# ISAE-PNX/SaDVIO

Measured on AMD Instinct MI355X. Metric: BA iterations/sec (ms/solve in ms_per_solve), 20-KF/8k-landmark window, higher is better.
Workload: dtype f64; 1 GPU; synthetic 20 KF x 8000 landmarks x 40000 reprojection factors (pixel), GN 10 iters (LM step attempts, early exits disabled); windows_per_gpu=1, parallelism=single window, n_kf=20, n_lmk=8000, n_obs=40000, reduced_dim=114

## Files before the change

### sadvio_amd/csrc/ba_capi.hip

```cpp
#include <hip/hip_runtime.h>
#include <dlfcn.h>

#include <algorithm>
#include <chrono>
#include <cmath>
#include <cstdio>
#include <cstdlib>
#include <cstring>
#include <map>
#include <string>
#include <vector>

#include "../../include/sadvio_ba.h"
#include "kernels.h"
#include "dense_chol.h"
#include "marg_kernels.h"
#include "lm_kernels.h"
#include "viinit_kernels.h"
#include "nofov_kernels.h"

using namespace sadvio;

namespace {

#define HIP_TRY(expr)                                                                         \
    do {                                                                                      \
        hipError_t _e = (expr);                                                               \
        if (_e != hipSuccess) {                                                               \
            h->err = std::string(#expr) + ": " + hipGetErrorString(_e);                       \
            return SADVIO_E_HIP;                                                              \
        }                                                                                     \
    } while (0)

template <typename T>
struct DevBuf {
    T* p = nullptr;
    size_t n = 0;
    hipError_t alloc(size_t count) {
        if (count <= n && p && !view) return hipSuccess;
        if (p && !view) (void)hipFree(p);
        view = false;
        p = nullptr; n = 0;
        hipError_t e = hipMalloc((void**)&p, std::max<size_t>(count, 1) * sizeof(T));
        if (e == hipSuccess) n = count;
        return e;
    }
    bool view = false;
    void set_view(T* ptr, size_t count) { if (p && !view) (void)hipFree(p); p = ptr; n = count; view = true; }
    void release() { if (p && !view) (void)hipFree(p); p = nullptr; n = 0; view = false; }
    void swap(DevBuf& o) { std::swap(p, o.p); std::swap(n, o.n); std::swap(view, o.view); }
    DevBuf() = default;
    DevBuf(const DevBuf&) = delete;
    DevBuf& operator=(const DevBuf&) = delete;
    ~DevBuf() { release(); }
};

struct KernelClass {
    const char* name;
    double total_ms = 0;
    long long launches = 0;
};

struct HostWin {
    WinDev d;
    std::vector<int64_t> kf_id, lmk_id;
    int hb_lmk = 0;
};

}

struct NcclId { char internal[128]; };
struct RcclLib {
    void* lib = nullptr;
    void* comm = nullptr;
    int (*get_id)(NcclId*) = nullptr;
    int (*init_rank)(void**, int, NcclId, int) = nullptr;
    int (*all_reduce)(const void*, void*, size_t, int, int, void*, hipStream_t) = nullptr;
    int (*destroy)(void*) = nullptr;
    const char* (*err_string)(int) = nullptr;
    int (*comm_count)(void*, int*) = nullptr;
    int (*comm_user_rank)(void*, int*) = nullptr;
    int (*comm_cu_device)(void*, int*) = nullptr;
};

struct SrcWin {
    sadvio_flat_window v{};
    std::vector<int64_t> kf_id, lmk_id;
    std::vector<double> kf_T, kf_vel, kf_ba, kf_bg, cam_K, cam_T, cam_sigma, lmk_p, obs_meas;
    std::vector<uint8_t> kf_const, lmk_const;
    std::vector<int32_t> lmk_obs_ptr, obs_kf, obs_cam;
    std::vector<int32_t> a_ptr, a_kf, a_cam, a_src;
    std::vector<double> a_meas;
    std::vector<double> u_cam_K, u_cam_T, u_cam_sigma;
    std::vector<int32_t> u_obs_cam;
    std::vector<int> cam_map;
};

// ... 27 lines not shown
        if (pinned) { memcpy(np, pinned, used); (void)hipHostFree(pinned); }
        pinned = np; pinned_cap = cap;
    }
    void add(void* dst, const void* src, size_t bytes) {
        if (!bytes) return;
        wait();
        const size_t off = (used + 7) & ~(size_t)7;
        reserve(off + bytes);
        if (failed) return;
        memcpy(pinned + off, src, bytes);
        used = off + bytes;
        items.push_back({(unsigned long long)dst, (unsigned long long)off, (unsigned long long)bytes});
    }
    hipError_t flush(hipStream_t stream) {
        if (failed) { failed = false; items.clear(); used = 0; return hipErrorOutOfMemory; }
        if (items.empty()) return hipSuccess;
        const size_t data_bytes = (used + 7) & ~(size_t)7;
        const size_t total = data_bytes + items.size() * sizeof(UploadItem);
        reserve(total);
        if (failed) { failed = false; items.clear(); used = 0; return hipErrorOutOfMemory; }
        hipError_t e = hipSuccess;
        auto drop = [&](hipError_t err) { items.clear(); used = 0; return err; };
        if (!ev && (e = hipEventCreateWithFlags(&ev, hipEventDisableTiming)) != hipSuccess) return drop(e);
        if (dev_cap < total) {
            if (dev) { (void)hipStreamSynchronize(stream); (void)hipFree(dev); }
            dev = nullptr; dev_cap = 0;
            if ((e = hipMalloc((void**)&dev, total + total / 2)) != hipSuccess) return drop(e);
            dev_cap = total + total / 2;
        }
        memcpy(pinned + data_bytes, items.data(), items.size() * sizeof(UploadItem));
        if ((e = hipMemcpyAsync(dev, pinned, total, hipMemcpyHostToDevice, stream)) != hipSuccess) return drop(e);
        hipLaunchKernelGGL(k_scatter_uploads, dim3(64, (unsigned)std::min<size_t>(items.size(), 64)), dim3(256), 0, stream, dev, (const UploadItem*)(dev + data_bytes), (int)items.size());
        e = hipEventRecord(ev, stream);
        in_flight = e == hipSuccess;
        if (!in_flight) e = hipStreamSynchronize(stream);
        items.clear(); used = 0;
        return e;
    }
    ~UploadBatch() { wait(); if (ev) (void)hipEventDestroy(ev); if (pinned) (void)hipHostFree(pinned); if (dev) (void)hipFree(dev); }
};

struct DensePriorHost {
    int n_full = 0, n = 0, kf_keep = -1, kf_col = 0;
    bool resident = false;
    unsigned long long serial = 0;
    std::vector<double> J, r0;
    std::vector<int> lmk_index, lmk_col;
};

struct PriorState {
    bool valid = false;
    int n_full = 0, n = 0, form = 0, cut_mode = 0;
    DevBuf<double> J, r0;
    DevBuf<double> Z;
    bool z_valid = false;
    DevBuf<int> step_of;
    DevBuf<double> H, g;
    bool hg_valid = false;
    unsigned long long serial = 0;
};

struct TriLevel { int first, count, max_m, max_n; };
struct MargScratch {
    DevBuf<double> A, b, G, V, ev, Vs, Ainv, T, Ak, bk, newJ, newr, lastJ, lastr, L, Tb, Zt, S, mi, jsel, lam, wtmp, Hl;
    DevBuf<int> ditems, flag, sel, lastcol, piv_of, lc, piv_mm;
    DevBuf<MargSmall> small;
    DevBuf<NfrSpecC> spec;
    std::vector<int> lcol, items, items_l, col;
    std::vector<double> hev, hS;
    struct TriPlan { DevBuf<TriNode> nodes; std::vector<TriLevel> levels; int leaves = 0; };
    std::map<int, TriPlan> tri_plans;
};

struct LineSetHost {
    std::vector<int64_t> id;
    std::vector<double> T, model, meas;
    std::vector<unsigned char> is_const;
    std::vector<int> ptr, obs_kf, obs_cam;
    int n() const { return (int)id.size(); }
};

struct LayoutScratch {
    std::vector<double> kf_T0, kf_vel, kf_ba, kf_bg, cam_K, cam_T, cam_isig, lmk_p, obs_meas;
    std::vector<int> kf_fidx, lmk_ob, lmk_oe, obs_kf, obs_cam, tile_kf, tile_row, pkf, pcam, run_max, idx, mark, add, kfs, slot_of, chunk_ob, chunk_lm, perm;
    std::vector<unsigned char> lmk_const, obs_slot, obs_lslot;
    std::vector<char> held;
};

struct EnvCfg {
    int debug = 0;
    int lm = -1, pf_wg = -1;
    int tile_rounds = 0, lm_subs = 0, band_c = 0;
    double jacobi_tol = 1e-14;
    bool marg_last_small = false, marg_eig_mm = false, marg_pivoted = false, marg_unpivoted = false, pchol_swap = false, pchol_strict = false,
         jacobi_b4 = false, jacobi_plain = false, no_lpt = false, no_pre = false, no_fork = false, no_bcr = false, imu_items = false;
    void read() {
        auto on = [](const char* k) { return getenv(k) != nullptr; };
        auto num = [](const char* k, int unset) { const char* e = getenv(k); return e ? atoi(e) : unset; };
        debug = num("SADVIO_DEBUG", 0); lm = num("SADVIO_LM", -1); pf_wg = num("SADVIO_PF_WG", -1);
        tile_rounds = num("SADVIO_TILE_ROUNDS", 0); lm_subs = num("SADVIO_LM_SUBS", 0); band_c = num("SADVIO_BAND_C", 0);
        if (const char* e = getenv("SADVIO_JACOBI_TOL")) jacobi_tol = atof(e);
        marg_last_small = on("SADVIO_MARG_LAST_SMALL"); marg_eig_mm = on("SADVIO_MARG_EIG_MM"); marg_pivoted = on("SADVIO_MARG_PIVOTED");
        marg_unpivoted = on("SADVIO_MARG_UNPIVOTED"); pchol_swap = on("SADVIO_PCHOL_SWAP"); pchol_strict = on("SADVIO_PCHOL_STRICT");
        jacobi_b4 = on("SADVIO_JACOBI_B4"); jacobi_plain = on("SADVIO_JACOBI_PLAIN"); no_lpt = on("SADVIO_NO_LPT"); no_pre = on("SADVIO_NO_PRE"); no_fork = on("SADVIO_NO_FORK");
        no_bcr = on("SADVIO_NO_BCR");
        imu_items = on("SADVIO_IMU_ITEMS");
    }
};

struct sadvio_ba_handle {
    EnvCfg env;
    sadvio_ba_config cfg{};
    LayoutScratch ls;
    int device = 0;
    hipStream_t stream = nullptr;
    std::string err;
    std::vector<HostWin> wins;
    std::vector<Tile> tiles;
    std::vector<PriorDev> priors;
    std::vector<int> obs_perm;
    std::vector<std::vector<PriorDev>> priors_per_win;
    std::vector<std::vector<ImuDev>> imus_per_win;
    std::vector<ImuDev> imus;
    int n_kf_tot = 0, n_cam_tot = 0, n_lmk_tot = 0, n_obs_tot = 0, np_tot = 0;
    long long s_tot = 0;
    int factor_type = 0;
    int max_n_kf = 0, max_npose = 0, max_np = 0, n_big = 0;
    DevBuf<int> d_big_info;
    DevBuf<double> d_big_M;
    DevBuf<double> d_big_Lx;
    DevBuf<double> d_big_linv;
    DevBuf<double> d_coll_band;
    DevBuf<double> d_bcr;
    DevBuf<double> d_big_mid;
    bool uploaded = false, solved = false;
    bool defer = false, pending = false;
    UploadBatch up;
    int world = 1, rank = 0;
    sadvio_allreduce_fn coll_fn = nullptr;
    void* coll_ctx = nullptr;
    RcclLib rccl;
    long long red_total = 0;
    DevBuf<double> d_rank_b, d_rank_s;
    std::vector<DensePriorHost> dprior_per_win;
    PriorState prior;
    MargScratch mg;
    std::vector<SrcWin> src;
    std::vector<std::vector<char>> sp_elim;
    std::vector<int> n_obs_user;
    std::vector<std::vector<sadvio_sparse_prior>> sparse_per_win;
    std::vector<LineSetHost> lines_per_win;
    DevBuf<LineDev> d_lines;
    DevBuf<LineObsDev> d_lobs;
    DevBuf<double> d_xline, d_line_scratch;
    int n_line_tot = 0, n_lobs_tot = 0;
    DevBuf<SparseDev> d_sparse;
    DevBuf<int> d_sp_list;
    int n_sp_list = 0;
    size_t n_sparse_tot = 0;
    DevBuf<double> d_sp_scratch;
    std::vector<unsigned char> h_lmk_const_user;
    std::vector<int> h_lmk_ob, h_lmk_oe, h_kf_fidx, h_obs_kf;
    bool user_lmk_const = false;
    int n_kept = 0;
    DevBuf<int> d_lmk_red, d_kept_obs, d_dp_ints;
    DevBuf<double> d_dp_data;
    int slots_cap = 0;
    int last_slots = 0;
    DevBuf<WinDev> d_win;
    DevBuf<Tile> d_tiles;
    DevBuf<double> d_kf_T0, d_xp, d_xv, d_xba, d_xbg, d_kf_vel, d_kf_ba, d_kf_bg;
    DevBuf<int> d_kf_fidx;
    DevBuf<double> d_cam_K, d_cam_T, d_cam_isig;
    DevBuf<double> d_lmk_p, d_xl, d_s_lmk;
    DevBuf<unsigned char> d_lmk_const;
    DevBuf<int> d_lmk_ob, d_lmk_oe, d_obs_kf, d_obs_cam, d_tile_kf, d_tile_row;
    DevBuf<int> d_pre_lane, d_pre_kf;
    bool pre_ok = false, pre_dirty = false;
    DevBuf<int> d_rank_col; DevBuf<double> d_rank_x;
    DevBuf<unsigned char> d_obs_slot, d_obs_lslot;
    DevBuf<int> d_chunk_ob, d_chunk_lm, d_tile_perm;
    DevBuf<int> d_jac_ints;
    DevBuf<double> d_jac_dbl;
    DevBuf<double> d_lm_hg, d_lm_dt, d_lm_sacc;
    DevBuf<int> d_lm_sub;
    int lm_n_sub = 0, lm_ksub = 1, lm_sub_per_item = 8;
    int lm_max_cam = 1;
    int hidden_eig_count = 0;
    int marg_stats[4] = {0, 0, 0, 0};
    int lm_sub_obs = 0;
    bool gemm_run4 = false;
    bool lm_ok = false;
    long long lm_landmarks = 0;
    DevBuf<double> d_ptab;
    int max_tile_kf = 1, max_tile_free = 0, max_gemm_free = 0;
    DevBuf<double> d_obs_meas;
    DevBuf<PriorDev> d_priors;
    DevBuf<double> d_prior_lin;
    DevBuf<ImuDev> d_imus;
    DevBuf<double> d_imu_scratch;
    DevBuf<double> d_S, d_gred, d_gfull, d_hdiag, d_delta, d_s_pose;
    DevBuf<LmState> d_states;
    DevBuf<double> d_trace;
    DevBuf<long long> d_tstart;
    DevBuf<IterAcc> d_acc;
    DevBuf<FinalRec> d_final;
    FinalRec* h_final = nullptr;
    double* h_deltas = nullptr; size_t h_deltas_cap = 0; bool deltas_cached = false;
    size_t h_final_n = 0;
    std::vector<FinalRec> fin;
    DevBuf<TileAcc> d_tacc;
    DevBuf<long long> d_dbg;
    hipGraphExec_t graph_exec = nullptr;
    std::vector<unsigned char> graph_key;
    DevBuf<double> d_probe;
    bool has_lmk_const = false;
    std::vector<KernelClass> kclasses;
    hipStream_t side = nullptr;
    hipEvent_t ev_fork = nullptr, ev_lin = nullptr, ev_solved = nullptr, ev_cost = nullptr;
    std::vector<std::pair<hipEvent_t, hipEvent_t>> ev_pool;
    std::vector<std::pair<int, int>> ev_used;
    size_t ev_next = 0;
};

namespace {

int kclass_id(sadvio_ba_handle* h, const char* name) {
    for (size_t i = 0; i < h->kclasses.size(); i++)
        if (!strcmp(h->kclasses[i].name, name)) return (int)i;
    KernelClass k; k.name = name;
    h->kclasses.push_back(k);
    return (int)h->kclasses.size() - 1;
}

struct ScopedTimer {
    sadvio_ba_handle* h;
    int pool = -1;
    ScopedTimer(sadvio_ba_handle* h_, const char* name) : h(h_) {
        if (!h->cfg.profile_kernels) return;
        if (h->ev_next == h->ev_pool.size()) {
            hipEvent_t a, b;
            if (hipEventCreate(&a) != hipSuccess || hipEventCreate(&b) != hipSuccess) return;
            h->ev_pool.push_back({a, b});
        }
        pool = (int)h->ev_next++;
        h->ev_used.push_back({kclass_id(h, name), pool});
        (void)hipEventRecord(h->ev_pool[pool].first, h->stream);
    }
    ~ScopedTimer() {
        if (pool >= 0) (void)hipEventRecord(h->ev_pool[pool].second, h->stream);
    }
};

void collect_timers(sadvio_ba_handle* h) {
    for (auto& u : h->ev_used) {
        float ms = 0;
        if (hipEventElapsedTime(&ms, h->ev_pool[u.second].first, h->ev_pool[u.second].second) == hipSuccess) {
            h->kclasses[u.first].total_ms += ms;
            h->kclasses[u.first].launches += 1;
        }
    }
    h->ev_used.clear();
    h->ev_next = 0;
}

DevPtrs make_ptrs(sadvio_ba_handle* h, const SolveOpts& o, int state_stride) {
    DevPtrs P{};
    P.win = h->d_win.p; P.tiles = h->d_tiles.p;
    P.kf_T0 = h->d_kf_T0.p; P.kf_fidx = h->d_kf_fidx.p;
    P.xp = h->d_xp.p; P.xv = h->d_xv.p; P.xba = h->d_xba.p; P.xbg = h->d_xbg.p;
    P.xp_stride = 6LL * h->n_kf_tot; P.xv_stride = 3LL * h->n_kf_tot; P.xl_stride = 3LL * h->n_lmk_tot;
    P.kf_vel = h->d_kf_vel.p; P.kf_ba = h->d_kf_ba.p; P.kf_bg = h->d_kf_bg.p;
    P.cam_K = h->d_cam_K.p; P.cam_T = h->d_cam_T.p; P.cam_isig = h->d_cam_isig.p;
    P.lmk_p = h->d_lmk_p.p; P.xl = h->d_xl.p; P.s_lmk = h->d_s_lmk.p;
    P.lmk_const = h->has_lmk_const ? h->d_lmk_const.p : nullptr;
    P.lmk_ob = h->d_lmk_ob.p; P.lmk_oe = h->d_lmk_oe.p;
    P.obs_kf = h->d_obs_kf.p; P.obs_cam = h->d_obs_cam.p; P.obs_meas = h->d_obs_meas.p;
    P.obs_slot = h->d_obs_slot.p; P.tile_kf = h->d_tile_kf.p; P.tile_row = h->d_tile_row.p;
    P.pre_lane = h->pre_ok ? (const int4*)h->d_pre_lane.p : nullptr; P.pre_kf = h->pre_ok ? (const int2*)h->d_pre_kf.p : nullptr;
    P.ptab = h->d_ptab.p; P.ptab_stride = (long long)POSE_TAB * h->n_kf_tot;
    P.priors = h->d_priors.p; P.prior_lin = h->d_prior_lin.p; P.prior_lin_stride = (long long)h->priors.size() * PRIOR_LIN; P.n_prior_tot = (int)h->priors.size();
    P.imus = h->d_imus.p; P.imu_scratch = h->d_imu_scratch.p; P.imu_scratch_stride = (long long)h->imus.size() * IMU_ROW;
    P.S = h->d_S.p; P.gred = h->d_gred.p; P.gfull = h->d_gfull.p; P.hdiag = h->d_hdiag.p;
    P.delta = h->d_delta.p; P.s_pose = h->d_s_pose.p;
    P.dbg_ts = h->d_dbg.p;
    P.trace = h->d_trace.p; P.t_start = h->d_tstart.p;
    P.states = h->d_states.p; P.acc = h->d_acc.p; P.tacc = h->d_tacc.p; P.n_tiles = (int)h->tiles.size();
    P.state_stride = state_stride;
    P.final_out = h->h_final ? h->h_final : h->d_final.p;
    P.big_info = h->d_big_info.p;
    P.world = h->world; P.rank = h->rank; P.rank_b = h->d_rank_b.p; P.rank_s = h->d_rank_s.p;
    P.lmk_red = h->d_lmk_red.p; P.kept_obs = h->d_kept_obs.p; P.n_kept = h->n_kept;
    P.dp_data = h->d_dp_data.p; P.dp_ints = h->d_dp_ints.p;
    P.sparse = h->d_sparse.p; P.sp_scratch = h->d_sp_scratch.p; P.sp_list = h->d_sp_list.p;
    P.sp_scratch_stride = (long long)std::max<size_t>(h->n_sparse_tot, 1) * SPARSE_J; P.n_imu_tot = (int)h->imus.size(); P.n_sp_list = h->n_sp_list;
    P.chunk_ob = h->d_chunk_ob.p; P.chunk_lm = h->d_chunk_lm.p; P.tile_perm = h->d_tile_perm.p; P.obs_lslot = h->d_obs_lslot.p;
    P.lm_hg = h->d_lm_hg.p; P.lm_hg_stride = (long long)LM_HG * std::max(h->n_lmk_tot, 1);
    P.lm_dt = h->d_lm_dt.p; P.lm_dt_stride = (long long)LM_DT * std::max<long long>((long long)h->tiles.size(), 1) * h->lm_ksub;
    P.lm_sub = h->d_lm_sub.p; P.lm_ksub = h->lm_ksub; P.lm_sub_per_item = h->lm_sub_per_item; P.lm_sacc = h->lm_ok ? h->d_lm_sacc.p : nullptr;
    P.lines = h->d_lines.p; P.lobs = h->d_lobs.p; P.xline = h->d_xline.p; P.line_scratch = h->d_line_scratch.p;
    P.xline_stride = 6LL * h->n_line_tot;
    P.n_xp = (long long)h->d_xp.n; P.n_xv = (long long)h->d_xv.n; P.n_xl = (long long)h->d_xl.n;
    P.n_win = (int)h->wins.size();
    P.debug = h->env.debug;
    P.o = o;
    return P;
}

__global__ void k_dense_prior_prepare(const double* J, double* Jt, int nf, int n) {
    const long long idx = (long long)blockIdx.x * blockDim.x + threadIdx.x;
    if (idx < (long long)nf * n) {
        const int i = (int)(idx / n), a = (int)(idx - (long long)i * n);
        Jt[(size_t)a * nf + i] = J[idx];
    }
}

__global__ void k_sym_from_lower(const double* __restrict__ A, int n, double* __restrict__ H) {
    const long long idx = (long long)blockIdx.x * blockDim.x + threadIdx.x;
    if (idx >= (long long)n * n) return;
    const int i = (int)(idx / n), j = (int)(idx - (long long)i * n);
    H[idx] = i >= j ? A[idx] : A[(size_t)j * n + i];
}

int layout_reduced(sadvio_ba_handle* h) {
    const int n_windows = (int)h->wins.size();
    for (int w = 0; w < n_windows && w < (int)h->dprior_per_win.size(); w++) {
        const DensePriorHost& D = h->dprior_per_win[w];
        if (D.n_full > 0 && D.resident && (!h->prior.valid || h->prior.serial != D.serial || h->prior.n_full != D.n_full || h->prior.n != D.n)) {
            h->up.reset();
            h->err = "the handle's prior changed after set_dense_prior(SADVIO_PRIOR_RESIDENT) attached it to a window: attach it again"; return SADVIO_E_STATE;
        }
    }
    int red_b = 0; long long s_b = 0;
    h->max_np = 0; h->n_big = 0;
    std::vector<int> lmk_red(std::max(h->n_lmk_tot, 1), -1);
    std::vector<unsigned char> lmk_const = h->h_lmk_const_user;
    std::vector<int> kept, dp_ints;
    std::vector<SparseDev> sparse;
    std::vector<int> sp_list;
    std::vector<LineDev> lines;
    std::vector<LineObsDev> lobs;
    long long dp_total = 0;
    bool any_red = false;
    struct Prep { long long off; int nf, n, w; };
    std::vector<Prep> preps;
    for (int w = 0; w < n_windows; w++) {
        WinDev& d = h->wins[w].d;
        const DensePriorHost& D = h->dprior_per_win[w];
        int n_red = 0;
        d.dp_n_full = d.dp_n = 0; d.dp_off = 0; d.dp_int_off = 0;
        d.kept_begin = (int)kept.size() / 3;
        if (D.n_full > 0) {
            const int n = D.n, nf = D.n_full;
            std::vector<int> kind(n, -1), index(n, 0), col(n, -1);
            if (D.kf_keep >= 0) {
                const int g = d.kf_base + D.kf_keep, fi = h->h_kf_fidx[g];
                for (int q = 0; q < 15; q++) {
                    const int a = D.kf_col + q;
                    if (q < 6) { kind[a] = 0; index[a] = 6 * g + q; }
                    else { kind[a] = 1 + (q - 6) / 3; index[a] = 3 * g + (q - 6) % 3; }
                    col[a] = (fi >= 0 && q < d.dpf) ? fi * d.dpf + q : -1;
// ... 98 lines not shown
    h->d_gred.set_view(h->d_S.p + s_b, (size_t)red_b); h->d_gfull.set_view(h->d_gred.p + red_b, (size_t)red_b);
    h->d_hdiag.set_view(h->d_gfull.p + red_b, (size_t)red_b); h->d_rank_b.set_view(h->d_hdiag.p + red_b, (size_t)nrb);
    HIP_TRY(h->d_rank_s.alloc((size_t)nrb));
    HIP_TRY(h->d_delta.alloc((size_t)std::max(red_b, 1))); HIP_TRY(h->d_s_pose.alloc((size_t)std::max(red_b, 1)));
    HIP_TRY(hipMemsetAsync(h->d_S.p, 0, sizeof(double) * (size_t)std::max<long long>(h->red_total, 1), h->stream));
    HIP_TRY(hipMemsetAsync(h->d_rank_s.p, 0, sizeof(double) * (size_t)nrb, h->stream));
    HIP_TRY(h->d_sparse.alloc(std::max<size_t>(sparse.size(), 1))); HIP_TRY(h->d_sp_scratch.alloc(2 * std::max<size_t>(sparse.size(), 1) * SPARSE_J)); h->n_sparse_tot = sparse.size();
    h->up.add(h->d_sparse.p, sparse.data(), sparse.size() * sizeof(SparseDev));
    HIP_TRY(h->d_sp_list.alloc(std::max<size_t>(sp_list.size(), 1)));
    h->n_sp_list = (int)sp_list.size();
    h->up.add(h->d_sp_list.p, sp_list.data(), sp_list.size() * sizeof(int));
    h->n_line_tot = (int)lines.size(); h->n_lobs_tot = (int)lobs.size();
    HIP_TRY(h->d_lines.alloc(std::max<size_t>(lines.size(), 1))); HIP_TRY(h->d_lobs.alloc(std::max<size_t>(lobs.size(), 1)));
    HIP_TRY(h->d_xline.alloc(std::max<size_t>(12 * lines.size(), 1))); HIP_TRY(h->d_line_scratch.alloc(std::max<size_t>(lobs.size(), 1) * LINE_ROW));
    h->up.add(h->d_lines.p, lines.data(), lines.size() * sizeof(LineDev));
    h->up.add(h->d_lobs.p, lobs.data(), lobs.size() * sizeof(LineObsDev));
    if (kept.empty()) kept.assign(3, 0);
    if (dp_ints.empty()) dp_ints.push_back(0);
    HIP_TRY(h->d_tiles.alloc(h->tiles.size())); HIP_TRY(h->d_lmk_red.alloc(lmk_red.size())); HIP_TRY(h->d_lmk_const.alloc(lmk_const.size()));
    HIP_TRY(h->d_kept_obs.alloc(kept.size())); HIP_TRY(h->d_dp_ints.alloc(dp_ints.size())); HIP_TRY(h->d_dp_data.alloc((size_t)std::max<long long>(dp_total, 1)));
#define UP(dst, src) h->up.add((dst).p, (src).data(), (src).size() * sizeof((src)[0]))
    UP(h->d_tiles, h->tiles); UP(h->d_lmk_red, lmk_red); UP(h->d_lmk_const, lmk_const); UP(h->d_kept_obs, kept);
    UP(h->d_dp_ints, dp_ints);
#undef UP
    if (!preps.empty()) HIP_TRY(hipMemsetAsync(h->d_dp_data.p, 0, sizeof(double) * (size_t)dp_total, h->stream));
    for (const Prep& pr : preps) {
        const DensePriorHost& D = h->dprior_per_win[pr.w];
        double* J = h->d_dp_data.p + pr.off;
        double* r0 = J + 2 * (size_t)pr.nf * pr.n + (size_t)pr.n * pr.n;
        if (D.resident) {
            if (!h->prior.valid || h->prior.serial != D.serial || h->prior.n_full != pr.nf || h->prior.n != pr.n) {
                h->err = "the handle's prior changed after set_dense_prior(SADVIO_PRIOR_RESIDENT) attached it to a window: attach it again"; return SADVIO_E_STATE;
            }
            HIP_TRY(hipMemcpyAsync(J, h->prior.J.p, sizeof(double) * (size_t)pr.nf * pr.n, hipMemcpyDeviceToDevice, h->stream));
            HIP_TRY(hipMemcpyAsync(r0, h->prior.r0.p, sizeof(double) * (size_t)pr.nf, hipMemcpyDeviceToDevice, h->stream));
        } else {
            h->up.add(J, D.J.data(), sizeof(double) * (size_t)pr.nf * pr.n);
            h->up.add(r0, D.r0.data(), sizeof(double) * (size_t)pr.nf);
        }
    }
    if (!preps.empty()) HIP_TRY(h->up.flush(h->stream));
    for (const Prep& pr : preps) {
        double* J = h->d_dp_data.p + pr.off;
        double* Jt = J + (size_t)pr.nf * pr.n;
        double* H = Jt + (size_t)pr.n * pr.nf;
        const long long items = (long long)pr.nf * pr.n;
        hipLaunchKernelGGL(k_dense_prior_prepare, dim3((unsigned)((items + 255) / 256)), dim3(256), 0, h->stream, J, Jt, pr.nf, pr.n);
        if (h->dprior_per_win[pr.w].resident && h->prior.hg_valid && h->prior.n == pr.n && !h->env.marg_last_small)
            hipLaunchKernelGGL(k_sym_from_lower, dim3((unsigned)(((long long)pr.n * pr.n + 255) / 256)), dim3(256), 0, h->stream, h->prior.H.p, pr.n, H);
        else
        hipLaunchKernelGGL(k_mgemm, dim3((pr.n + 63) / 64, (pr.n + 63) / 64), dim3(256), 0, h->stream, H, (long long)pr.n, J, 1LL, (long long)pr.n, J, (long long)pr.n, 1LL,
                           pr.n, pr.n, pr.nf, 1.0, 0.0);
    }
    return SADVIO_OK;
}

int upload_priors(sadvio_ba_handle* h) {
    h->priors.clear();
    for (size_t w = 0; w < h->wins.size(); w++) {
        h->wins[w].d.prior_begin = (int)h->priors.size();
        for (auto& p : h->priors_per_win[w]) h->priors.push_back(p);
        h->wins[w].d.prior_end = (int)h->priors.size();
    }
    HIP_TRY(h->d_priors.alloc(h->priors.size()));
    HIP_TRY(h->d_prior_lin.alloc(2 * h->priors.size() * (size_t)PRIOR_LIN));
    if (!h->priors.empty())
        h->up.add(h->d_priors.p, h->priors.data(), h->priors.size() * sizeof(PriorDev));
    h->imus.clear();
    for (size_t w = 0; w < h->wins.size(); w++) {
        h->wins[w].d.imu_begin = (int)h->imus.size();
        for (auto& f : h->imus_per_win[w]) { h->imus.push_back(f); h->imus.back().win = (int)w; }
        h->wins[w].d.imu_end = (int)h->imus.size();
    }
    HIP_TRY(h->d_imus.alloc(h->imus.size()));
    HIP_TRY(h->d_imu_scratch.alloc(2 * h->imus.size() * (size_t)IMU_ROW));
    if (!h->imus.empty())
        h->up.add(h->d_imus.p, h->imus.data(), h->imus.size() * sizeof(ImuDev));
    std::vector<WinDev> wd(h->wins.size());
    for (size_t w = 0; w < h->wins.size(); w++) wd[w] = h->wins[w].d;
    h->up.add(h->d_win.p, wd.data(), wd.size() * sizeof(WinDev));
    HIP_TRY(h->up.flush(h->stream));
    if (h->pre_ok && h->pre_dirty) {
        hipLaunchKernelGGL(k_pre_packets, dim3((unsigned)h->tiles.size()), dim3(BUILD_THREADS), 0, h->stream, h->d_tiles.p, h->d_lmk_ob.p, h->d_lmk_oe.p, h->d_tile_kf.p,
                           h->d_kf_fidx.p, (int4*)h->d_pre_lane.p, (int2*)h->d_pre_kf.p);
        h->pre_dirty = false;
    }
    return SADVIO_OK;
}

}

extern "C" {

int sadvio_ba_device_count(void) {
    int n = 0;
    if (hipGetDeviceCount(&n) != hipSuccess) return 0;
    int ok = 0;
    for (int i = 0; i < n; i++) {
        hipDeviceProp_t p;
        if (hipGetDeviceProperties(&p, i) == hipSuccess && strstr(p.gcnArchName, "gfx950")) ok++;
    }
    return ok;
}

void sadvio_ba_default_options(sadvio_solve_options* o) {
    if (!o) return;
    memset(o, 0, sizeof(*o));
    o->max_num_iterations = 20;
    o->function_tolerance = 1e-3;
    o->jacobi_scaling = 1;
    o->max_num_consecutive_invalid_steps = 5;
    o->gradient_tolerance = 1e-10;
    o->parameter_tolerance = 1e-8;
    o->initial_trust_region_radius = 1e4;
    o->max_trust_region_radius = 1e16;
    o->min_trust_region_radius = 1e-32;
    o->min_lm_diagonal = 1e-6;
    o->max_lm_diagonal = 1e32;
    o->min_relative_decrease = 1e-3;
}

int sadvio_ba_create(const sadvio_ba_config* cfg, sadvio_ba_handle** out) {
    if (!out) return SADVIO_E_INVALID_ARG;
    *out = nullptr;
    int n = 0;
    if (hipGetDeviceCount(&n) != hipSuccess || n == 0) return SADVIO_E_NO_DEVICE;
    int dev = cfg ? cfg->device : 0;
    if (dev < 0 || dev >= n) return SADVIO_E_INVALID_ARG;
    hipDeviceProp_t prop;
    if (hipGetDeviceProperties(&prop, dev) != hipSuccess) return SADVIO_E_HIP;
    if (!strstr(prop.gcnArchName, "gfx950")) return SADVIO_E_NO_DEVICE;
    if (hipSetDevice(dev) != hipSuccess) return SADVIO_E_HIP;
    auto* h = new sadvio_ba_handle();
    h->env.read();
    if (cfg) h->cfg = *cfg;
    h->device = dev;
    if (hipStreamCreateWithFlags(&h->stream, hipStreamNonBlocking) != hipSuccess) { delete h; return SADVIO_E_HIP; }
    if (hipStreamCreateWithFlags(&h->side, hipStreamNonBlocking) != hipSuccess) h->side = nullptr;
    for (hipEvent_t* e : {&h->ev_fork, &h->ev_lin, &h->ev_solved, &h->ev_cost})
        if (hipEventCreateWithFlags(e, hipEventDisableTiming) != hipSuccess) { *e = nullptr; if (h->side) { (void)hipStreamDestroy(h->side); h->side = nullptr; } }
    *out = h;
    return SADVIO_OK;
}

void sadvio_ba_destroy(sadvio_ba_handle* h) {
    if (!h) return;
    (void)hipSetDevice(h->device);
    if (h->stream) { (void)hipStreamSynchronize(h->stream); }
    if (h->graph_exec) (void)hipGraphExecDestroy(h->graph_exec);
    if (h->rccl.comm) (void)h->rccl.destroy(h->rccl.comm);
    if (h->h_final) (void)hipHostFree(h->h_final);
    if (h->h_deltas) (void)hipHostFree(h->h_deltas);
    if (h->side) { (void)hipStreamSynchronize(h->side); (void)hipStreamDestroy(h->side); }
    for (hipEvent_t e : {h->ev_fork, h->ev_lin, h->ev_solved, h->ev_cost}) if (e) (void)hipEventDestroy(e);
    if (h->stream) (void)hipStreamDestroy(h->stream);
    for (auto& e : h->ev_pool) { (void)hipEventDestroy(e.first); (void)hipEventDestroy(e.second); }
    h->d_win.release(); h->d_tiles.release(); h->d_kf_T0.release(); h->d_xp.release(); h->d_xv.release();
    h->d_xba.release(); h->d_xbg.release(); h->d_kf_vel.release(); h->d_kf_ba.release(); h->d_kf_bg.release();
    h->d_kf_fidx.release(); h->d_cam_K.release(); h->d_cam_T.release(); h->d_cam_isig.release();
    h->d_lmk_p.release(); h->d_xl.release(); h->d_s_lmk.release(); h->d_lmk_const.release();
    h->d_lmk_ob.release(); h->d_lmk_oe.release(); h->d_obs_kf.release(); h->d_obs_cam.release();
    h->d_obs_meas.release(); h->d_priors.release(); h->d_prior_lin.release(); h->d_S.release(); h->d_rank_s.release(); h->d_gred.release(); h->d_gfull.release();
    h->d_hdiag.release(); h->d_delta.release(); h->d_s_pose.release(); h->d_states.release(); h->d_trace.release(); h->d_tstart.release(); h->d_acc.release();
    h->d_probe.release(); h->d_tile_kf.release(); h->d_tile_row.release(); h->d_obs_slot.release(); h->d_ptab.release(); h->d_tacc.release(); h->d_dbg.release(); h->d_imus.release(); h->d_imu_scratch.release();
    delete h;
}

static int build_layout(sadvio_ba_handle* h) {
    const bool dbg_t = (h->env.debug & 8192) != 0;
    auto t_start = std::chrono::steady_clock::now();
    auto lap = [&](const char* what) { if (dbg_t) { auto t = std::chrono::steady_clock::now(); fprintf(stderr, "[sadvio dbg] build_layout %-14s %.3f ms\n", what, std::chrono::duration<double, std::milli>(t - t_start).count()); t_start = t; } };
    const int n_windows = (int)h->src.size();
    HIP_TRY(hipSetDevice(h->device));
    h->solved = false;
    h->up.reset();
    h->wins.assign(n_windows, HostWin());
    h->tiles.clear();
    h->sp_elim.assign(n_windows, {});
    h->n_obs_user.assign(n_windows, 0);
    std::vector<sadvio_flat_window> views(n_windows);
    int sp_global = 0;
    for (int w = 0; w < n_windows; w++) {
        SrcWin& S = h->src[w];
        const auto& sp = h->sparse_per_win[w];
        h->sp_elim[w].assign(sp.size(), 0);
        h->n_obs_user[w] = S.v.n_obs;
        views[w] = S.v;
        {
            std::vector<int> cmap(S.v.n_cam, -1);
            S.u_cam_K.clear(); S.u_cam_T.clear(); S.u_cam_sigma.clear();
            for (int c = 0; c < S.v.n_cam; c++) {
                const double sg = S.cam_sigma.empty() ? 1.0 : S.cam_sigma[c];
                const int nu = (int)S.u_cam_sigma.size();
                for (int u = 0; u < nu && cmap[c] < 0; u++)
                    if (!memcmp(&S.u_cam_K[4 * u], &S.cam_K[4 * c], 32) && !memcmp(&S.u_cam_T[12 * u], &S.cam_T[12 * c], 96) && S.u_cam_sigma[u] == sg) cmap[c] = u;
                if (cmap[c] < 0) {
                    cmap[c] = nu;
                    S.u_cam_K.insert(S.u_cam_K.end(), &S.cam_K[4 * c], &S.cam_K[4 * c] + 4);
                    S.u_cam_T.insert(S.u_cam_T.end(), &S.cam_T[12 * c], &S.cam_T[12 * c] + 12);
                    S.u_cam_sigma.push_back(sg);
                }
            }
            S.u_obs_cam.resize(S.obs_cam.size());
            for (size_t o = 0; o < S.obs_cam.size(); o++) S.u_obs_cam[o] = cmap[S.obs_cam[o]];
            S.cam_map = cmap;
            views[w].n_cam = (int32_t)S.u_cam_sigma.size();
            views[w].cam_K = S.u_cam_K.data(); views[w].cam_T_s_f = S.u_cam_T.data(); views[w].cam_sigma = S.u_cam_sigma.data();
            views[w].obs_cam = S.u_obs_cam.data();
        }
        if (sp.empty()) { S.a_src.clear(); continue; }
        auto& held = h->ls.held;
        held.assign(std::max(S.v.n_lmk, 1), 0);
        const DensePriorHost& D = h->dprior_per_win[w];
        for (size_t i = 0; i < D.lmk_index.size(); i++) if (D.n_full > 0 && D.lmk_col[i] >= 0) held[D.lmk_index[i]] = 1;
        for (const auto& s : sp) {
            if (s.type == SADVIO_SPARSE_LMK_PRIOR) held[s.lmk0] = 1;
            if (s.type == SADVIO_SPARSE_LMK_TO_LMK) { held[s.lmk0] = 1; held[s.lmk1] = 1; }
        }
        std::vector<std::vector<int>> extra(S.v.n_lmk);
        bool any = false;
        for (size_t k = 0; k < sp.size(); k++) {
            const auto& s = sp[k];
            if (s.type != SADVIO_SPARSE_POSE_TO_LMK || held[s.lmk0]) continue;
            if (!S.lmk_const.empty() && S.lmk_const[s.lmk0]) continue;
            h->sp_elim[w][k] = 1;
            extra[s.lmk0].push_back(sp_global + (int)k);
            any = true;
        }
        sp_global += (int)sp.size();
        if (any) {
            const int ms = S.v.factor_type == SADVIO_FACTOR_PIXEL ? 2 : 3;
            S.a_ptr.assign(1, 0); S.a_kf.clear(); S.a_cam.clear(); S.a_src.clear(); S.a_meas.clear();
            for (int l = 0; l < S.v.n_lmk; l++) {
                for (int o = S.lmk_obs_ptr[l]; o < S.lmk_obs_ptr[l + 1]; o++) {
                    S.a_kf.push_back(S.obs_kf[o]); S.a_cam.push_back(S.u_obs_cam[o]); S.a_src.push_back(o);
                    for (int q = 0; q < ms; q++) S.a_meas.push_back(S.obs_meas[(size_t)ms * o + q]);
                }
                for (int gfi : extra[l])
                    for (int half = 0; half < 2; half++) {
                        const auto& s = sp[gfi - (sp_global - (int)sp.size())];
                        S.a_kf.push_back(s.kf); S.a_cam.push_back(-1 - (2 * gfi + half)); S.a_src.push_back(-1);
                        for (int q = 0; q < ms; q++) S.a_meas.push_back(0.0);
                    }
                S.a_ptr.push_back((int32_t)S.a_kf.size());
            }
            views[w].n_obs = (int32_t)S.a_kf.size();
            views[w].lmk_obs_ptr = S.a_ptr.data(); views[w].obs_kf = S.a_kf.data(); views[w].obs_cam = S.a_cam.data();
            views[w].obs_meas = S.a_meas.data();
        } else {
            S.a_src.clear();
        }
    }
    lap("views");
    const sadvio_flat_window* wins = views.data();
    h->factor_type = wins[0].factor_type;
    int kf_b = 0, cam_b = 0, lmk_b = 0, obs_b = 0;
    h->max_n_kf = h->max_npose = h->max_np = 0; h->n_big = 0;
    h->has_lmk_const = false;
    for (int w = 0; w < n_windows; w++) {
        const sadvio_flat_window& F = wins[w];
        if (F.n_kf <= 0 || F.n_cam < 0 || F.n_lmk < 0 || F.n_obs < 0 || !F.kf_T_f_w || (F.n_cam > 0 && (!F.cam_K || !F.cam_T_s_f)) ||
            (F.n_obs > 0 && F.n_cam == 0) ||
            (F.n_lmk > 0 && (!F.lmk_p || !F.lmk_obs_ptr)) || (F.n_obs > 0 && (!F.obs_kf || !F.obs_cam || !F.obs_meas))) {
            h->err = "set_windows: missing array in window " + std::to_string(w);
            return SADVIO_E_INVALID_ARG;
        }
        if (F.factor_type != h->factor_type || (F.factor_type != SADVIO_FACTOR_PIXEL && F.factor_type != SADVIO_FACTOR_ANGULAR)) {
            h->err = "set_windows: all windows of a batch must share one factor_type";
            return SADVIO_E_INVALID_ARG;
        }
        if (F.n_lmk > 0 && (F.lmk_obs_ptr[0] != 0 || F.lmk_obs_ptr[F.n_lmk] != F.n_obs)) {
            h->err = "set_windows: lmk_obs_ptr is not a CSR over n_obs";
            return SADVIO_E_INVALID_ARG;
        }
        if (F.lmk_const) h->has_lmk_const = true;
        HostWin& H = h->wins[w];
        WinDev& d = H.d;
        memset(&d, 0, sizeof(d));
        d.n_kf = F.n_kf; d.n_cam = F.n_cam; d.n_lmk = F.n_lmk; d.n_obs = F.n_obs;
        d.kf_base = kf_b; d.cam_base = cam_b; d.lmk_base = lmk_b; d.obs_base = obs_b;
        d.factor_type = F.factor_type; d.has_imu = F.has_imu;
        d.dpf = F.has_imu ? 15 : 6;
        int nfree = 0;
        for (int k = 0; k < F.n_kf; k++)
            if (!(F.kf_const && F.kf_const[k])) nfree++;
        d.n_free_kf = nfree;
        d.Npose = nfree * 6;
        d.Np = nfree * d.dpf;
        H.kf_id.assign(F.n_kf, 0); H.lmk_id.assign(F.n_lmk, 0);
        for (int k = 0; k < F.n_kf; k++) H.kf_id[k] = F.kf_id ? F.kf_id[k] : k;
        for (int l = 0; l < F.n_lmk; l++) H.lmk_id[l] = F.lmk_id ? F.lmk_id[l] : l;
        kf_b += F.n_kf; cam_b += F.n_cam; lmk_b += F.n_lmk; obs_b += F.n_obs;
        h->max_n_kf = std::max(h->max_n_kf, F.n_kf);
        h->max_npose = std::max(h->max_npose, d.Npose);
    }
    h->n_kf_tot = kf_b; h->n_cam_tot = cam_b; h->n_lmk_tot = lmk_b; h->n_obs_tot = obs_b;

    lap("  validate");
    LayoutScratch& ls = h->ls;
    auto& kf_T0 = ls.kf_T0; auto& kf_vel = ls.kf_vel; auto& kf_ba = ls.kf_ba; auto& kf_bg = ls.kf_bg; auto& kf_fidx = ls.kf_fidx;
    auto& cam_K = ls.cam_K; auto& cam_T = ls.cam_T; auto& cam_isig = ls.cam_isig; auto& lmk_p = ls.lmk_p; auto& lmk_const = ls.lmk_const;
    auto& lmk_ob = ls.lmk_ob; auto& lmk_oe = ls.lmk_oe; auto& obs_kf = ls.obs_kf; auto& obs_cam = ls.obs_cam; auto& obs_meas = ls.obs_meas;
    auto& tile_kf = ls.tile_kf; auto& tile_row = ls.tile_row; auto& obs_slot = ls.obs_slot;
    kf_T0.resize(12 * (size_t)kf_b); kf_vel.assign(3 * (size_t)kf_b, 0.0); kf_ba.assign(3 * (size_t)kf_b, 0.0); kf_bg.assign(3 * (size_t)kf_b, 0.0);
    kf_fidx.resize(kf_b);
    cam_K.resize(4 * (size_t)cam_b); cam_T.resize(12 * (size_t)cam_b); cam_isig.resize(cam_b);
    lmk_p.resize(3 * (size_t)lmk_b);
    lmk_const.assign(std::max(lmk_b, 1), 0);
    lmk_ob.resize(std::max(lmk_b, 1)); lmk_oe.resize(std::max(lmk_b, 1)); obs_kf.resize(std::max(obs_b, 1)); obs_cam.resize(std::max(obs_b, 1));
    const int ms = h->factor_type == SADVIO_FACTOR_PIXEL ? 2 : 3;
    obs_meas.resize((size_t)ms * std::max(obs_b, 1));
    tile_kf.clear(); tile_row.clear();
    obs_slot.assign(std::max(obs_b, 1), 0);
    h->obs_perm.assign(std::max(obs_b, 1), 0);
    h->max_tile_kf = 1; h->max_tile_free = 0; h->max_gemm_free = 0; h->gemm_run4 = false;
    for (int w = 0; w < n_windows; w++) {
        const sadvio_flat_window& F = wins[w];
        WinDev& d = h->wins[w].d;
        memcpy(&kf_T0[12 * (size_t)d.kf_base], F.kf_T_f_w, sizeof(double) * 12 * F.n_kf);
        if (F.kf_vel) memcpy(&kf_vel[3 * (size_t)d.kf_base], F.kf_vel, sizeof(double) * 3 * F.n_kf);
        if (F.kf_ba) memcpy(&kf_ba[3 * (size_t)d.kf_base], F.kf_ba, sizeof(double) * 3 * F.n_kf);
        if (F.kf_bg) memcpy(&kf_bg[3 * (size_t)d.kf_base], F.kf_bg, sizeof(double) * 3 * F.n_kf);
        int fi = 0;
        for (int k = 0; k < F.n_kf; k++) kf_fidx[d.kf_base + k] = (F.kf_const && F.kf_const[k]) ? -1 : fi++;
        memcpy(&cam_K[4 * (size_t)d.cam_base], F.cam_K, sizeof(double) * 4 * F.n_cam);
        memcpy(&cam_T[12 * (size_t)d.cam_base], F.cam_T_s_f, sizeof(double) * 12 * F.n_cam);
        for (int c = 0; c < F.n_cam; c++) cam_isig[d.cam_base + c] = 1.0 / (F.cam_sigma ? F.cam_sigma[c] : 1.0);
        if (F.n_lmk) memcpy(&lmk_p[3 * (size_t)d.lmk_base], F.lmk_p, sizeof(double) * 3 * F.n_lmk);
        for (int l = 0; l < F.n_lmk; l++) {
            lmk_const[d.lmk_base + l] = F.lmk_const ? F.lmk_const[l] : 0;
            lmk_ob[d.lmk_base + l] = d.obs_base + F.lmk_obs_ptr[l];
            lmk_oe[d.lmk_base + l] = d.obs_base + F.lmk_obs_ptr[l + 1];
            if (F.lmk_obs_ptr[l + 1] < F.lmk_obs_ptr[l]) { h->err = "set_windows: CSR not monotone"; return SADVIO_E_INVALID_ARG; }
        }
        lap("  concat");
        auto& pkf = ls.pkf; auto& pcam = ls.pcam; auto& run_max = ls.run_max; auto& idx = ls.idx;
        pkf.resize(std::max(F.n_obs, 1)); pcam.resize(std::max(F.n_obs, 1));
        run_max.assign(std::max(F.n_lmk, 1), 0);
        const bool has_asrc = !h->src[w].a_src.empty();
        const int32_t* asrc = has_asrc ? h->src[w].a_src.data() : nullptr;
        bool all_sorted = true;
        int hb_win = 0;
        const int* fidx_w = kf_fidx.data() + d.kf_base;
        for (int l = 0; l < F.n_lmk; l++) {
            const int o0 = F.lmk_obs_ptr[l], o1 = F.lmk_obs_ptr[l + 1];
            int run = 0, rm = 0, prev = -1, lo = 1 << 30, hi = -1;
            for (int o = o0; o < o1; o++) {
                const int kf = F.obs_kf[o];
                if (kf < prev) { all_sorted = false; }
                run = (kf == prev) ? run + 1 : 1;
                rm = std::max(rm, run);
                prev = kf;
                const int fi = fidx_w[kf];
                if (fi >= 0) { lo = std::min(lo, fi); hi = std::max(hi, fi); }
            }
            run_max[l] = rm;
            if (hi >= 0) hb_win = std::max(hb_win, hi - lo);
        }
        h->wins[w].hb_lmk = hb_win;
        if (all_sorted) {
            const int kb = d.kf_base, cb = d.cam_base, ob = d.obs_base, n = F.n_obs;
            for (int o = 0; o < n; o++) { pkf[o] = F.obs_kf[o]; obs_kf[ob + o] = kb + F.obs_kf[o]; }
            for (int o = 0; o < n; o++) { const int c = F.obs_cam[o]; pcam[o] = c; obs_cam[ob + o] = c < 0 ? c : cb + c; }
            if (has_asrc) for (int o = 0; o < n; o++) h->obs_perm[ob + o] = asrc[o];
            else for (int o = 0; o < n; o++) h->obs_perm[ob + o] = o;
            if (n) memcpy(&obs_meas[(size_t)ms * ob], F.obs_meas, sizeof(double) * (size_t)ms * n);
        } else
        for (int l = 0; l < F.n_lmk; l++) {
            const int o0 = F.lmk_obs_ptr[l], o1 = F.lmk_obs_ptr[l + 1], k_n = o1 - o0;
            int key[64];
            const int32_t* okf = F.obs_kf + o0;
            if (k_n <= 64 && F.n_kf < (1 << 22)) {
                for (int k = 0; k < k_n; k++) key[k] = (okf[k] << 8) | k;
                for (int a = 1; a < k_n; a++) {
                    const int v = key[a];
                    int b = a - 1;
                    while (b >= 0 && key[b] > v) { key[b + 1] = key[b]; b--; }
                    key[b + 1] = v;
                }
            } else {
                idx.resize(k_n);
                for (int k = 0; k < k_n; k++) idx[k] = k;
                std::stable_sort(idx.begin(), idx.end(), [&](int a, int b) { return okf[a] < okf[b]; });
            }
            int run = 0, rm = 0, prev = -1;
            const int kb = d.kf_base, cb = d.cam_base, ob = d.obs_base;
            for (int k = 0; k < k_n; k++) {
                const int rel = k_n <= 64 && F.n_kf < (1 << 22) ? (key[k] & 255) : idx[k];
                const int src = o0 + rel, dst = o0 + k;
                const int kf = okf[rel], c = F.obs_cam[src];
                pkf[dst] = kf; pcam[dst] = c;
                h->obs_perm[ob + dst] = has_asrc ? asrc[src] : src;
                obs_kf[ob + dst] = kb + kf;
                obs_cam[ob + dst] = c < 0 ? c : cb + c;
                const double* m = F.obs_meas + (size_t)ms * src;
                double* md = &obs_meas[(size_t)ms * (ob + dst)];
                md[0] = m[0]; md[1] = m[1]; if (ms == 3) md[2] = m[2];
                run = (kf == prev) ? run + 1 : 1;
                rm = std::max(rm, run);
                prev = kf;
            }
            run_max[l] = rm;
        }
        lap("  sort+permute");
        lap("  half-bandwidth");
        if (F.n_cam > MAX_WIN_CAM) { h->err = "set_windows: more than 8 distinct cameras per window"; return SADVIO_E_INVALID_ARG; }
        int tile_rounds = 1;
        {
            long long l_tot = 0;
            for (int ww = 0; ww < n_windows; ww++) l_tot += views[ww].n_lmk;
            tile_rounds = (int)std::min<long long>(16, std::max<long long>(1, (l_tot + 32LL * 2048 - 1) / (32LL * 2048)));
            if (h->env.tile_rounds > 0) tile_rounds = h->env.tile_rounds;
        }
        d.tile_begin = (int)h->tiles.size();
        {
            int l = 0;
            auto& mark = ls.mark; auto& add = ls.add; auto& kfs = ls.kfs; auto& slot_of = ls.slot_of;
            mark.assign(F.n_kf, -1); slot_of.assign(F.n_kf, -1);
            while (l < F.n_lmk || (int)h->tiles.size() == d.tile_begin) {
                Tile t{};
                t.w = w; t.lmk0 = d.lmk_base + l; t.kmax = 1; t.G = 8;
                t.dpf = d.dpf;
                t.cam_base = d.cam_base; t.n_cam = F.n_cam;
                t.first_of_window = ((int)h->tiles.size() == d.tile_begin) ? 1 : 0;
                kfs.clear();
                int nfree = 0, tile_run_max = 0;
                const int l_begin = l;
                while (l < F.n_lmk) {
                    const int k = F.lmk_obs_ptr[l + 1] - F.lmk_obs_ptr[l];
                    if (k > MAX_LMK_OBS) { h->err = "set_windows: a landmark has more than 64 observations"; return SADVIO_E_INVALID_ARG; }
                    int G = t.G;
                    while (G < k) G <<= 1;
                    const int cap = tile_rounds * BUILD_WAVES * (64 / G);
                    if (l - l_begin + 1 > cap && l > l_begin) break;
                    add.clear();
                    int add_free = 0;
                    for (int o = F.lmk_obs_ptr[l]; o < F.lmk_obs_ptr[l + 1]; o++) {
                        const int kf = pkf[o];
                        if (mark[kf] != (int)h->tiles.size()) {
                            mark[kf] = (int)h->tiles.size();
                            add.push_back(kf);
                            if (!(F.kf_const && F.kf_const[kf])) add_free++;
                        }
                    }
                    const bool fits_hard = (int)(kfs.size() + add.size()) <= MAX_TILE_KF && nfree + add_free <= MAX_TILE_FREE_KF;
                    const bool fits = fits_hard && (nfree + add_free <= MAX_GEMM_FREE_KF || l == l_begin);
                    if (!fits && l > l_begin) {
                        for (int kf : add) mark[kf] = -1;
                        break;
                    }
                    for (int kf : add) kfs.push_back(kf);
                    nfree += add_free;
                    t.G = G;
                    t.kmax = std::max(t.kmax, k);
                    tile_run_max = std::max(tile_run_max, run_max[l]);
                    l++;
                    if (!fits_hard) break;
                }
                t.lmk1 = d.lmk_base + l;
                std::sort(kfs.begin(), kfs.end());
                t.lds_mode = ((int)kfs.size() <= MAX_TILE_KF && nfree <= MAX_TILE_FREE_KF) ? ((nfree <= MAX_GEMM_FREE_KF && tile_run_max <= (has_asrc ? 4 : 2) && t.G == 8) ? 2 : 1) : 0;
                if (t.lds_mode == 2 && tile_run_max > 2) h->gemm_run4 = true;
                if (t.lds_mode == 2) h->max_gemm_free = std::max(h->max_gemm_free, nfree);
                if ((int)kfs.size() > 64) { h->err = "set_windows: a landmark is observed from more than 64 key-frames"; return SADVIO_E_INVALID_ARG; }
                t.kf_off = (int)tile_kf.size(); t.n_kf = (int)kfs.size(); t.n_free = t.lds_mode ? nfree : 0;
                int rank = 0;
                for (size_t i = 0; i < kfs.size(); i++) {
                    const int kf = kfs[i];
                    slot_of[kf] = (int)i;
                    tile_kf.push_back(d.kf_base + kf);
                    const bool is_const = F.kf_const && F.kf_const[kf];
                    if (is_const) tile_row.push_back(-1);
                    else if (t.lds_mode) tile_row.push_back(6 * rank++);
                    else tile_row.push_back(6 * kf_fidx[d.kf_base + kf]);
                }
                for (int ll = l_begin; ll < l; ll++)
                    for (int o = F.lmk_obs_ptr[ll]; o < F.lmk_obs_ptr[ll + 1]; o++)
                        obs_slot[d.obs_base + o] = (unsigned char)slot_of[pkf[o]];
                h->max_tile_kf = std::max(h->max_tile_kf, t.n_kf);
                h->max_tile_free = std::max(h->max_tile_free, t.n_free);
                h->tiles.push_back(t);
                if (F.n_lmk == 0) break;
            }
        }
        d.tile_end = (int)h->tiles.size();
        for (int ti = d.tile_begin; ti < d.tile_end; ti++) { h->tiles[ti].win_tile0 = d.tile_begin; h->tiles[ti].win_ntiles = d.tile_end - d.tile_begin; }
    }
    lap("concat+tiles");
    auto& chunk_ob = ls.chunk_ob; auto& chunk_lm = ls.chunk_lm;
    auto& obs_lslot = ls.obs_lslot;
    chunk_ob.clear(); chunk_lm.clear();
    obs_lslot.assign(std::max(obs_b, 1), 0);
    bool want_lm = lmk_b >= 65536;
    if (h->env.lm >= 0) want_lm = h->env.lm != 0;
    h->lm_ok = want_lm && !h->tiles.empty();
    h->lm_landmarks = 0;
    h->lm_sub_obs = 0;
    for (auto& t : h->tiles) {
        if (!want_lm) { t.chunk0 = t.chunk1 = 0; continue; }
        t.chunk0 = (int)chunk_lm.size();
        if (t.lds_mode != 2) h->lm_ok = false;
        int l = t.lmk0;
        while (l < t.lmk1) {
            chunk_lm.push_back(l); chunk_ob.push_back(lmk_ob[l]);
            int nl = 0, no = 0;
            while (l < t.lmk1 && nl < LM_CHUNK && no + (lmk_oe[l] - lmk_ob[l]) <= 64) {
                for (int o = lmk_ob[l]; o < lmk_oe[l]; o++) obs_lslot[o] = (unsigned char)nl;
                no += lmk_oe[l] - lmk_ob[l]; nl++; l++;
            }
            if (nl == 0) { h->lm_ok = false; l++; }
        }
        t.chunk1 = (int)chunk_lm.size();
        h->lm_landmarks += t.lmk1 - t.lmk0;
    }
    chunk_lm.push_back(lmk_b); chunk_ob.push_back(obs_b);
    if (want_lm) {
        for (const auto& t : h->tiles)
            for (int l0 = t.lmk0; l0 < t.lmk1; l0 += LM_PASS_THREADS) {
                const int l1 = std::min(l0 + LM_PASS_THREADS, t.lmk1);
                h->lm_sub_obs = std::max(h->lm_sub_obs, lmk_oe[l1 - 1] - lmk_ob[l0]);
            }
        h->lm_sub_obs = (h->lm_sub_obs + 3) & ~3;
        h->lm_max_cam = 1;
        for (const auto& t : h->tiles) h->lm_max_cam = std::max(h->lm_max_cam, t.n_cam);
        HIP_TRY(h->d_lm_hg.alloc(2 * (size_t)LM_HG * std::max(lmk_b, 1)));
        h->lm_ksub = 1;
        for (const auto& t : h->tiles) h->lm_ksub = std::max(h->lm_ksub, (t.lmk1 - t.lmk0 + LM_PASS_THREADS - 1) / LM_PASS_THREADS);
        const size_t n_rec = std::max<size_t>(h->tiles.size(), 1) * h->lm_ksub;
        HIP_TRY(h->d_lm_dt.alloc(2 * (size_t)LM_DT * n_rec));
        HIP_TRY(h->d_lm_sacc.alloc(2 * 4 * n_rec));
        HIP_TRY(hipMemsetAsync(h->d_lm_sacc.p, 0, sizeof(double) * 2 * 4 * n_rec, h->stream));
        HIP_TRY(hipMemsetAsync(h->d_lm_dt.p, 0, sizeof(double) * 2 * (size_t)LM_DT * n_rec, h->stream));
    }
    HIP_TRY(h->d_chunk_ob.alloc(chunk_ob.size())); HIP_TRY(h->d_chunk_lm.alloc(chunk_lm.size())); HIP_TRY(h->d_obs_lslot.alloc(obs_lslot.size()));
    h->up.add(h->d_chunk_ob.p, chunk_ob.data(), chunk_ob.size() * sizeof(int));
    h->up.add(h->d_chunk_lm.p, chunk_lm.data(), chunk_lm.size() * sizeof(int));
    h->up.add(h->d_obs_lslot.p, obs_lslot.data(), obs_lslot.size());
    {
        auto& perm = ls.perm;
        perm.resize(h->tiles.size());
        for (size_t i = 0; i < perm.size(); i++) perm[i] = (int)i;
        if (want_lm && !h->env.no_lpt)
            std::stable_sort(perm.begin(), perm.end(), [&](int a, int b) {
                return h->tiles[a].chunk1 - h->tiles[a].chunk0 > h->tiles[b].chunk1 - h->tiles[b].chunk0; });
        if (h->env.debug && want_lm && !perm.empty())
            fprintf(stderr, "[sadvio dbg] chunks per tile: largest %d, median %d, smallest %d\n", h->tiles[perm.front()].chunk1 - h->tiles[perm.front()].chunk0,
                    h->tiles[perm[perm.size() / 2]].chunk1 - h->tiles[perm[perm.size() / 2]].chunk0, h->tiles[perm.back()].chunk1 - h->tiles[perm.back()].chunk0);
        HIP_TRY(h->d_tile_perm.alloc(std::max<size_t>(perm.size(), 1)));
        h->up.add(h->d_tile_perm.p, perm.data(), perm.size() * sizeof(int));
        std::vector<int> sub;
        if (h->env.lm_subs > 0) h->lm_sub_per_item = h->env.lm_subs;
        if (want_lm)
            for (int ti : perm) {
                const Tile& t = h->tiles[ti];
                for (int q = 0, l0 = t.lmk0; l0 < t.lmk1; l0 += LM_PASS_THREADS * h->lm_sub_per_item, q += h->lm_sub_per_item) { sub.push_back(ti); sub.push_back(q); }
            }
        h->lm_n_sub = (int)sub.size() / 2;
        HIP_TRY(h->d_lm_sub.alloc(std::max<size_t>(sub.size(), 2)));
        h->up.add(h->d_lm_sub.p, sub.data(), sub.size() * sizeof(int));
    }
    if (h->env.debug) {
        int hist[32] = {0}, modes[3] = {0};
        for (auto& t : h->tiles) { hist[std::min(t.n_free, 31)]++; modes[t.lds_mode]++; }
        fprintf(stderr, "[sadvio dbg] %zu tiles, modes global/atomic/gemm = %d/%d/%d, max_tile_kf %d, n_free histogram:", h->tiles.size(), modes[0], modes[1], modes[2], h->max_tile_kf);
        for (int i = 0; i < 32; i++) if (hist[i]) fprintf(stderr, " %d:%d", i, hist[i]);
        fprintf(stderr, "\n");
    }
    HIP_TRY(h->d_win.alloc(n_windows)); HIP_TRY(h->d_tacc.alloc(2 * h->tiles.size()));
    if (tile_kf.empty()) { tile_kf.push_back(0); tile_row.push_back(-1); }
    HIP_TRY(h->d_tile_kf.alloc(tile_kf.size())); HIP_TRY(h->d_tile_row.alloc(tile_row.size()));
    HIP_TRY(h->d_obs_slot.alloc(obs_slot.size())); HIP_TRY(h->d_ptab.alloc(2 * (size_t)POSE_TAB * kf_b));
    HIP_TRY(h->d_kf_T0.alloc(kf_T0.size())); HIP_TRY(h->d_kf_fidx.alloc(kf_fidx.size()));
    HIP_TRY(h->d_xp.alloc(2 * 6 * (size_t)kf_b)); HIP_TRY(h->d_xv.alloc(2 * 3 * (size_t)kf_b));
    HIP_TRY(h->d_xba.alloc(2 * 3 * (size_t)kf_b)); HIP_TRY(h->d_xbg.alloc(2 * 3 * (size_t)kf_b));
    HIP_TRY(h->d_kf_vel.alloc(kf_vel.size())); HIP_TRY(h->d_kf_ba.alloc(kf_ba.size())); HIP_TRY(h->d_kf_bg.alloc(kf_bg.size()));
    HIP_TRY(h->d_cam_K.alloc(cam_K.size())); HIP_TRY(h->d_cam_T.alloc(cam_T.size())); HIP_TRY(h->d_cam_isig.alloc(cam_isig.size()));
    HIP_TRY(h->d_lmk_p.alloc(lmk_p.size())); HIP_TRY(h->d_xl.alloc(2 * 3 * (size_t)std::max(lmk_b, 1)));
    HIP_TRY(h->d_s_lmk.alloc(3 * (size_t)std::max(lmk_b, 1)));
    HIP_TRY(h->d_lmk_ob.alloc(lmk_ob.size())); HIP_TRY(h->d_lmk_oe.alloc(lmk_oe.size()));
    HIP_TRY(h->d_obs_kf.alloc(obs_kf.size())); HIP_TRY(h->d_obs_cam.alloc(obs_cam.size())); HIP_TRY(h->d_obs_meas.alloc(obs_meas.size()));
#define UP(dst, src) h->up.add((dst).p, (src).data(), (src).size() * sizeof((src)[0]))
    UP(h->d_kf_T0, kf_T0); UP(h->d_kf_fidx, kf_fidx); UP(h->d_kf_vel, kf_vel);
    UP(h->d_kf_ba, kf_ba); UP(h->d_kf_bg, kf_bg); UP(h->d_cam_K, cam_K); UP(h->d_cam_T, cam_T); UP(h->d_cam_isig, cam_isig);
    if (lmk_b) { UP(h->d_lmk_p, lmk_p); }
    UP(h->d_lmk_ob, lmk_ob); UP(h->d_lmk_oe, lmk_oe); UP(h->d_obs_kf, obs_kf);
    UP(h->d_obs_cam, obs_cam); UP(h->d_obs_meas, obs_meas); UP(h->d_tile_kf, tile_kf); UP(h->d_tile_row, tile_row); UP(h->d_obs_slot, obs_slot);
    h->pre_ok = !h->tiles.empty() && h->tiles.size() <= PRE_MAX_TILES && !h->env.no_pre;
    if (h->pre_ok) {
        HIP_TRY(h->d_pre_lane.alloc((size_t)4 * (BUILD_THREADS / 8) * h->tiles.size())); HIP_TRY(h->d_pre_kf.alloc((size_t)2 * PRE_KF * h->tiles.size()));
        h->pre_dirty = true;
    }
#undef UP
    h->h_lmk_const_user = lmk_const; h->user_lmk_const = h->has_lmk_const;
    h->h_lmk_ob = lmk_ob; h->h_lmk_oe = lmk_oe; h->h_kf_fidx = kf_fidx; h->h_obs_kf = obs_kf;
    lap("alloc+queue");
    int rc = layout_reduced(h);
    if (rc != SADVIO_OK) return rc;
    lap("layout_reduced");
    rc = upload_priors(h);
    if (rc != SADVIO_OK) return rc;
    lap("flush");
    h->uploaded = true;
    for (auto& k : h->kclasses) { k.total_ms = 0; k.launches = 0; }
    return SADVIO_OK;
}

int sadvio_ba_set_windows(sadvio_ba_handle* h, int32_t n_windows, const sadvio_flat_window* wins) {
    if (!h) return SADVIO_E_INVALID_ARG;
    if (n_windows <= 0 || !wins) { h->err = "set_windows: no windows"; return SADVIO_E_INVALID_ARG; }
    h->uploaded = false; h->solved = false;
    for (int w = 0; w < n_windows; w++) {
        const sadvio_flat_window& F = wins[w];
        if (F.n_kf <= 0 || F.n_cam < 0 || F.n_lmk < 0 || F.n_obs < 0 || !F.kf_T_f_w || (F.n_cam > 0 && (!F.cam_K || !F.cam_T_s_f)) ||
            (F.n_obs > 0 && F.n_cam == 0) ||
            (F.n_lmk > 0 && (!F.lmk_p || !F.lmk_obs_ptr)) || (F.n_obs > 0 && (!F.obs_kf || !F.obs_cam || !F.obs_meas))) {
            h->err = "set_windows: missing array in window " + std::to_string(w);
            return SADVIO_E_INVALID_ARG;
        }
        if (F.n_lmk > 0 && (F.lmk_obs_ptr[0] != 0 || F.lmk_obs_ptr[F.n_lmk] != F.n_obs)) {
            h->err = "set_windows: lmk_obs_ptr is not a CSR over n_obs";
            return SADVIO_E_INVALID_ARG;
        }
        for (int l = 0; l < F.n_lmk; l++)
            if (F.lmk_obs_ptr[l + 1] < F.lmk_obs_ptr[l]) { h->err = "set_windows: CSR not monotone"; return SADVIO_E_INVALID_ARG; }
        for (int o = 0; o < F.n_obs; o++)
            if (F.obs_kf[o] < 0 || F.obs_kf[o] >= F.n_kf || F.obs_cam[o] < 0 || F.obs_cam[o] >= F.n_cam) {
                h->err = "set_windows: observation index out of range";
                return SADVIO_E_INVALID_ARG;
            }
    }
    if ((int)h->src.size() != n_windows) h->src.assign(n_windows, SrcWin());
    for (int w = 0; w < n_windows; w++) {
        const sadvio_flat_window& F = wins[w];
        SrcWin& S = h->src[w];
        S.cam_sigma.clear(); S.kf_id.clear(); S.kf_const.clear(); S.kf_vel.clear(); S.kf_ba.clear(); S.kf_bg.clear();
        S.lmk_p.clear(); S.lmk_id.clear(); S.lmk_const.clear(); S.obs_kf.clear(); S.obs_cam.clear(); S.obs_meas.clear();
        S.a_src.clear();
        const int ms = F.factor_type == SADVIO_FACTOR_PIXEL ? 2 : 3;
        S.kf_T.assign(F.kf_T_f_w, F.kf_T_f_w + 12 * (size_t)F.n_kf);
        S.cam_K.assign(F.cam_K, F.cam_K + 4 * (size_t)F.n_cam); S.cam_T.assign(F.cam_T_s_f, F.cam_T_s_f + 12 * (size_t)F.n_cam);
        if (F.cam_sigma) S.cam_sigma.assign(F.cam_sigma, F.cam_sigma + F.n_cam);
        if (F.kf_id) S.kf_id.assign(F.kf_id, F.kf_id + F.n_kf);
        if (F.kf_const) S.kf_const.assign(F.kf_const, F.kf_const + F.n_kf);
        if (F.kf_vel) S.kf_vel.assign(F.kf_vel, F.kf_vel + 3 * (size_t)F.n_kf);
        if (F.kf_ba) S.kf_ba.assign(F.kf_ba, F.kf_ba + 3 * (size_t)F.n_kf);
        if (F.kf_bg) S.kf_bg.assign(F.kf_bg, F.kf_bg + 3 * (size_t)F.n_kf);
        if (F.n_lmk) { S.lmk_p.assign(F.lmk_p, F.lmk_p + 3 * (size_t)F.n_lmk); S.lmk_obs_ptr.assign(F.lmk_obs_ptr, F.lmk_obs_ptr + F.n_lmk + 1); }
        else S.lmk_obs_ptr.assign(1, 0);
        if (F.lmk_id) S.lmk_id.assign(F.lmk_id, F.lmk_id + F.n_lmk);
        if (F.lmk_const) S.lmk_const.assign(F.lmk_const, F.lmk_const + F.n_lmk);
        if (F.n_obs) {
            S.obs_kf.assign(F.obs_kf, F.obs_kf + F.n_obs); S.obs_cam.assign(F.obs_cam, F.obs_cam + F.n_obs);
            S.obs_meas.assign(F.obs_meas, F.obs_meas + (size_t)ms * F.n_obs);
        }
        S.v = F;
        S.v.kf_T_f_w = S.kf_T.data(); S.v.cam_K = S.cam_K.data(); S.v.cam_T_s_f = S.cam_T.data();
        S.v.cam_sigma = F.cam_sigma ? S.cam_sigma.data() : nullptr;
        S.v.kf_id = F.kf_id ? S.kf_id.data() : nullptr; S.v.kf_const = F.kf_const ? S.kf_const.data() : nullptr;
        S.v.kf_vel = F.kf_vel ? S.kf_vel.data() : nullptr; S.v.kf_ba = F.kf_ba ? S.kf_ba.data() : nullptr; S.v.kf_bg = F.kf_bg ? S.kf_bg.data() : nullptr;
        S.v.lmk_p = S.lmk_p.data(); S.v.lmk_obs_ptr = S.lmk_obs_ptr.data();
        S.v.lmk_id = F.lmk_id ? S.lmk_id.data() : nullptr; S.v.lmk_const = F.lmk_const ? S.lmk_const.data() : nullptr;
        S.v.obs_kf = S.obs_kf.data(); S.v.obs_cam = S.obs_cam.data(); S.v.obs_meas = S.obs_meas.data();
    }
    h->priors_per_win.assign(n_windows, {});
    h->imus_per_win.assign(n_windows, {});
    h->dprior_per_win.assign(n_windows, {});
    h->sparse_per_win.assign(n_windows, {});
    h->lines_per_win.assign(n_windows, {});
    if (h->defer) {
// ... 242 lines not shown
        }
        const bool need_kf = s.type == SADVIO_SPARSE_IMU_PRIOR || s.type == SADVIO_SPARSE_POSE_TO_LMK || rel;
        const bool need_l0 = s.type != SADVIO_SPARSE_IMU_PRIOR && !rel, need_l1 = s.type == SADVIO_SPARSE_LMK_TO_LMK;
        if (s.type < 0 || s.type > 4 || (need_kf && (s.kf < 0 || s.kf >= d.n_kf)) || (need_l0 && (s.lmk0 < 0 || s.lmk0 >= d.n_lmk)) ||
            (need_l1 && (s.lmk1 < 0 || s.lmk1 >= d.n_lmk || s.lmk1 == s.lmk0))) {
            h->err = "set_sparse_priors: factor " + std::to_string(i) + " has a bad type or index";
            return SADVIO_E_INVALID_ARG;
        }
    }
    h->sparse_per_win[w].assign(f, f + n);
    if (h->defer) { h->pending = true; return SADVIO_OK; }
    return build_layout(h);
}

namespace {
int run_pchol(sadvio_ba_handle* h, double* S, int n, double* G, double tau, bool allow_swap = true) {
    if (h->d_jac_ints.alloc((size_t)n + 8) != hipSuccess) return -1;
    int* piv = h->d_jac_ints.p; int* rank_d = piv + n;
    if (h->d_jac_dbl.alloc(2 * (size_t)n + 8) != hipSuccess) return -1;
    double* dg = h->d_jac_dbl.p; double* dctl = dg + 2 * (size_t)n;
    if (hipMemsetAsync(rank_d, 0, sizeof(int) * 8, h->stream) != hipSuccess) return -1;
    if (hipMemsetAsync(rank_d, 0xff, sizeof(int), h->stream) != hipSuccess) return -1;
    const bool swap_pchol = allow_swap && h->env.pchol_swap;
    if (swap_pchol) {
        for (int k0 = 0; k0 < n; k0 += PCH_NB) {
            hipLaunchKernelGGL(k_pchol_panel, dim3(1), dim3(PCH_THREADS), 0, h->stream, S, n, G, piv, dg, rank_d, dctl, k0, tau);
            const int m = n - (k0 + PCH_NB);
            if (m > 0) hipLaunchKernelGGL(k_pchol_syrk, dim3((m + 63) / 64, (m + 63) / 64), dim3(256), 0, h->stream, S, n, G, rank_d, k0);
        }
    } else {
        if (hipMemsetAsync(piv, 0xff, sizeof(int) * (size_t)n, h->stream) != hipSuccess) return -1;
        const unsigned gt = (unsigned)((n + 63) / 64);
        if (!h->env.pchol_strict) {
            const double safe = 1024.0 * n * 2.220446049250313e-16;
            const int nb = n <= PCH_THREADS ? 32 : 16;
            int launched = 0, r = -1;
            for (int round = 0; round < 64 && r < 0; round++) {
                const int np = round == 0 ? (n + nb - 1) / nb + 8 : 4;
                for (int pnl = 0; pnl < np; pnl++, launched++) {
                    if (n <= PCH_THREADS) {
                        hipLaunchKernelGGL((k_pchol_panel_rx<1, 32>), dim3(1), dim3(PCH_THREADS), 0, h->stream, S, n, G, piv, dg, rank_d, dctl, launched == 0 ? 1 : 0, tau, safe);
                        hipLaunchKernelGGL(k_pchol_syrk_mma<32>, dim3(gt, gt), dim3(256), 0, h->stream, S, n, G, rank_d);
                    } else {
                        hipLaunchKernelGGL((k_pchol_panel_rx<2, 16>), dim3(1), dim3(PCH_THREADS), 0, h->stream, S, n, G, piv, dg, rank_d, dctl, launched == 0 ? 1 : 0, tau, safe);
                        hipLaunchKernelGGL(k_pchol_syrk_mma<16>, dim3(gt, gt), dim3(256), 0, h->stream, S, n, G, rank_d);
                    }
                }
                if (hipMemcpyAsync(&r, rank_d, sizeof(int), hipMemcpyDeviceToHost, h->stream) != hipSuccess || hipStreamSynchronize(h->stream) != hipSuccess) return -1;
            }
            if ((h->env.debug & 16384)) {
                int c8[8];
                if (hipMemcpy(c8, rank_d, sizeof(c8), hipMemcpyDeviceToHost) == hipSuccess)
                    fprintf(stderr, "[sadvio dbg] relaxed pivoted cholesky n %d rank %d: %d panels launched, %d ran (%d strict), %d candidates skipped\n", n, r, launched, c8[3] + 1, c8[4], c8[5]);
            }
            return r < 0 ? -1 : r;
        } else if (n <= PCH_THREADS) {
            for (int k0 = 0; k0 < n; k0 += 32) {
                hipLaunchKernelGGL((k_pchol_panel_np<1, 32>), dim3(1), dim3(PCH_THREADS), 0, h->stream, S, n, G, piv, dg, rank_d, dctl, k0, tau);
                if (k0 + 32 < n) hipLaunchKernelGGL(k_pchol_syrk_full<32>, dim3(gt, gt), dim3(256), 0, h->stream, S, n, G, rank_d, k0);
            }
        } else {
            for (int k0 = 0; k0 < n; k0 += 16) {
                hipLaunchKernelGGL((k_pchol_panel_np<2, 16>), dim3(1), dim3(PCH_THREADS), 0, h->stream, S, n, G, piv, dg, rank_d, dctl, k0, tau);
                if (k0 + 16 < n) hipLaunchKernelGGL(k_pchol_syrk_full<16>, dim3(gt, gt), dim3(256), 0, h->stream, S, n, G, rank_d, k0);
            }
        }
    }
    int r = 0;
    if (hipMemcpyAsync(&r, rank_d, sizeof(int), hipMemcpyDeviceToHost, h->stream) != hipSuccess || hipStreamSynchronize(h->stream) != hipSuccess) return -1;
    if (r < 0) r = n;
    return r;
}

int run_jacobi_rows(sadvio_ba_handle* h, double* G, int r, int n, int* flag) {
    const bool b4 = h->env.jacobi_b4 || n > JM_MAXN;
    const int ldx = jm_ldx(n);
    const size_t jm_lds = (size_t)JM2 * ldx * sizeof(double);
    if (!b4 && hipFuncSetAttribute((const void*)k_jacobi_mma, hipFuncAttributeMaxDynamicSharedMemorySize, (int)jm_lds) != hipSuccess) return -1;
    const int jb = b4 ? JB : JM;
    const int nb = (r + jb - 1) / jb, nbpad = nb + (nb & 1);
    const double jtol = h->env.jacobi_tol;
    int sweeps = 0;
    long long* jts = nullptr;
    if ((h->env.debug & 4096) && n > 500 && h->d_dbg.alloc(128) == hipSuccess) jts = h->d_dbg.p + 44;
    for (; sweeps < 40 && nbpad >= 2; sweeps++) {
        if (hipMemsetAsync(flag, 0, sizeof(int), h->stream) != hipSuccess) return -1;
        for (int st = 0; st < nbpad - 1; st++) {
            long long* ts = sweeps == 0 && st == 3 ? jts : nullptr;
            if (!b4) hipLaunchKernelGGL(k_jacobi_mma, dim3(nbpad / 2), dim3(JAC_THREADS), jm_lds, h->stream, G, r, n, ldx, nbpad, st, jtol, flag, ts);
            else if (n <= 4 * JAC_THREADS) hipLaunchKernelGGL(k_jacobi_block<4>, dim3(nbpad / 2), dim3(JAC_THREADS), 0, h->stream, G, r, n, nbpad, st, jtol, flag);
            else hipLaunchKernelGGL(k_jacobi_block<8>, dim3(nbpad / 2), dim3(JAC_THREADS), 0, h->stream, G, r, n, nbpad, st, jtol, flag);
        }
        int f = 0;
        if (hipMemcpyAsync(&f, flag, sizeof(int), hipMemcpyDeviceToHost, h->stream) != hipSuccess || hipStreamSynchronize(h->stream) != hipSuccess) return -1;
        if ((h->env.debug & 16384)) fprintf(stderr, "[sadvio dbg] block jacobi n %d rank %d sweep %d block pairs rotated %d\n", n, r, sweeps, f);
        if (!f) { sweeps++; break; }
    }
    if (jts) {
        long long t8[8];
        if (hipMemcpy(t8, jts, sizeof(t8), hipMemcpyDeviceToHost) == hipSuccess) {
            fprintf(stderr, "[sadvio dbg] k_jacobi_mma phases (us, cumulative): gram | update loads issued | barrier | M | check | inner sweep | end:");
            for (int i = 1; i < 8; i++) fprintf(stderr, " %.2f", (t8[i] - t8[0]) * 0.01);
            fprintf(stderr, "\n");
        }
    }
    return sweeps;
}

double pchol_tau(int n, int eig_cut_mode) {
    return eig_cut_mode == SADVIO_EIG_CUT_NOISE_FLOOR ? 4.0 * n * 2.220446049250313e-16 : -1e-12 / std::max(n, 1);
}

void launch_wfac(sadvio_ba_handle* h, double* A, long long ld, int N, double* y, double* Lx, double* Ltw, double* M, int* info, const int* skip, long long* dbg) {
    const int nsteps = (N + WD - 1) / WD;
    const size_t lds_d = sizeof(double) * wd16_lds_doubles() + 64, lds_st = sizeof(double) * wdstep_lds_doubles() + 64;
    (void)hipFuncSetAttribute((const void*)k_wchol_diag16, hipFuncAttributeMaxDynamicSharedMemorySize, (int)lds_d);
    (void)hipFuncSetAttribute((const void*)k_wchol_step, hipFuncAttributeMaxDynamicSharedMemorySize, (int)lds_st);
    hipLaunchKernelGGL(k_wchol_diag16, dim3(1), dim3(SOLVE_THREADS), lds_d, h->stream, A, ld, y, (double*)nullptr, N, 0, info, skip, Ltw);
    for (int st = 0; st + 1 < nsteps; st++) {
        const int c0 = st * WD, m = N - (c0 + WD);
        const int nt = (m + CH_TS - 1) / CH_TS;
        hipLaunchKernelGGL(k_wchol_step, dim3(nt * (nt + 1) / 2 + 2), dim3(SOLVE_THREADS), lds_st, h->stream, A, ld, Lx, y,
                           Ltw + (size_t)st * WD_LT, Ltw + (size_t)(st + 1) * WD_LT, M ? M + (size_t)st * WD * WD : nullptr,
                           M ? M + (size_t)(st + 1) * WD * WD : nullptr, N, c0, info, skip, st == 1 ? dbg : nullptr);
    }
}

int run_wfac(sadvio_ba_handle* h, double* V, int n, double* y, double* Lx, double* Ltw, const double* A0, long long ld0, double tau_rel, double* dmax, int* info) {
    const int nsteps = (n + WD - 1) / WD;
    double* Ld = Ltw + (size_t)nsteps * WD_LT;
    if (hipMemsetAsync(info, 0, sizeof(int) * 2, h->stream) != hipSuccess) return -1;
    launch_wfac(h, V, (long long)n, n, y, Lx, Ltw, nullptr, info, nullptr, nullptr);
    hipLaunchKernelGGL(k_diag_max, dim3(1), dim3(256), 0, h->stream, A0, ld0, n, dmax);
    hipLaunchKernelGGL(k_wfac_diag, dim3(nsteps * WD_T), dim3(64), 0, h->stream, Ltw, n, A0, ld0, tau_rel, dmax, 1024.0 * n * 2.220446049250313e-16, Ld, info + 1);
    int st2[2] = {0, 0};
    if (hipMemcpyAsync(st2, info, sizeof(st2), hipMemcpyDeviceToHost, h->stream) != hipSuccess || hipStreamSynchronize(h->stream) != hipSuccess) return -1;
    return st2[0] == 0 && st2[1] == 0 ? 1 : 0;
}
size_t wfac_scratch_doubles(int n) { return (size_t)((n + WD - 1) / WD) * (WD_LT + WD_T * 256) + 8; }

int run_jacobi(sadvio_ba_handle* h, const double* A, long long lda, int n, int lower_only, double* G, double* V, double* ev, int* flag, int eig_cut_mode) {
    const long long nn = (long long)n * n;
    if (n >= 32 && n <= PCH_MAXN && !h->env.jacobi_plain) {
        hipLaunchKernelGGL(k_jacobi_init, dim3((unsigned)((nn + 255) / 256)), dim3(256), 0, h->stream, A, lda, n, V, G, lower_only);
        const int r = run_pchol(h, V, n, G, pchol_tau(n, eig_cut_mode));
        if (r < 0) return -1;
        const int sweeps = run_jacobi_rows(h, G, r, n, flag);
        if (sweeps < 0) return -1;
        const bool swap_pchol = h->env.pchol_swap;
        hipLaunchKernelGGL(k_eig_from_rows, dim3(n), dim3(JAC_THREADS), 0, h->stream, G, swap_pchol ? h->d_jac_ints.p : (const int*)nullptr, h->d_jac_ints.p + n, n, V, ev);
        return sweeps;
    }
    hipLaunchKernelGGL(k_jacobi_init, dim3((unsigned)((nn + 255) / 256)), dim3(256), 0, h->stream, A, lda, n, G, V, lower_only);
    const int npad = n + (n & 1);
    unsigned long long* amax = (unsigned long long*)(flag + 2);
    double* floor2 = (double*)(flag + 4);
    if (hipMemsetAsync(flag, 0, 8 * sizeof(int), h->stream) != hipSuccess) return -1;
    if (n > 0 && eig_cut_mode == SADVIO_EIG_CUT_NOISE_FLOOR) {
        hipLaunchKernelGGL(k_jacobi_floor, dim3(n), dim3(JAC_THREADS), 0, h->stream, G, n, amax, floor2, 0);
        hipLaunchKernelGGL(k_jacobi_floor, dim3(1), dim3(JAC_THREADS), 0, h->stream, G, n, amax, floor2, 1);
    }
    int sweeps = 0;
    for (; sweeps < 40 && npad >= 2; sweeps++) {
        if (hipMemsetAsync(flag, 0, sizeof(int), h->stream) != hipSuccess) return -1;
        for (int s = 0; s < npad - 1; s++)
            hipLaunchKernelGGL(k_jacobi_step, dim3(npad / 2), dim3(JAC_THREADS), 0, h->stream, G, V, n, npad, s, 1e-14, flag, floor2);
        int f = 0;
// ... 952 lines not shown
    (void)hipFuncSetAttribute((const void*)k_bcr_back<6>, hipFuncAttributeMaxDynamicSharedMemorySize, (int)lds_b);
    hipLaunchKernelGGL(k_bcr_extract, dim3(Kb), dim3(256), 0, h->stream, S, (long long)d.ld, y, B, skip, info);
    int smax = 0, s_root = 0;
    for (int sst = 1; sst < Kb; sst *= 2) {
        const int na = (Kb + sst - 1) / sst;
        if (na == 2) { s_root = sst; break; }
        hipLaunchKernelGGL(k_bcr_elim<6>, dim3(na / 2, 2), dim3(SOLVE_THREADS), lds_e, h->stream, B, sst, info, skip);
        hipLaunchKernelGGL(k_bcr_combine, dim3(na), dim3(512), lds_c, h->stream, B, sst, info, skip);
        smax = sst;
    }
    hipLaunchKernelGGL(k_bcr_root<6>, dim3(1), dim3(SOLVE_THREADS), lds_r, h->stream, B, s_root, info, skip);
    for (int sst = smax; sst >= 1; sst /= 2) {
        const int na = (Kb + sst - 1) / sst;
        hipLaunchKernelGGL(k_bcr_back<6>, dim3(na / 2), dim3(256), lds_b, h->stream, B, sst, info, skip);
    }
    hipLaunchKernelGGL(k_bcr_writeback, dim3((N + 255) / 256), dim3(256), 0, h->stream, B, y, info, skip);
    if (dbg) fprintf(stderr, "[sadvio dbg] block cyclic reduction N %d bw %d K %d\n", N, bw, Kb);
}

void solve_wide(sadvio_ba_handle* h, const WinDev& d, const BigPlan& p, double* S, double* y, int* info, const int* skip, bool dbg) {
    const int N = d.Np, nsteps = (N + WD - 1) / WD;
    double* M = h->d_big_M.p + p.M_off;
    double* Ltw = M + (size_t)nsteps * WD * WD;
    (void)hipFuncSetAttribute((const void*)k_wchol_backstep, hipFuncAttributeMaxDynamicSharedMemorySize, (int)(sizeof(double) * WD * WDS));
    launch_wfac(h, S, (long long)d.ld, N, y, h->d_big_Lx.p + p.Lx_off, Ltw, M, info, skip, dbg ? h->d_dbg.p + 106 : nullptr);
    for (int bs = nsteps - 1; bs >= 0; bs--)
        hipLaunchKernelGGL(k_wchol_backstep, dim3(1 + (bs + 1 < nsteps ? (bs * WD + 63) / 64 : 0)), dim3(SOLVE_THREADS), sizeof(double) * WD * WDS, h->stream,
                           h->d_big_Lx.p + p.Lx_off, (long long)d.ld, y, M, N, bs, info, skip);
}

void solve_panel(sadvio_ba_handle* h, const WinDev& d, const BigPlan& p, double* S, double* y, int* info, const int* skip, bool dbg) {
    const int N = d.Np;
    for (int k0 = 0; k0 < N; k0 += CH_NB) {
        const int nb = std::min(CH_NB, N - k0), s0 = k0 + nb;
        const int rows_end = std::min(N, s0 + p.bw), m = rows_end - s0;
        hipLaunchKernelGGL(k_chol_panel, dim3((m + 1 + CH_THREADS - 1) / CH_THREADS), dim3(CH_THREADS), 0, h->stream,
                           S, (long long)d.ld, y, N, k0, rows_end, info, skip, dbg && k0 == 64 ? h->d_dbg.p + 44 : nullptr);
        if (m > 0) {
            const int nt = (m + CH_TS - 1) / CH_TS;
            hipLaunchKernelGGL(k_chol_update, dim3(nt * (nt + 1) / 2 + (m + CH_THREADS - 1) / CH_THREADS), dim3(CH_THREADS), 0,
                               h->stream, S, (long long)d.ld, y, N, k0, rows_end, info, skip);
        }
    }
    hipLaunchKernelGGL(k_chol_backsolve, dim3(1), dim3(CH_THREADS), 0, h->stream, S, (long long)d.ld, y, N, p.bw, info, skip);
}

void solve_big(sadvio_ba_handle* h, const BigPlan& p, int w, int s, int stride, bool dbg) {
    const WinDev& d = h->wins[w].d;
    double* S = h->d_S.p + d.S_off;
    double* y = h->d_gred.p + d.red_off;
    int* info = h->d_big_info.p + w;
    const int* skip = (const int*)((const char*)(h->d_states.p + (size_t)w * stride + s) + offsetof(LmState, done));
    switch (p.route) {
        case BigRoute::band: case BigRoute::band_twisted: solve_band(h, d, p, S, y, info, skip, dbg); break;
        case BigRoute::bcr: solve_bcr(h, d, p, S, y, info, skip, dbg); break;
        case BigRoute::wide: solve_wide(h, d, p, S, y, info, skip, dbg); break;
        case BigRoute::panel: solve_panel(h, d, p, S, y, info, skip, dbg); break;
    }
}
}

int sadvio_ba_solve(sadvio_ba_handle* h, const sadvio_solve_options* opts, sadvio_solve_summary* summaries) {
    if (!h) return SADVIO_E_INVALID_ARG;
    if (!h->uploaded) { h->err = "solve before set_windows"; return SADVIO_E_STATE; }
    if (h->defer) { h->err = "solve between begin_update and commit_update"; return SADVIO_E_STATE; }
    sadvio_solve_options defo;
    if (!opts) { sadvio_ba_default_options(&defo); opts = &defo; }
    if (opts->max_num_iterations < 0 || opts->max_num_iterations > 1000) { h->err = "solve: max_num_iterations out of range"; return SADVIO_E_INVALID_ARG; }
    HIP_TRY(hipSetDevice(h->device));
    SolveOpts o{};
    o.max_num_iterations = opts->max_num_iterations; o.jacobi_scaling = opts->jacobi_scaling;
    o.max_num_consecutive_invalid_steps = opts->max_num_consecutive_invalid_steps;
    o.function_tolerance = opts->function_tolerance; o.gradient_tolerance = opts->gradient_tolerance;
    o.parameter_tolerance = opts->parameter_tolerance; o.initial_radius = opts->initial_trust_region_radius;
    o.max_radius = opts->max_trust_region_radius; o.min_radius = opts->min_trust_region_radius;
    o.min_lm_diagonal = opts->min_lm_diagonal; o.max_lm_diagonal = opts->max_lm_diagonal;
    o.min_relative_decrease = opts->min_relative_decrease;
    o.huber_a = opts->huber_a;
    o.max_time_ticks = (opts->max_solver_time_in_seconds > 0.0 && h->world == 1) ? opts->max_solver_time_in_seconds * 1e8 : 0.0;
    if (!(o.huber_a >= 0.0)) { h->err = "solve: huber_a must be >= 0"; return SADVIO_E_INVALID_ARG; }
    const int n_win = (int)h->wins.size();
    const int slots = std::max(1, o.max_num_iterations);
    const int stride = slots + 2;
    HIP_TRY(h->d_dbg.alloc(128));
    HIP_TRY(h->d_states.alloc((size_t)n_win * stride));
    HIP_TRY(h->d_trace.alloc((size_t)n_win * stride * 8));
    HIP_TRY(h->d_tstart.alloc(1));
    HIP_TRY(h->d_acc.alloc((size_t)n_win * stride));
    HIP_TRY(h->d_final.alloc((size_t)n_win));
    HIP_TRY(h->d_big_info.alloc((size_t)n_win));
    if (h->h_final_n < (size_t)n_win) {
        if (h->h_final) (void)hipHostFree(h->h_final);
        h->h_final = nullptr; h->h_final_n = 0;
        HIP_TRY(hipHostMalloc((void**)&h->h_final, sizeof(FinalRec) * (size_t)n_win, hipHostMallocDefault));
        h->h_final_n = (size_t)n_win;
    }
    DevPtrs P = make_ptrs(h, o, stride);
    const int n_tiles = (int)h->tiles.size();
    int max_win_tiles = 0;
    for (int w = 0; w < n_win; w++) max_win_tiles = std::max(max_win_tiles, h->wins[w].d.tile_end - h->wins[w].d.tile_begin);
    P.decide_kernel = max_win_tiles > 4 * BUILD_THREADS ? 1 : 0;
    P.imu_direct = (!h->coll_fn && P.world == 1 && !h->env.imu_items) ? 1 : 0;
    const int mtk = h->max_tile_kf;
    const size_t nt = 6 * (size_t)h->max_tile_free;
    int Rp = 16 * ((6 * h->max_gemm_free + 15) / 16);
    int strip_doubles = std::max(STAGE_VALS * 64, 2 * Rp * (32 + 2));
    size_t lds_build = tile_tables_bytes(mtk) + sizeof(double) * ((size_t)BUILD_WAVES * strip_doubles + nt * (nt + 1) / 2 + 3 * nt +
                                                                   0) + 16;
    if (lds_build > 160 * 1024 && h->max_gemm_free > 0) {
        for (auto& t : h->tiles) if (t.lds_mode == 2) t.lds_mode = 1;
        HIP_TRY(hipMemcpyAsync(h->d_tiles.p, h->tiles.data(), h->tiles.size() * sizeof(Tile), hipMemcpyHostToDevice, h->stream));
        h->max_gemm_free = 0;
        Rp = 0; strip_doubles = STAGE_VALS * 64;
        lds_build = tile_tables_bytes(mtk) + sizeof(double) * ((size_t)BUILD_WAVES * strip_doubles + nt * (nt + 1) / 2 + 3 * nt +
                                                               0) + 16;
    }
    if (h->env.debug) fprintf(stderr, "[sadvio dbg] lds_build %zu B, Rp %d, strip_doubles %d, max_tile_kf %d, max_tile_free %d, tiles %d\n", lds_build, Rp, strip_doubles, mtk, h->max_tile_free, n_tiles);
    const size_t lds_back = tile_tables_bytes(mtk) + sizeof(double) * ((size_t)mtk * 18) + 16;
    const size_t npq = (size_t)h->max_np;
    const size_t lds_solve = sizeof(double) * ((size_t)c16_size((int)npq) + 4 * npq + 1 + C16_WORK + 16 * (size_t)c16_blocks((int)npq + 1) + SOLVE_KFC * SOLVE_KFC_STRIDE) + 64;
    bool any_pseudo = false;
    for (const auto& v : h->sp_elim) for (char e : v) any_pseudo |= e != 0;
    bool any_kept_lmk = false;
    for (int w = 0; w < n_win; w++) any_kept_lmk |= h->wins[w].d.n_red > 0;
    const bool rare = o.huber_a > 0.0 || h->n_kept > 0 || any_kept_lmk || any_pseudo || h->gemm_run4;
    const bool pix = h->factor_type == SADVIO_FACTOR_PIXEL;
    const bool have_pf = !h->imus.empty() || h->n_sp_list > 0;
    bool with_imu = have_pf && n_tiles <= 3 * 256;
    if (h->env.pf_wg >= 0) with_imu = have_pf && h->env.pf_wg != 0;
    auto kb = with_imu ? (pix ? (rare ? k_build<0, true, true> : k_build<0, false, true>) : (rare ? k_build<1, true, true> : k_build<1, false, true>))
                       : (pix ? (rare ? k_build<0, true, false> : k_build<0, false, false>) : (rare ? k_build<1, true, false> : k_build<1, false, false>));
    auto kk = with_imu ? (pix ? (rare ? k_backsub<0, true, true> : k_backsub<0, false, true>) : (rare ? k_backsub<1, true, true> : k_backsub<1, false, true>))
                       : (pix ? (rare ? k_backsub<0, true, false> : k_backsub<0, false, false>) : (rare ? k_backsub<1, true, false> : k_backsub<1, false, false>));
    auto kbk = h->factor_type == SADVIO_FACTOR_PIXEL ? k_build_kept<0> : k_build_kept<1>;
    bool use_lm = h->lm_ok && !rare && !h->coll_fn && h->world == 1 && h->lm_landmarks >= 65536;
    if (h->env.lm >= 0) use_lm = h->lm_ok && !rare && !h->coll_fn && h->world == 1 && h->env.lm != 0;
    auto kbo = pix ? k_build_obs<0> : k_build_obs<1>;
    auto kps = pix ? k_lm_pass<0, false> : k_lm_pass<1, false>;
    auto kps0 = pix ? k_lm_pass<0, true> : k_lm_pass<1, true>;
    const size_t lds_views = pix ? sizeof(double) * (size_t)mtk * h->lm_max_cam * LM_VT : 0;
    const size_t lds_bobs = tile_tables_bytes(mtk) + sizeof(double) * ((size_t)BUILD_WAVES * Rp * LM_KS + nt * (nt + 1) / 2 + nt + 1 + LM_DT) + lds_views + 16;
    const size_t lds_pass0 = tile_tables_bytes(mtk) + sizeof(double) * LM_DT_COST + (size_t)h->lm_sub_obs * ((pix ? 2 : 3) * sizeof(double) + sizeof(int)) + lds_views + 16;
    const size_t lds_pass = lds_pass0 + sizeof(double) * (size_t)mtk * (POSE_TAB + 6) + lds_views;
    if (!use_lm) P.lm_sacc = nullptr;
    if (use_lm) {
        P.decide_kernel = 1;
        HIP_TRY(hipFuncSetAttribute((const void*)kbo, hipFuncAttributeMaxDynamicSharedMemorySize, (int)lds_bobs));
        HIP_TRY(hipFuncSetAttribute((const void*)kps, hipFuncAttributeMaxDynamicSharedMemorySize, (int)lds_pass));
        HIP_TRY(hipFuncSetAttribute((const void*)kps0, hipFuncAttributeMaxDynamicSharedMemorySize, (int)lds_pass0));
    }
    HIP_TRY(hipFuncSetAttribute((const void*)kb, hipFuncAttributeMaxDynamicSharedMemorySize, (int)lds_build));
    HIP_TRY(hipFuncSetAttribute((const void*)kk, hipFuncAttributeMaxDynamicSharedMemorySize, (int)lds_back));
    bool extras = false;
    for (int w = 0; w < n_win; w++) {
        const WinDev& d = h->wins[w].d;
        if (d.imu_end > d.imu_begin || d.sp_end > d.sp_begin || d.dp_n_full > 0 || d.dpf == 15 || d.lobs_end > d.lobs_begin || d.line_end > d.line_begin) extras = true;
    }
    auto ks0 = extras ? k_solve<0, true> : k_solve<0, false>;
    auto ks1 = extras ? k_solve<1, true> : k_solve<1, false>;
    auto ks2 = extras ? k_solve<2, true> : k_solve<2, false>;
    HIP_TRY(hipFuncSetAttribute((const void*)ks0, hipFuncAttributeMaxDynamicSharedMemorySize, (int)lds_solve));
    const int reset_blocks = (int)std::min<long long>(1024, std::max<long long>(1, (P.n_xl + P.n_xp + 255) / 256));
    std::vector<BigPlan> big(n_win);
    for (int w = 0; w < n_win; w++) {
        const WinDev& d = h->wins[w].d;
        if (!d.ld) continue;
        int hb = h->wins[w].hb_lmk;
// ... 63 lines not shown
            if (use_lm) {
                if (s == 0) { ScopedTimer t(h, "k_lm_pass0"); hipLaunchKernelGGL(kps0, dim3(h->lm_n_sub), dim3(LM_PASS_THREADS), lds_pass0, h->stream, P, s, mtk, h->lm_sub_obs); }
                { ScopedTimer t(h, "k_build_obs"); hipLaunchKernelGGL(kbo, dim3(n_tiles), dim3(BUILD_THREADS), lds_bobs, h->stream, P, s, mtk, Rp); }
            } else
            { ScopedTimer t(h, "k_build"); hipLaunchKernelGGL(kb, dim3(n_tiles + (with_imu ? n_pf : 0)), dim3(BUILD_THREADS), lds_build, h->stream, P, s, mtk, strip_doubles, Rp); }
            if (n_pf && (use_lm || !with_imu)) { ScopedTimer t(h, "k_pf_lin"); hipLaunchKernelGGL(k_pf_eval<false>, dim3(n_pf), dim3(BUILD_THREADS), 0, h->stream, P, s); }
            if (h->n_kept) { ScopedTimer t(h, "k_build_kept"); hipLaunchKernelGGL(kbk, dim3((h->n_kept + 127) / 128), dim3(128), 0, h->stream, P, s); }
            if (dp_max_nf > 0) {
                ScopedTimer t(h, "k_prior_r+gh");
                const int colb = (dp_max_n + 3) / 4;
                hipLaunchKernelGGL(k_prior_r, dim3((dp_max_nf + 3) / 4, n_win), dim3(256), 0, h->stream, P, s);
                hipLaunchKernelGGL(k_prior_gh, dim3(colb + (unsigned)(((long long)dp_max_n * dp_max_n + 255) / 256), n_win), dim3(256), 0, h->stream, P, s, colb);
            }
            if (h->coll_fn) {
                { ScopedTimer t(h, "k_rank_partials"); hipLaunchKernelGGL(k_rank_partials, dim3(n_win), dim3(64), 0, h->stream, P, s, 0); }
                ScopedTimer t(h, "allreduce_reduced_system");
                const WinDev& d0 = h->wins[0].d;
                if (n_win == 1 && d0.ld && big[0].bw < d0.Np && d0.S_off == 0) {
                    const long long nbd = (long long)d0.Np * big[0].bw, tail = h->red_total - (long long)d0.Np * d0.ld;
                    if (h->d_coll_band.alloc((size_t)(nbd + tail)) != hipSuccess) coll_failed = true;
                    else {
                        const int pb = (int)std::min<long long>((nbd + tail + 255) / 256, 2048);
                        hipLaunchKernelGGL(k_band_pack, dim3(pb), dim3(256), 0, h->stream, h->d_S.p, (long long)d0.ld, d0.Np, big[0].bw, tail, h->d_coll_band.p, 0);
                        if (h->coll_fn(h->coll_ctx, h->d_coll_band.p, (int64_t)(nbd + tail), (void*)h->stream) != 0) coll_failed = true;
                        hipLaunchKernelGGL(k_band_pack, dim3(pb), dim3(256), 0, h->stream, h->d_S.p, (long long)d0.ld, d0.Np, big[0].bw, tail, h->d_coll_band.p, 1);
                    }
                } else if (h->coll_fn(h->coll_ctx, h->d_S.p, (int64_t)h->red_total, (void*)h->stream) != 0) coll_failed = true;
            }
            if (fork) (void)hipStreamWaitEvent(h->stream, h->ev_lin, 0);
            else {
                if (n_lo) { ScopedTimer t(h, "k_line_lin"); hipLaunchKernelGGL(k_line_eval<true>, dim3(n_lo), dim3(64), 0, h->stream, P, s, 0); }
            }
            if (h->n_big < n_win) { ScopedTimer t(h, "k_solve"); hipLaunchKernelGGL(ks0, dim3(n_win), dim3(SOLVE_THREADS), lds_solve, h->stream, P, s); }
            if (h->n_big) {
                { ScopedTimer t(h, "k_solve_front"); hipLaunchKernelGGL(ks1, dim3(n_win), dim3(SOLVE_THREADS), 64, h->stream, P, s); }
                {
                    ScopedTimer t(h, "reduced_cholesky_solve");
                    for (int w = 0; w < n_win; w++)
                        if (h->wins[w].d.ld) solve_big(h, big[w], w, s, stride, (P.debug & 4096) && s == 3);
                }
                { ScopedTimer t(h, "k_solve_back"); hipLaunchKernelGGL(ks2, dim3(n_win), dim3(SOLVE_THREADS), 64, h->stream, P, s); }
                for (int w = 0; w < n_win; w++) {
                    const WinDev& d = h->wins[w].d;
                    if (!d.ld) continue;
                    if (big[w].banded())
                        hipLaunchKernelGGL(k_band_zero, dim3((unsigned)std::min<long long>(((long long)d.Np * big[w].bw + 255) / 256, 4096)), dim3(256), 0, h->stream,
                                           h->d_S.p + d.S_off, (long long)d.ld, d.Np, big[w].bw);
                    else (void)hipMemsetAsync(h->d_S.p + d.S_off, 0, sizeof(double) * (size_t)d.Np * d.Np, h->stream);
                }
            }
            if (fork) {
                (void)hipEventRecord(h->ev_solved, h->stream);
                (void)hipStreamWaitEvent(h->side, h->ev_solved, 0);
                if (n_lo) hipLaunchKernelGGL(k_line_eval<false>, dim3(n_lo), dim3(64), 0, h->side, P, s, 0);
                (void)hipEventRecord(h->ev_cost, h->side);
            } else {
                if (n_lo) { ScopedTimer t(h, "k_line_cost"); hipLaunchKernelGGL(k_line_eval<false>, dim3(n_lo), dim3(64), 0, h->stream, P, s, 0); }
            }
            if (dp_max_nf > 0) { ScopedTimer t(h, "k_prior_m"); hipLaunchKernelGGL(k_prior_m, dim3((dp_max_nf + 3) / 4, n_win), dim3(256), 0, h->stream, P, s); }
            if (n_pf && (use_lm || !with_imu)) { ScopedTimer t(h, "k_pf_cost"); hipLaunchKernelGGL(k_pf_eval<true>, dim3(n_pf), dim3(64), 0, h->stream, P, s); }
            if (use_lm) {
                ScopedTimer t(h, "k_lm_pass"); hipLaunchKernelGGL(kps, dim3(h->lm_n_sub), dim3(LM_PASS_THREADS), lds_pass, h->stream, P, s, mtk, h->lm_sub_obs);
            }
            else
            { ScopedTimer t(h, "k_backsub"); hipLaunchKernelGGL(kk, dim3(n_tiles + (with_imu ? n_pf : 0)), dim3(BUILD_THREADS), lds_back, h->stream, P, s, mtk); }
            if (fork) (void)hipStreamWaitEvent(h->stream, h->ev_cost, 0);
            if (h->coll_fn) {
                { ScopedTimer t(h, "k_rank_partials"); hipLaunchKernelGGL(k_rank_partials, dim3(n_win), dim3(64), 0, h->stream, P, s, 1); }
                ScopedTimer t(h, "allreduce_step_partials");
                if (h->coll_fn(h->coll_ctx, h->d_rank_s.p, (int64_t)n_win * h->world * 4, (void*)h->stream) != 0) coll_failed = true;
            }
            if (P.decide_kernel) { ScopedTimer t(h, "k_decide"); hipLaunchKernelGGL(k_decide, dim3(n_win), dim3(max_win_tiles > 4 * BUILD_THREADS ? 1024 : 64), 0, h->stream, P, s, 0); }
        }
        { ScopedTimer t(h, "k_final"); hipLaunchKernelGGL(k_decide, dim3(n_win), dim3(64), 0, h->stream, P, slots - 1, 1); }
    };
    if (h->cfg.use_graph && !h->cfg.profile_kernels && !h->coll_fn) {
        std::vector<int> lay;
        for (int w = 0; w < n_win; w++) { lay.push_back(h->wins[w].d.Np); lay.push_back(h->wins[w].d.ld); lay.push_back(big[w].bw); }
        lay.push_back(h->n_kept); lay.push_back(h->lm_sub_obs); lay.push_back(h->lm_n_sub); lay.push_back(h->lm_max_cam); lay.push_back(h->n_lobs_tot); lay.push_back(h->n_line_tot); lay.push_back(h->n_big); lay.push_back(dp_max_nf); lay.push_back(dp_max_n);
        std::vector<unsigned char> key(sizeof(DevPtrs) + 8 * sizeof(int) + 3 * sizeof(size_t) + lay.size() * sizeof(int));
        unsigned char* kp = key.data();
        memcpy(kp + sizeof(DevPtrs) + 8 * sizeof(int) + 3 * sizeof(size_t), lay.data(), lay.size() * sizeof(int));
        memcpy(kp, &P, sizeof(DevPtrs)); kp += sizeof(DevPtrs);
        const int env_bits = (int)with_imu + 2 * (int)h->env.no_fork + 32 * (int)h->env.no_bcr + 128 * (int)h->env.no_lpt;
        const int ints[8] = {slots, n_tiles, n_win, mtk, strip_doubles, Rp, h->n_kf_tot, h->factor_type + 2 * (int)extras + 4 * (int)rare + 8 * (int)use_lm + 16 * env_bits};
        memcpy(kp, ints, sizeof(ints)); kp += sizeof(ints);
        const size_t szs[3] = {lds_build, lds_back, lds_solve};
        memcpy(kp, szs, sizeof(szs));
        if (!h->graph_exec || key != h->graph_key) {
            if (h->graph_exec) { (void)hipGraphExecDestroy(h->graph_exec); h->graph_exec = nullptr; }
            hipGraph_t g = nullptr;
            HIP_TRY(hipStreamBeginCapture(h->stream, hipStreamCaptureModeThreadLocal));
            enqueue();
            HIP_TRY(hipStreamEndCapture(h->stream, &g));
            HIP_TRY(hipGraphInstantiate(&h->graph_exec, g, nullptr, nullptr, 0));
            (void)hipGraphDestroy(g);
            h->graph_key = key;
        }
        HIP_TRY(hipGraphLaunch(h->graph_exec, h->stream));
    } else {
        enqueue();
    }
    HIP_TRY(hipGetLastError());
    if (coll_failed) { h->err = "solve: the all-reduce of the reduced system failed"; return SADVIO_E_RCCL; }
    HIP_TRY(hipStreamSynchronize(h->stream));
    if (h->cfg.profile_kernels) collect_timers(h);
    if ((h->env.debug & 4096)) {
        long long ts[128];
        if (hipMemcpy(ts, h->d_dbg.p, sizeof(ts), hipMemcpyDeviceToHost) == hipSuccess) {
            fprintf(stderr, "[sadvio dbg] phase dt (us):");
            for (int i = 1; i < 16; i++) fprintf(stderr, " %d:%.2f", i, (ts[i] - ts[0]) * 0.01);
            fprintf(stderr, "  shader clock %.3f GHz\n[sadvio dbg] k_build:", (double)(ts[21] - ts[20]) / ((ts[15] - ts[0]) * 10.0));
            for (int i = 33; i < 43; i++) fprintf(stderr, " %d:%.2f", i, (ts[i] - ts[32]) * 0.01);
            fprintf(stderr, "\n[sadvio dbg] first IMU pair of k_build, us since its start (residual + Jacobian on lane 0 | decision | W J | entries + adds): %.2f %.2f %.2f %.2f, start %.2f us after tile 0",
                    (ts[57] - ts[56]) * 0.01, (ts[58] - ts[56]) * 0.01, (ts[59] - ts[56]) * 0.01, (ts[60] - ts[56]) * 0.01, (ts[56] - ts[32]) * 0.01);
            fprintf(stderr, "\n[sadvio dbg] k_wchol_step (panel 1), us since the workgroup's start: look-ahead (operands in LDS | substituted | block updated | factored) %.2f %.2f %.2f %.2f",
                    (ts[107] - ts[106]) * 0.01, (ts[108] - ts[106]) * 0.01, (ts[109] - ts[106]) * 0.01, (ts[110] - ts[106]) * 0.01);
            fprintf(stderr, " | tile workgroup 7, %.2f us after it (operands | substituted | end) %.2f %.2f %.2f | inverse workgroup, %.2f us after it: %.2f",
                    (ts[114] - ts[106]) * 0.01, (ts[115] - ts[114]) * 0.01, (ts[116] - ts[114]) * 0.01, (ts[117] - ts[114]) * 0.01, (ts[120] - ts[106]) * 0.01, (ts[121] - ts[120]) * 0.01);
            fprintf(stderr, "\n[sadvio dbg] chol16 cycles since its first barrier (panel | trailing + next pivot, per block column):");
            for (int i = 65; i < 81; i++) fprintf(stderr, " %lld", ts[i] - ts[64]);
            fprintf(stderr, " | end %lld", ts[84] - ts[64]);
            fprintf(stderr, "\n[sadvio dbg] k_chol_panel / k_band_solve (fwd window 2: carry fresh chol store | fwd end | bwd window 2: load below steps | bwd end):");
            for (int i = 45; i < 55; i++) fprintf(stderr, " %d:%.2f", i - 44, (ts[i] - ts[44]) * 0.01);
            fprintf(stderr, "\n");
        }
    }
    h->fin.assign(h->h_final, h->h_final + n_win);
    h->deltas_cached = false;
    h->last_slots = slots;
    h->solved = true;
    int rc = SADVIO_OK;
    for (int w = 0; w < n_win; w++) {
        const LmState& s = h->fin[w].s;
        if (summaries) {
            sadvio_solve_summary& S = summaries[w];
            S.iterations = s.iter; S.num_successful_steps = s.n_success; S.num_unsuccessful_steps = s.n_unsuccess;
            S.termination = s.termination; S.initial_cost = s.initial_cost; S.final_cost = s.x_cost;
            S.fixed_cost = 0.5 * h->fin[w].fixed_cost; S.final_radius = s.radius;
        }
        if (s.termination == SADVIO_TERM_FAILURE) rc = SADVIO_E_NOT_USABLE;
    }
    (void)h->d_probe.alloc(1);
    return rc;
}

int sadvio_ba_get_deltas(sadvio_ba_handle* h, int32_t w, double* pose, double* lmk, double* dv, double* dba, double* dbg) {
    if (!h) return SADVIO_E_INVALID_ARG;
    if (!h->solved) { h->err = "get_deltas before solve"; return SADVIO_E_STATE; }
    if (w < 0 || w >= (int)h->wins.size()) { h->err = "get_deltas: window out of range"; return SADVIO_E_INVALID_ARG; }
    HIP_TRY(hipSetDevice(h->device));
    const WinDev& d = h->wins[w].d;
    const int cur = h->fin[w].s.cur;
    const size_t nk = (size_t)h->n_kf_tot, nl = (size_t)h->n_lmk_tot;
    const size_t o_xp = 0, o_xl = o_xp + 12 * nk, o_xv = o_xl + 6 * nl, o_xba = o_xv + 6 * nk, o_xbg = o_xba + 6 * nk, total = o_xbg + 6 * nk;
    if (!h->deltas_cached) {
        if (h->h_deltas_cap < total) {
            if (h->h_deltas) (void)hipHostFree(h->h_deltas);
            h->h_deltas = nullptr; h->h_deltas_cap = 0;
            HIP_TRY(hipHostMalloc((void**)&h->h_deltas, sizeof(double) * (total + total / 2), hipHostMallocDefault));
            h->h_deltas_cap = total + total / 2;
        }
        bool any_imu = false;
        for (const auto& hw : h->wins) any_imu |= hw.d.has_imu != 0;
        HIP_TRY(hipMemcpyAsync(h->h_deltas + o_xp, h->d_xp.p, sizeof(double) * 12 * nk, hipMemcpyDeviceToHost, h->stream));
        if (nl) HIP_TRY(hipMemcpyAsync(h->h_deltas + o_xl, h->d_xl.p, sizeof(double) * 6 * nl, hipMemcpyDeviceToHost, h->stream));
        if (any_imu) {
            HIP_TRY(hipMemcpyAsync(h->h_deltas + o_xv, h->d_xv.p, sizeof(double) * 6 * nk, hipMemcpyDeviceToHost, h->stream));
            HIP_TRY(hipMemcpyAsync(h->h_deltas + o_xba, h->d_xba.p, sizeof(double) * 6 * nk, hipMemcpyDeviceToHost, h->stream));
            HIP_TRY(hipMemcpyAsync(h->h_deltas + o_xbg, h->d_xbg.p, sizeof(double) * 6 * nk, hipMemcpyDeviceToHost, h->stream));
        } else {
            memset(h->h_deltas + o_xv, 0, sizeof(double) * 18 * nk);
        }
        HIP_TRY(hipStreamSynchronize(h->stream));
        h->deltas_cached = true;
    }
    if (pose) memcpy(pose, h->h_deltas + o_xp + (size_t)cur * 6 * nk + 6 * (size_t)d.kf_base, sizeof(double) * 6 * d.n_kf);
    if (lmk && d.n_lmk) memcpy(lmk, h->h_deltas + o_xl + (size_t)cur * 3 * nl + 3 * (size_t)d.lmk_base, sizeof(double) * 3 * d.n_lmk);
    double* outs[3] = {dv, dba, dbg};
    const size_t offs[3] = {o_xv, o_xba, o_xbg};
    for (int q = 0; q < 3; q++)
        if (outs[q]) memcpy(outs[q], h->h_deltas + offs[q] + (size_t)cur * 3 * nk + 3 * (size_t)d.kf_base, sizeof(double) * 3 * d.n_kf);
    return SADVIO_OK;
}

int sadvio_ba_get_trace(sadvio_ba_handle* h, int32_t w, int32_t cap_rows, double* rows8, int32_t* n_rows) {
    if (!h) return SADVIO_E_INVALID_ARG;
    if (!h->solved) { h->err = "get_trace before solve"; return SADVIO_E_STATE; }
    if (w < 0 || w >= (int)h->wins.size() || cap_rows < 0 || (cap_rows > 0 && !rows8)) { h->err = "get_trace: bad argument"; return SADVIO_E_INVALID_ARG; }
    HIP_TRY(hipSetDevice(h->device));
    const int stride = h->last_slots + 2;
    const int n = std::min(h->fin[w].s.iter + 1, stride);
    if (n_rows) *n_rows = n;
    const int m = std::min(n, cap_rows);
    if (m > 0) HIP_TRY(hipMemcpy(rows8, h->d_trace.p + (size_t)w * stride * 8, sizeof(double) * 8 * (size_t)m, hipMemcpyDeviceToHost));
    return SADVIO_OK;
}

int sadvio_ba_get_ids(sadvio_ba_handle* h, int32_t w, int64_t* kf_id, int64_t* lmk_id) {
    if (!h) return SADVIO_E_INVALID_ARG;
    if (w < 0 || w >= (int)h->wins.size()) { h->err = "get_ids: window out of range"; return SADVIO_E_INVALID_ARG; }
    if (kf_id) memcpy(kf_id, h->wins[w].kf_id.data(), sizeof(int64_t) * h->wins[w].kf_id.size());
    if (lmk_id) memcpy(lmk_id, h->wins[w].lmk_id.data(), sizeof(int64_t) * h->wins[w].lmk_id.size());
    return SADVIO_OK;
}

int sadvio_ba_linearize(sadvio_ba_handle* h, int32_t w, const double* pose_delta6, const double* lmk_delta3, double* r2,
                        double* Jp12, double* Jl6) {
    if (!h) return SADVIO_E_INVALID_ARG;
// ... 302 lines not shown
```

### sadvio_amd/csrc/ba_types.h

```cpp
#pragma once
#include <stdint.h>

namespace sadvio {

struct SolveOpts {
    int max_num_iterations;
    int jacobi_scaling;
    int max_num_consecutive_invalid_steps;
    int pad;
    double function_tolerance, gradient_tolerance, parameter_tolerance;
    double initial_radius, max_radius, min_radius;
    double min_lm_diagonal, max_lm_diagonal, min_relative_decrease;
    double huber_a;
    double max_time_ticks;
};

struct WinDev {
    int n_kf, n_cam, n_lmk, n_obs;
    int kf_base, cam_base, lmk_base, obs_base;
    int n_free_kf, dpf, Np, Npose;
    long long S_off;
    int red_off;
    int tile_begin, tile_end;
    int prior_begin, prior_end;
    int imu_begin, imu_end;
    int factor_type, has_imu;
    int ld;
    int n_red;
    int dp_n_full, dp_n;
    int dp_int_off;
    long long dp_off;
    int kept_begin, kept_end;
    int sp_begin, sp_end;
    int spl_begin, spl_end;
    int line_begin, line_end;
    int lobs_begin, lobs_end;
};

struct Tile {
    int w;
    int lmk0, lmk1;
    int G;
    int kf_off, n_kf;
    int n_free;
    int lds_mode;
    int dpf, Np;
    int red_off;
    int cam_base, n_cam;
    int first_of_window;
    int kmax;
    int win_tile0, win_ntiles;
    int ld;
    long long S_off;
    int chunk0, chunk1;
};

struct PriorDev {
    int kf;
    int pad;
    double T_prior[12];
    double inf[6];
};

struct ImuDev {
    int kf_i, kf_j;
    double dt;
    double dR[9], dv[3], dp[3];
    double J_dR_bg[9], J_dv_ba[9], J_dv_bg[9], J_dp_ba[9], J_dp_bg[9];
    double W[81];
    double sa, sg;
    int win, pad;
};
struct SparseDev {
    int type, kf, lmk0, lmk1;
    int win, kf2;
    double T_prior[12], v_prior[3], ba_prior[3], bg_prior[3], delta[3];
    double W[225];
};
struct LineDev {
    double T[12], model[6];
    int col;
    int win;
};
struct LineObsDev {
    int line, kf, cam, win;
    double meas[6];
};
constexpr int LINE_ROW = 4 * 12 + 4 + 2;
constexpr int SPARSE_NE = 136, SPARSE_E_G = 120, SPARSE_E_COST = 135;
constexpr int SPARSE_H = 15 * 15 + 15 + 2;
constexpr int SPARSE_IX = SPARSE_H + SPARSE_NE;
constexpr int SPARSE_COL = SPARSE_IX + SPARSE_NE;
constexpr int SPARSE_J = SPARSE_COL + 16;
constexpr int IMU_J = 9 * 24 + 9;
constexpr int IMU_NE = 355;
constexpr int IMU_E_G = 300, IMU_E_BH = 324, IMU_E_BG = 342, IMU_E_COST = 354;
constexpr int IMU_H = IMU_J + 6;
constexpr int IMU_IX = IMU_H + IMU_NE;
constexpr int IMU_META = IMU_IX + IMU_NE;
constexpr int IMU_ROW = IMU_META + 5;

struct LmState {
    double radius, decrease_factor, x_cost, x_norm, initial_cost;
    int cur;
    int done, termination, iter;
    int n_success, n_unsuccess, n_invalid, pad;
};

struct FinalRec {
    LmState s;
    double fixed_cost;
};

struct IterAcc {
    double lin_cost;
    double cand_cost;
    double mcc;
    double step_norm2;
    double cand_norm2;
    double fixed_cost;
    unsigned long long gmax_bits;
    int chol_fail;
    int time_up;
};
// ... 25 lines not shown
```

### sadvio_amd/csrc/kernels.h

```cpp
#pragma once
#include "ba_types.h"
#include "device_math.h"
#include "chol16.h"

namespace sadvio {

struct DevPtrs {
    const WinDev* win;
    const Tile* tiles;
    const double* kf_T0;
    const int* kf_fidx;
    double* xp; double* xv; double* xba; double* xbg;
    long long xp_stride, xv_stride, xl_stride;
    const double* kf_vel; const double* kf_ba; const double* kf_bg;
    const double* cam_K; const double* cam_T; const double* cam_isig;
    const double* lmk_p; double* xl; double* s_lmk;
    const unsigned char* lmk_const;
    const int* lmk_ob; const int* lmk_oe;
    const int* obs_kf; const int* obs_cam; const double* obs_meas;
    const unsigned char* obs_slot;
    const int* tile_kf;
    const int* tile_row;
    const int4* pre_lane;
    const int2* pre_kf;
    double* ptab;
    long long ptab_stride;
    const PriorDev* priors;
    double* prior_lin;
    long long prior_lin_stride;
    int n_prior_tot;
    const ImuDev* imus;
    double* imu_scratch;
    long long imu_scratch_stride;
    double* S; double* gred; double* gfull; double* hdiag; double* delta; double* s_pose;
    LmState* states;
    IterAcc* acc;
    TileAcc* tacc;
    FinalRec* final_out;
    int* big_info;
    int imu_direct;
    int decide_kernel;
    int world, rank;
    double* rank_b;
    double* rank_s;
    const int* lmk_red;
    const int* kept_obs;
    int n_kept;
    double* dp_data;
    const SparseDev* sparse;
    const int* sp_list;
    double* sp_scratch;
    long long sp_scratch_stride;
    int n_imu_tot, n_sp_list;
    const int* dp_ints;
    const int* chunk_ob;
    const int* chunk_lm;
    const int* tile_perm;
    const unsigned char* obs_lslot;
    double* lm_hg;
    double* lm_dt;
    long long lm_hg_stride, lm_dt_stride;
    const int* lm_sub;
    int lm_sub_per_item;
    int lm_ksub;
    double* lm_sacc;
    const LineDev* lines;
    const LineObsDev* lobs;
    double* xline;
    double* line_scratch;
    long long xline_stride;
    long long n_xp, n_xv, n_xl;
    int n_tiles;
    int state_stride;
    int n_win;
    long long* t_start;
    double* trace;
    long long* dbg_ts;
    int debug;
    SolveOpts o;
};

#ifdef SADVIO_KERNEL_TS
#define SADVIO_TS(slot_, idx_) do { if ((P.debug & 4096) && blockIdx.x == 0 && threadIdx.x == 0 && slot == (slot_)) P.dbg_ts[idx_] = wall_clock64(); } while (0)
#define SADVIO_TS_PTR(cond_) ((cond_) ? P.dbg_ts : nullptr)
#else
#define SADVIO_TS(slot_, idx_) do { } while (0)
#define SADVIO_TS_PTR(cond_) nullptr
#endif

__device__ __forceinline__ int tri(int i, int j) { return i * (i + 1) / 2 + j; }
__device__ __forceinline__ long long s_index(int ld, int i, int j) { return ld ? (long long)i * ld + j : (long long)c16_index(i, j); }

__device__ __forceinline__ void atomic_add_f64(double* p, double v) { unsafeAtomicAdd(p, v); }

__device__ __forceinline__ void atomic_max_u64(unsigned long long* p, unsigned long long v) { atomicMax(p, v); }

__device__ __forceinline__ LmState lm_decide(LmState s, const IterAcc& a, const SolveOpts& o) {
    if (s.done) return s;
    double x_cost = 0.5 * a.lin_cost;
    if (s.iter == 0) s.initial_cost = x_cost;
    s.x_cost = x_cost;
    s.iter += 1;
    bool valid = (a.chol_fail == 0) && (a.mcc > 0.0);
    if (!valid) {
        s.n_invalid += 1;
        s.n_unsuccess += 1;
        if (s.n_invalid >= o.max_num_consecutive_invalid_steps) { s.done = 1; s.termination = 5; return s; }
        s.radius *= 0.5;
    } else {
        s.n_invalid = 0;
        double step_norm = sqrt(a.step_norm2);
        double cand_cost = 0.5 * a.cand_cost;
        if (step_norm <= o.parameter_tolerance * (s.x_norm + o.parameter_tolerance)) {
            s.done = 1; s.termination = 2; return s;
        }
        double cost_change = x_cost - cand_cost;
        if (fabs(cost_change) <= o.function_tolerance * x_cost) { s.done = 1; s.termination = 1; return s; }
        double rel = cost_change / a.mcc;
        if (rel > o.min_relative_decrease) {
            s.cur ^= 1;
            s.x_norm = sqrt(a.cand_norm2);
            s.x_cost = cand_cost;
            double t = 2.0 * rel - 1.0;
            s.radius = s.radius / fmax(1.0 / 3.0, 1.0 - t * t * t);
            s.radius = fmin(o.max_radius, s.radius);
            s.decrease_factor = 2.0;
            s.n_success += 1;
        } else {
            s.radius = s.radius / s.decrease_factor;
            s.decrease_factor *= 2.0;
            s.n_unsuccess += 1;
        }
    }
    if (s.iter >= o.max_num_iterations) { s.done = 1; s.termination = 0; }
    else if (s.radius <= o.min_radius) { s.done = 1; s.termination = 4; }
    return s;
}

__device__ __forceinline__ void trace_write(const DevPtrs& P, int w, int slot, const LmState& prev, const IterAcc& a, const LmState& next) {
    if (!P.trace || prev.done) return;
    double* R = P.trace + ((long long)w * P.state_stride + slot) * 8;
    if (slot == 0) { R[0] = 0.5 * a.lin_cost; R[1] = 0.0; R[2] = prev.radius; R[3] = 0.0; R[4] = 0.0; R[5] = 1.0; R[7] = 0.0; }
    R[6] = __longlong_as_double((long long)a.gmax_bits);
    double* N = R + 8;
    const bool valid = a.chol_fail == 0 && a.mcc > 0.0;
    const double cc = valid ? 0.5 * (a.lin_cost - a.cand_cost) : 0.0;
    const bool judged = valid && !(next.done && (next.termination == 1 || next.termination == 2));
    N[0] = next.x_cost; N[1] = cc; N[2] = next.radius; N[3] = valid ? sqrt(a.step_norm2) : 0.0;
    N[4] = judged ? cc / a.mcc : 0.0; N[5] = next.n_success > prev.n_success ? 1.0 : 0.0; N[6] = -1.0; N[7] = a.mcc;
}

template <int CTRL>
__device__ __forceinline__ double dpp_f64_(double v) {
    int lo = __double2loint(v), hi = __double2hiint(v);
    lo = __builtin_amdgcn_update_dpp(0, lo, CTRL, 0xF, 0xF, true);
    hi = __builtin_amdgcn_update_dpp(0, hi, CTRL, 0xF, 0xF, true);
    return __hiloint2double(hi, lo);
}
__device__ __forceinline__ void swap16_pair_f64(double v, double& x0, double& x1) {
    unsigned lo = __double2loint(v), hi = __double2hiint(v);
    auto a = __builtin_amdgcn_permlane16_swap(lo, lo, false, false);
    auto b = __builtin_amdgcn_permlane16_swap(hi, hi, false, false);
    x0 = __hiloint2double(b[0], a[0]); x1 = __hiloint2double(b[1], a[1]);
}
__device__ __forceinline__ void swap32_pair_f64(double v, double& x0, double& x1) {
    unsigned lo = __double2loint(v), hi = __double2hiint(v);
    auto a = __builtin_amdgcn_permlane32_swap(lo, lo, false, false);
    auto b = __builtin_amdgcn_permlane32_swap(hi, hi, false, false);
    x0 = __hiloint2double(b[0], a[0]); x1 = __hiloint2double(b[1], a[1]);
}
// ... 180 lines not shown
    if (L.row < 0) {
#pragma unroll
        for (int i = 0; i < 12; i++) L.Jp[i] = 0.0;
    }
    if (!keep_jl) {
#pragma unroll
        for (int i = 0; i < 6; i++) L.Jl[i] = 0.0;
    }
    L.counted = (L.row >= 0) || lcounted;
    if (!L.counted) {  }
}

__device__ __forceinline__ bool group_eliminate(const DevPtrs& P, const ObsLin& L, int G, int gl, bool lmk_valid,
                                                bool lfree, int nobs, double radius, bool write_scale, bool leader,
                                                double* Mi, double* g) {
    double H[6];
    H[0] = L.Jl[0] * L.Jl[0] + L.Jl[3] * L.Jl[3];
    H[1] = L.Jl[0] * L.Jl[1] + L.Jl[3] * L.Jl[4];
    H[2] = L.Jl[0] * L.Jl[2] + L.Jl[3] * L.Jl[5];
    H[3] = L.Jl[1] * L.Jl[1] + L.Jl[4] * L.Jl[4];
    H[4] = L.Jl[1] * L.Jl[2] + L.Jl[4] * L.Jl[5];
    H[5] = L.Jl[2] * L.Jl[2] + L.Jl[5] * L.Jl[5];
    g[0] = L.Jl[0] * L.r[0] + L.Jl[3] * L.r[1];
    g[1] = L.Jl[1] * L.r[0] + L.Jl[4] * L.r[1];
    g[2] = L.Jl[2] * L.r[0] + L.Jl[5] * L.r[1];
#pragma unroll
    for (int i = 0; i < 6; i++) H[i] = group_sum(H[i], G);
#pragma unroll
    for (int i = 0; i < 3; i++) g[i] = group_sum(g[i], G);
    const bool active = lmk_valid && lfree && nobs > 0;
    if (!active) {
#pragma unroll
        for (int i = 0; i < 6; i++) Mi[i] = 0.0;
        return false;
    }
    double s[3];
    if (write_scale) {
        s[0] = P.o.jacobi_scaling ? 1.0 / (1.0 + sqrt(H[0])) : 1.0;
        s[1] = P.o.jacobi_scaling ? 1.0 / (1.0 + sqrt(H[3])) : 1.0;
        s[2] = P.o.jacobi_scaling ? 1.0 / (1.0 + sqrt(H[5])) : 1.0;
        if (leader) {
            P.s_lmk[3 * (long long)gl] = s[0]; P.s_lmk[3 * (long long)gl + 1] = s[1]; P.s_lmk[3 * (long long)gl + 2] = s[2];
        }
    } else {
        s[0] = P.s_lmk[3 * (long long)gl]; s[1] = P.s_lmk[3 * (long long)gl + 1]; s[2] = P.s_lmk[3 * (long long)gl + 2];
    }
    const double ir = 1.0 / radius;
    const double s0 = s[0] * s[0], s1 = s[1] * s[1], s2 = s[2] * s[2];
    double M[6] = {H[0], H[1], H[2], H[3], H[4], H[5]};
    M[0] += fmin(fmax(s0 * H[0], P.o.min_lm_diagonal), P.o.max_lm_diagonal) * ir / s0;
    M[3] += fmin(fmax(s1 * H[3], P.o.min_lm_diagonal), P.o.max_lm_diagonal) * ir / s1;
    M[5] += fmin(fmax(s2 * H[5], P.o.min_lm_diagonal), P.o.max_lm_diagonal) * ir / s2;
    sym3_chol_inverse(M, Mi);
    return true;
}

__device__ __forceinline__ void stage_tables(const DevPtrs& P, const Tile& T, int buf, double* poseTab, double* camTab,
                                             int* rowTab) {
    const int tid = threadIdx.x;
    const double* src = P.ptab + (long long)buf * P.ptab_stride;
    for (int i = tid; i < T.n_kf * POSE_TAB; i += blockDim.x) {
        const int k = i / POSE_TAB, e = i - k * POSE_TAB;
        poseTab[i] = src[(long long)P.tile_kf[T.kf_off + k] * POSE_TAB + e];
    }
    for (int i = tid; i < T.n_cam * 17; i += blockDim.x) {
        const int c = i / 17, e = i - 17 * c;
        const int gc = T.cam_base + c;
        camTab[i] = e < 4 ? P.cam_K[4 * (long long)gc + e] : (e < 16 ? P.cam_T[12 * (long long)gc + e - 4] : P.cam_isig[gc]);
    }
    for (int i = tid; i < T.n_kf; i += blockDim.x) rowTab[i] = P.tile_row[T.kf_off + i];
}

__device__ __forceinline__ void wave_lds_fence() {
    __builtin_amdgcn_fence(__ATOMIC_RELEASE, "wavefront");
    __builtin_amdgcn_wave_barrier();
    __builtin_amdgcn_fence(__ATOMIC_ACQUIRE, "wavefront");
}

__host__ __device__ inline size_t tile_tables_bytes(int n_kf) {
    size_t b = sizeof(double) * ((size_t)n_kf * POSE_TAB + MAX_WIN_CAM * 17) + sizeof(int) * (size_t)(n_kf > MAX_TILE_KF ? n_kf : MAX_TILE_KF);
    return (b + 15) & ~(size_t)15;
}

__global__ __launch_bounds__(BUILD_THREADS) void k_pre_packets(const Tile* __restrict__ tiles, const int* __restrict__ lmk_ob, const int* __restrict__ lmk_oe,
                                                               const int* __restrict__ tile_kf, const int* __restrict__ kf_fidx, int4* __restrict__ pre_lane,
                                                               int2* __restrict__ pre_kf) {
    const Tile T = tiles[blockIdx.x];
    const int tid = threadIdx.x;
    if (tid < BUILD_THREADS / 8) {
        const int lane0 = tid * 8, wv = lane0 >> 6, ln = lane0 & 63;
        const int G = T.G, lpw = 64 / G, grp = ln / G, q0 = ln - grp * G, nl = T.lmk1 - T.lmk0;
        const bool valid = wv * lpw + grp < nl;
        const int gl = T.lmk0 + (valid ? wv * lpw + grp : 0);
        const int ob = nl > 0 ? lmk_ob[gl] : 0, nobs = (valid && nl > 0) ? lmk_oe[gl] - ob : 0;
        pre_lane[(long long)blockIdx.x * (BUILD_THREADS / 8) + tid] = make_int4(gl, ob, nobs | (valid ? 1 << 16 : 0), q0);
    }
    if (tid < PRE_KF) {
        int2 e = make_int2(-1, -1);
        if (tid < T.n_kf) { e.x = tile_kf[T.kf_off + tid]; e.y = kf_fidx[e.x]; }
        pre_kf[(long long)blockIdx.x * PRE_KF + tid] = e;
    }
}

template <bool COST_ONLY> __device__ __forceinline__ void pose_factor_eval(const DevPtrs& P, int slot, int idx, int ln);
template <int FACTOR, bool RARE, bool IMU>
__global__ __launch_bounds__(BUILD_THREADS, IMU ? 1 : 2) void k_build(DevPtrs P, int slot, int max_tile_kf, int strip_doubles, int Rp) {
    extern __shared__ __attribute__((aligned(16))) char smem[];
    if (IMU && (int)blockIdx.x >= P.n_tiles) {
        pose_factor_eval<false>(P, slot, (int)blockIdx.x - P.n_tiles, threadIdx.x);
        return;
    }
    const Tile T = P.tiles[blockIdx.x];
    const int tid = threadIdx.x, wv = tid >> 6, ln = tid & 63;
    int4 pl = make_int4(0, -1, 0, 0);
    int2 pk = make_int2(-1, -1);
    if (P.pre_lane) {
        pl = P.pre_lane[(long long)blockIdx.x * (BUILD_THREADS / 8) + (tid >> 3)];
        pk = P.pre_kf[(long long)blockIdx.x * PRE_KF + tid / POSE_TAB];
    }
    SADVIO_TS(3, 32);
    __shared__ double s_part[BUILD_WAVES * 4];
    double* poseTab = (double*)smem;
    double* camTab = poseTab + (size_t)max_tile_kf * POSE_TAB;
    int* rowTab = (int*)(camTab + MAX_WIN_CAM * 17);
    double* stage = (double*)(smem + tile_tables_bytes(max_tile_kf));
    const int G = T.G, lpw = 64 / G;
    const int grp = ln / G, q = ln - grp * G;
    const int nl = T.lmk1 - T.lmk0;
    LmState st;
    IterAcc a;
    LmState prev;
    const bool own_decision = !(slot == 0 || P.decide_kernel);
    double pc = 0.0, pm = 0.0, psn = 0.0, pcn = 0.0;
    auto decision_inputs = [&](int dec_w, int t0, int nt) {
        if (!own_decision) {
            st = P.states[(long long)dec_w * P.state_stride + slot];
            return;
        }
        a = P.acc[(long long)dec_w * P.state_stride + slot - 1];
        prev = P.states[(long long)dec_w * P.state_stride + slot - 1];
        if (P.world > 1) {
            if (wv == 0) {
                const double* rs = P.rank_s + (long long)dec_w * P.world * 4;
                for (int r = ln; r < P.world; r += 64) { pc += rs[4 * r]; pm += rs[4 * r + 1]; psn += rs[4 * r + 2]; pcn += rs[4 * r + 3]; }
            }
        } else {
            const TileAcc* ta = P.tacc + (long long)((slot - 1) & 1) * P.n_tiles + t0;
            double v[4][4];
#pragma unroll
            for (int u = 0; u < 4; u++) {
                const int t = tid + u * BUILD_THREADS;
                const bool in = t < nt;
                const TileAcc* e = ta + (in ? t : 0);
                v[u][0] = in ? e->cand_cost : 0.0; v[u][1] = in ? e->mcc : 0.0; v[u][2] = in ? e->step_norm2 : 0.0; v[u][3] = in ? e->cand_norm2 : 0.0;
            }
            pc = (v[0][0] + v[1][0]) + (v[2][0] + v[3][0]); pm = (v[0][1] + v[1][1]) + (v[2][1] + v[3][1]);
            psn = (v[0][2] + v[1][2]) + (v[2][2] + v[3][2]); pcn = (v[0][3] + v[1][3]) + (v[2][3] + v[3][3]);
        }
    };
    if (P.n_win == 1) decision_inputs(0, 0, P.n_tiles);
    else decision_inputs(T.w, T.win_tile0, T.win_ntiles);
    bool first_valid;
    int gl_first, pre_ob, pre_oe, pre_o;
    if (P.pre_lane) {
        first_valid = (pl.z >> 16) & 1; gl_first = pl.x; pre_ob = pl.y; pre_oe = pl.y + (pl.z & 0xff);
        pre_o = (pl.w + (tid & 7) < (pl.z & 0xff)) ? pl.y + pl.w + (tid & 7) : -1;
    } else {
        first_valid = wv * lpw + grp < nl;
        gl_first = T.lmk0 + (first_valid ? wv * lpw + grp : 0);
        pre_ob = P.lmk_ob[gl_first]; pre_oe = P.lmk_oe[gl_first];
        pre_o = (first_valid && q < pre_oe - pre_ob) ? pre_ob + q : -1;
    }
    const int pre_lcode = P.lmk_const ? P.lmk_const[gl_first] : 0;
    double pre_p[3], pre_x0[3], pre_x1[3];
#pragma unroll
    for (int i = 0; i < 3; i++) {
        pre_p[i] = P.lmk_p[3 * (long long)gl_first + i];
        pre_x0[i] = P.xl[3 * (long long)gl_first + i];
        pre_x1[i] = P.xl[P.xl_stride + 3 * (long long)gl_first + i];
    }
    double pre_t0 = 0.0, pre_t1 = 0.0;
    if (P.pre_lane) {
        if (pk.x >= 0) {
            const long long src = (long long)pk.x * POSE_TAB + (tid - (tid / POSE_TAB) * POSE_TAB);
            pre_t0 = P.ptab[src]; pre_t1 = P.ptab[P.ptab_stride + src];
        }
    } else if (tid < T.n_kf * POSE_TAB) {
        const int k = tid / POSE_TAB, e = tid - k * POSE_TAB;
        const long long src = (long long)P.tile_kf[T.kf_off + k] * POSE_TAB + e;
        pre_t0 = P.ptab[src]; pre_t1 = P.ptab[P.ptab_stride + src];
    }
    for (int i = tid; i < T.n_cam * 17; i += blockDim.x) {
        const int c = i / 17, e = i - 17 * c;
        const int gc = T.cam_base + c;
        camTab[i] = e < 4 ? P.cam_K[4 * (long long)gc + e] : (e < 16 ? P.cam_T[12 * (long long)gc + e - 4] : P.cam_isig[gc]);
    }
    for (int i = tid; i < T.n_kf; i += blockDim.x) rowTab[i] = P.tile_row[T.kf_off + i];
    ObsPre pre_obs;
    pre_obs.slot = 0; pre_obs.craw = 0; pre_obs.m[0] = pre_obs.m[1] = pre_obs.m[2] = 0.0;
    if (pre_o >= 0) pre_obs = obs_prefetch<FACTOR>(P, pre_o);
    if (own_decision) {
        pc = wave_sum(pc); pm = wave_sum(pm); psn = wave_sum(psn); pcn = wave_sum(pcn);
        if (ln == 0) { s_part[wv * 4] = pc; s_part[wv * 4 + 1] = pm; s_part[wv * 4 + 2] = psn; s_part[wv * 4 + 3] = pcn; }
        __syncthreads();
        a.cand_cost += (s_part[0] + s_part[4]) + (s_part[8] + s_part[12]); a.mcc += (s_part[1] + s_part[5]) + (s_part[9] + s_part[13]);
        a.step_norm2 += (s_part[2] + s_part[6]) + (s_part[10] + s_part[14]); a.cand_norm2 += (s_part[3] + s_part[7]) + (s_part[11] + s_part[15]);
        st = lm_decide(prev, a, P.o);
        __syncthreads();
        if (T.first_of_window && tid == 0) { P.states[(long long)T.w * P.state_stride + slot] = st; trace_write(P, T.w, slot - 1, prev, a, st); }
    }
    if (st.done) return;
    SADVIO_TS(3, 33);
    double* Stile = stage + BUILD_WAVES * strip_doubles;
    const int Nt = 6 * T.n_free;
    const int tri_n = Nt * (Nt + 1) / 2;
    double* gT = Stile + tri_n;
    double* gfT = gT + Nt;
    double* hdT = gfT + Nt;
    const bool lds_mode = T.lds_mode != 0;
    if (tid < T.n_kf * POSE_TAB) poseTab[tid] = st.cur ? pre_t1 : pre_t0;
    {
        const double* src = P.ptab + (long long)st.cur * P.ptab_stride;
        for (int i = tid + blockDim.x; i < T.n_kf * POSE_TAB; i += blockDim.x) {
            const int k = i / POSE_TAB, e = i - k * POSE_TAB;
            poseTab[i] = src[(long long)P.tile_kf[T.kf_off + k] * POSE_TAB + e];
        }
    }
    if (lds_mode) {
        const int nz = tri_n + 3 * Nt;
        for (int i = tid; i < nz; i += blockDim.x) Stile[i] = 0.0;
    }
    __syncthreads();

    SADVIO_TS(3, 34);
    double* Sg = P.S + T.S_off;
    double* gredg = P.gred + T.red_off;
    double* gfullg = P.gfull + T.red_off;
    double* hdg = P.hdiag + T.red_off;
    const int dpf = T.dpf, Np = T.Np;
    const double* xl = P.xl + (long long)st.cur * P.xl_stride;
    double* wstage = stage + wv * strip_doubles;
    const bool gemm_mode = T.lds_mode == 2;
    double cost_part = 0.0, fixed_part = 0.0, gmax_part = 0.0;
    typedef double d4 __attribute__((ext_vector_type(4)));
    d4 accs[3] = {(d4){0.0, 0.0, 0.0, 0.0}, (d4){0.0, 0.0, 0.0, 0.0}, (d4){0.0, 0.0, 0.0, 0.0}};
    for (int base = wv * lpw; base < nl; base += BUILD_WAVES * lpw) {
        const int lm = base + grp;
        const bool lmk_valid = lm < nl;
        const int gl = T.lmk0 + (lmk_valid ? lm : 0);
        const bool first = base == wv * lpw;
        const int ob = first ? pre_ob : P.lmk_ob[gl], oe = first ? pre_oe : P.lmk_oe[gl];
        const int nobs = lmk_valid ? oe - ob : 0;
        const int lcode = first ? pre_lcode : (P.lmk_const ? P.lmk_const[gl] : 0);
        const bool lfree = lcode == 0;
        ObsLin L;
        L.valid = q < nobs;
        L.row = -1; L.slot = 0; L.counted = false;
        if (L.valid) {
            double pw[3];
            ObsPre obq;
            if (first) {
#pragma unroll
                for (int i = 0; i < 3; i++) pw[i] = pre_p[i] + (st.cur ? pre_x1[i] : pre_x0[i]);
                obq = pre_obs;
            } else {
#pragma unroll
                for (int i = 0; i < 3; i++) pw[i] = P.lmk_p[3 * (long long)gl + i] + xl[3 * (long long)gl + i];
                obq = obs_prefetch<FACTOR>(P, ob + q);
            }
            lane_linearize<FACTOR, RARE>(P, poseTab, camTab, rowTab, T.cam_base, obq, pw, lfree, lcode != 1, L);
            const double c = L.rho;
            if (L.counted) cost_part += c;
            else { fixed_part += c; L.r[0] = 0.0; L.r[1] = 0.0; }
        } else {
            L.r[0] = L.r[1] = 0.0;
#pragma unroll
            for (int i = 0; i < 12; i++) L.Jp[i] = 0.0;
#pragma unroll
            for (int i = 0; i < 6; i++) L.Jl[i] = 0.0;
        }
    SADVIO_TS(3, 35);
        double Mi[6], g[3];
        const bool active = group_eliminate(P, L, G, gl, lmk_valid, lfree, nobs, st.radius, slot == 0, q == 0, Mi, g);
        if (active && q == 0) gmax_part = fmax(gmax_part, fmax(fabs(g[0]), fmax(fabs(g[1]), fabs(g[2]))));
    SADVIO_TS(3, 36);
        double N[6], gam[3];
        li_row(Mi, L.Jl[0], L.Jl[1], L.Jl[2], N);
        li_row(Mi, L.Jl[3], L.Jl[4], L.Jl[5], N + 3);
        li_vec(Mi, g, gam);
        if (gemm_mode) {
            constexpr int Kw = 32, KS = Kw + 2;
            double* Yb = wstage;
            const double* Eb = Yb;
            {
                double2* z = (double2*)wstage;
                const double2 zero2 = make_double2(0.0, 0.0);
                for (int i = ln; i < Rp * KS / 2; i += 64) z[i] = zero2;
            }
            const bool vrow = L.valid && L.row >= 0;
            const int myrow = vrow ? L.row : -2 - ln;
            const int row_prev = dpp_i32<0x111>(myrow);
            const int row_next = dpp_i32<0x101>(myrow);
            const bool follower = vrow && q > 0 && row_prev == myrow;
            const bool has_follower = vrow && q + 1 < G && row_next == myrow;
            const int row_next2 = RARE ? dpp_i32<0x102>(myrow) : -1;
            const bool has_follower2 = RARE && vrow && q + 2 < G && row_next2 == myrow;
            const bool head = vrow && !follower;
            const double rt0 = L.r[0] - (N[0] * gam[0] + N[1] * gam[1] + N[2] * gam[2]);
            const double rt1 = L.r[1] - (N[3] * gam[0] + N[4] * gam[1] + N[5] * gam[2]);
            wave_lds_fence();
    SADVIO_TS(3, 37);
#pragma unroll
            for (int i = 0; i < 6; i++) {
                const double j0 = vrow ? L.Jp[i] : 0.0, j1 = vrow ? L.Jp[6 + i] : 0.0;
                double y[3];
#pragma unroll
                for (int c = 0; c < 3; c++) {
                    y[c] = j0 * N[c] + j1 * N[3 + c];
                    const double yn = dpp_f64<0x101>(y[c]);
                    if (has_follower) y[c] += yn;
                    if (RARE) {
                        const double yn2 = dpp_f64<0x102>(y[c]);
                        if (has_follower2) y[c] += yn2;
                    }
                }
                if (head) {
                    double2* yp = (double2*)(Yb + (myrow + i) * KS + 4 * grp);
                    yp[0] = make_double2(y[0], y[1]); yp[1] = make_double2(y[2], 0.0);
                }
            }
            wave_lds_fence();
    SADVIO_TS(3, 38);
            {
// ... 98 lines not shown
#pragma unroll
                for (int i = 0; i < 6; i++) {
                    const double c0 = L.Jp[i] * w00 + L.Jp[6 + i] * w10;
                    const double c1 = L.Jp[i] * w01 + L.Jp[6 + i] * w11;
                    const int row = pa + i;
#pragma unroll
                    for (int j = 0; j < 6; j++) {
                        const int col = pb + j;
                        if (col > row) continue;
                        const double v = c0 * Jpb[j] + c1 * Jpb[6 + j];
                        if (lds_mode) atomic_add_f64(&Stile[tri(row, col)], v);
                        else atomic_add_f64(&Sg[s_index(T.ld, (pa / 6) * dpf + i, (pb / 6) * dpf + j)], v);
                    }
                }
            }
        }
        wave_lds_fence();
    }
        }
    if (gemm_mode && wv * lpw < nl) {
        const int lr = ln & 15, lk = ln >> 4;
        const int nt16 = (Nt + 15) >> 4;
#pragma unroll
        for (int pp = 0; pp < 3; pp++) {
            const int tr = pp < 1 ? 0 : 1, tc = pp - tr;
            if (tr < nt16) {
                const int col = 16 * tc + lr;
#pragma unroll
                for (int rg = 0; rg < 4; rg++) {
                    const int row = 16 * tr + lk + 4 * rg;
                    if (row < Nt && col <= row) atomic_add_f64(&Stile[tri(row, col)], -accs[pp][rg]);
                }
            }
        }
    }
    SADVIO_TS(3, 40);
    const double c = wave_sum(cost_part), f = wave_sum(fixed_part), gm = wave_max(gmax_part);
    if (ln == 0) { s_part[wv * 4] = c; s_part[wv * 4 + 1] = f; s_part[wv * 4 + 2] = gm; }
    __syncthreads();
    if (tid == 0) {
        double cs = 0.0, fs = 0.0, gs = 0.0;
        for (int k = 0; k < BUILD_WAVES; k++) { cs += s_part[k * 4]; fs += s_part[k * 4 + 1]; gs = fmax(gs, s_part[k * 4 + 2]); }
        TileAcc* ta = P.tacc + (long long)(slot & 1) * P.n_tiles + blockIdx.x;
        ta->lin_cost = cs; ta->fixed_cost = fs; ta->gmax = gs;
    }
    SADVIO_TS(3, 41);
    if (lds_mode) {
        int* growTab = (int*)stage;
        for (int k = tid; k < T.n_kf; k += blockDim.x) {
            const int r = rowTab[k];
            if (r >= 0) {
                const int fi = P.kf_fidx[P.tile_kf[T.kf_off + k]];
#pragma unroll
                for (int i = 0; i < 6; i++) growTab[r + i] = fi * dpf + i;
            }
        }
        __syncthreads();
        if (T.ld) {
            for (int row = wv; row < Nt; row += BUILD_WAVES) {
                const long long grow = (long long)growTab[row] * T.ld;
                const double* srow = Stile + tri(row, 0);
                for (int col = ln; col <= row; col += 64) {
                    const double v = srow[col];
                    if (v != 0.0) atomic_add_f64(&Sg[grow + growTab[col]], v);
                }
            }
        } else {
            for (int col = wv; col < Nt; col += BUILD_WAVES) {
                const int gc = growTab[col];
                for (int row = col + ln; row < Nt; row += 64) {
                    const double v = Stile[tri(row, col)];
                    if (v != 0.0) atomic_add_f64(&Sg[c16_index(growTab[row], gc)], v);
                }
            }
        }
        for (int i = tid; i < Nt; i += blockDim.x) {
            const int row = growTab[i];
            if (gT[i] != 0.0) atomic_add_f64(&gredg[row], gT[i]);
            if (gfT[i] != 0.0) atomic_add_f64(&gfullg[row], gfT[i]);
            if (hdT[i] != 0.0) atomic_add_f64(&hdg[row], hdT[i]);
        }
    }
    SADVIO_TS(3, 42);
}

__device__ __forceinline__ double rsqrt_nr(double d) {
    double y = __builtin_amdgcn_rsq(d);
    const double t = d * y;
    const double e = __builtin_fma(-t, y, 1.0);
    const double p = __builtin_fma(0.375, e, 0.5);
    const double q = e * p;
    return __builtin_fma(y, q, y);
}

__device__ __forceinline__ double readlane_f64(double v, int lane) {
    int lo = __double2loint(v), hi = __double2hiint(v);
    lo = __builtin_amdgcn_readlane(lo, lane);
    hi = __builtin_amdgcn_readlane(hi, lane);
    return __hiloint2double(hi, lo);
}

constexpr int NBP = 6;

template <int NB>
__device__ __forceinline__ void factor_pivot(double (&Lk)[NB][NB], double (&Li)[NB][NB], bool& bad) {
#pragma unroll
    for (int j = 0; j < NB; j++) {
        double d = Lk[j][j];
#pragma unroll
        for (int q = 0; q < j; q++) d -= Lk[j][q] * Lk[j][q];
        if (!(d > 0.0) || !isfinite(d)) bad = true;
        double inv = rsqrt_nr(d);
        Lk[j][j] = d * inv;
        Li[j][j] = inv;
#pragma unroll
        for (int i = j + 1; i < NB; i++) {
            double t = Lk[i][j];
#pragma unroll
            for (int q = 0; q < j; q++) t -= Lk[i][q] * Lk[j][q];
            Lk[i][j] = t * inv;
        }
    }
#pragma unroll
    for (int j = 0; j < NB; j++)
#pragma unroll
        for (int i = j + 1; i < NB; i++) {
            double t = 0.0;
#pragma unroll
            for (int q = j; q < i; q++) t -= Lk[i][q] * Li[q][j];
            Li[i][j] = t * Li[i][i];
        }
}

template <int NB, bool UPDATE>
__device__ __forceinline__ void pivot_gather_factor(const double* P, const double* LpT, int ldp, int s0, int ln,
                                                    double* linv_out, bool& bad) {
    constexpr int NE = NB * (NB + 1) / 2;
    int i = 0, j = 0;
    {
        int e = ln < NE ? ln : 0, r = 0;
        while (e >= r + 1) { e -= r + 1; r++; }
        i = r; j = e;
    }
    double acc = P[tri(s0 + i, s0 + j)];
    if (UPDATE) {
#pragma unroll
        for (int c = 0; c < NB; c++) acc -= LpT[c * ldp + i] * LpT[c * ldp + j];
    }
    double Lk[NB][NB], Li[NB][NB];
    {
        int e = 0;
#pragma unroll
        for (int ii = 0; ii < NB; ii++)
#pragma unroll
            for (int jj = 0; jj <= ii; jj++) { Lk[ii][jj] = readlane_f64(acc, e); e++; }
    }
    factor_pivot<NB>(Lk, Li, bad);
    {
        double v = 0.0;
        int e = 0;
#pragma unroll
        for (int ii = 0; ii < NB; ii++)
#pragma unroll
            for (int jj = 0; jj <= ii; jj++) { if (ln == e) v = Li[ii][jj]; e++; }
        if (ln < NE) linv_out[i * NB + j] = v;
    }
// ... 787 lines not shown
            const double* sc = P.sp_scratch + (long long)cur * P.sp_scratch_stride + (long long)P.sp_list[W.spl_begin + kl] * SPARSE_J;
            if (q >= (int)sc[SPARSE_COL + 15]) continue;
            double jr[15], cd[15];
#pragma unroll
            for (int a = 0; a < 15; a++) { jr[a] = sc[q * 15 + a]; cd[a] = sc[SPARSE_COL + a]; }
            const double r = sc[225 + q];
            double m = 0.0;
#pragma unroll
            for (int a = 0; a < 15; a++) { const int ca = (int)cd[a]; if (ca >= 0) m += jr[a] * y[ca]; }
            mcc += -m * (r + 0.5 * m);
        }
    }
    if (EXTRAS && W.lobs_end > W.lobs_begin) {
        const int rows = W.factor_type == 0 ? 4 : 2;
        for (int it = tid; it < (W.lobs_end - W.lobs_begin) * 4; it += blockDim.x) {
            const int k = it >> 2, q = it & 3;
            if (q >= rows) continue;
            const LineObsDev& ob = P.lobs[W.lobs_begin + k];
            const int fi = P.kf_fidx[ob.kf], lc = P.lines[ob.line].col;
            if (fi < 0 && lc < 0) continue;
            const double* sc = P.line_scratch + (long long)(W.lobs_begin + k) * LINE_ROW;
            double m = 0.0;
            for (int a = 0; a < 6; a++) {
                if (fi >= 0) m += sc[q * 12 + a] * y[fi * W.dpf + a];
                if (lc >= 0) m += sc[q * 12 + 6 + a] * y[lc + a];
            }
            mcc += -m * (sc[48 + q] + 0.5 * m);
        }
    }
    SADVIO_TS(3, 7);
    sn = wave_sum(sn); cn = wave_sum(cn); mcc = wave_sum(mcc); cc = wave_sum(cc);
    if (bad) acc->chol_fail = 1;
    __syncthreads();
    if (ln == 0) { s_red[wv * 4] = sn; s_red[wv * 4 + 1] = cn; s_red[wv * 4 + 2] = mcc; s_red[wv * 4 + 3] = cc; }
    __syncthreads();
    if (tid == 0) {
        double a0 = 0, a1 = 0, a2 = 0, a3 = 0;
        for (int k = 0; k < nwv; k++) { a0 += s_red[k * 4]; a1 += s_red[k * 4 + 1]; a2 += s_red[k * 4 + 2]; a3 += s_red[k * 4 + 3]; }
        acc->step_norm2 = a0; acc->cand_norm2 = a1; acc->mcc = a2; acc->cand_cost = a3;
    }
    SADVIO_TS(3, 8);
    if (ts && tid == 0) { ts[15] = wall_clock64(); ts[21] = clock64(); }
}


__device__ __forceinline__ void zero_s_slice(const DevPtrs& P, const Tile& T, int tile_index) {
    if (T.ld != 0) return;
    const int n2 = c16_size(T.Np) >> 1;
    const int per = (n2 + T.win_ntiles - 1) / T.win_ntiles;
    const int i0 = (tile_index - T.win_tile0) * per, i1 = min(i0 + per, n2);
    double2* S2 = (double2*)(P.S + T.S_off);
    const double2 z2 = make_double2(0.0, 0.0);
    for (int i = i0 + (int)threadIdx.x; i < i1; i += blockDim.x) S2[i] = z2;
}

template <int FACTOR, bool RARE, bool IMU>
__global__ __launch_bounds__(BUILD_THREADS) void k_backsub(DevPtrs P, int slot, int max_tile_kf) {
    extern __shared__ __attribute__((aligned(16))) char smem[];
    if (IMU && (int)blockIdx.x >= P.n_tiles) {
        if (threadIdx.x < 64) pose_factor_eval<true>(P, slot, (int)blockIdx.x - P.n_tiles, threadIdx.x);
        return;
    }
    const Tile T = P.tiles[blockIdx.x];
    const int tid = threadIdx.x, wv = tid >> 6, ln = tid & 63;
    int4 pl = make_int4(0, -1, 0, 0);
    int2 pk = make_int2(-1, -1), pk6 = make_int2(-1, -1);
    if (P.pre_lane) {
        pl = P.pre_lane[(long long)blockIdx.x * (BUILD_THREADS / 8) + (tid >> 3)];
        pk = P.pre_kf[(long long)blockIdx.x * PRE_KF + tid / POSE_TAB];
        if (tid < PRE_KF * 6) pk6 = P.pre_kf[(long long)blockIdx.x * PRE_KF + tid / 6];
    }
    LmState st;
    int chol_fail;
    if (P.n_win == 1) { st = P.states[slot]; chol_fail = P.acc[slot].chol_fail; }
    else { st = P.states[(long long)T.w * P.state_stride + slot]; chol_fail = P.acc[(long long)T.w * P.state_stride + slot].chol_fail; }
    zero_s_slice(P, T, blockIdx.x);
    double* poseTab = (double*)smem;
    double* camTab = poseTab + (size_t)max_tile_kf * POSE_TAB;
    int* rowTab = (int*)(camTab + MAX_WIN_CAM * 17);
    double* candTab = (double*)(smem + tile_tables_bytes(max_tile_kf));
    double* dpTab = candTab + (size_t)max_tile_kf * 12;
    const int G = T.G, lpw = 64 / G;
    const int grp = ln / G, q = ln - grp * G;
    const int nl = T.lmk1 - T.lmk0;
    bool first_valid;
    int gl_first, pre_ob, pre_oe, pre_o;
    if (P.pre_lane) {
        first_valid = (pl.z >> 16) & 1; gl_first = pl.x; pre_ob = pl.y; pre_oe = pl.y + (pl.z & 0xff);
        pre_o = (pl.w + (tid & 7) < (pl.z & 0xff)) ? pl.y + pl.w + (tid & 7) : -1;
    } else {
        first_valid = wv * lpw + grp < nl;
        gl_first = T.lmk0 + (first_valid ? wv * lpw + grp : 0);
        pre_ob = P.lmk_ob[gl_first]; pre_oe = P.lmk_oe[gl_first];
        pre_o = (first_valid && q < pre_oe - pre_ob) ? pre_ob + q : -1;
    }
    const int pre_lcode = P.lmk_const ? P.lmk_const[gl_first] : 0;
    double pre_p[3], pre_xa[3], pre_xb[3];
#pragma unroll
    for (int i = 0; i < 3; i++) {
        pre_p[i] = P.lmk_p[3 * (long long)gl_first + i];
        pre_xa[i] = P.xl[3 * (long long)gl_first + i];
        pre_xb[i] = P.xl[P.xl_stride + 3 * (long long)gl_first + i];
    }
    ObsPre pre_obs;
    pre_obs.slot = 0; pre_obs.craw = 0; pre_obs.m[0] = pre_obs.m[1] = pre_obs.m[2] = 0.0;
    if (pre_o >= 0) pre_obs = obs_prefetch<FACTOR>(P, pre_o);
    double pre_t0 = 0.0, pre_t1 = 0.0;
    const bool pre_tab = P.pre_lane != nullptr;
    if (pre_tab && pk.x >= 0) {
        const long long src = (long long)pk.x * POSE_TAB + (tid - (tid / POSE_TAB) * POSE_TAB);
        pre_t0 = P.ptab[src]; pre_t1 = P.ptab[P.ptab_stride + src];
    }
    if (st.done || chol_fail) {
        if (tid == 0) {
            TileAcc* ta = P.tacc + (long long)(slot & 1) * P.n_tiles + blockIdx.x;
            ta->cand_cost = 0.0; ta->mcc = 0.0; ta->step_norm2 = 0.0; ta->cand_norm2 = 0.0;
        }
        return;
    }
    const int cur = st.cur;
    const double* xl = P.xl + (long long)cur * P.xl_stride;
    double* xlc = P.xl + (long long)(1 - cur) * P.xl_stride;
    double pre_x[3];
#pragma unroll
    for (int i = 0; i < 3; i++) pre_x[i] = cur ? pre_xb[i] : pre_xa[i];
    if (pre_tab) {
        const double* src = P.ptab + (long long)cur * P.ptab_stride;
        const double* srcc = P.ptab + (long long)(1 - cur) * P.ptab_stride;
        if (tid < T.n_kf * POSE_TAB) {
            const int k = tid / POSE_TAB, e = tid - k * POSE_TAB;
            poseTab[tid] = cur ? pre_t1 : pre_t0;
            if (e < 12) candTab[k * 12 + e] = cur ? pre_t0 : pre_t1;
        }
        for (int i = tid + blockDim.x; i < T.n_kf * POSE_TAB; i += blockDim.x) {
            const int k = i / POSE_TAB, e = i - k * POSE_TAB;
            const long long o = (long long)P.tile_kf[T.kf_off + k] * POSE_TAB + e;
            poseTab[i] = src[o];
            if (e < 12) candTab[k * 12 + e] = srcc[o];
        }
        for (int i = tid; i < T.n_cam * 17; i += blockDim.x) {
            const int c = i / 17, e = i - 17 * c;
            const int gc = T.cam_base + c;
            camTab[i] = e < 4 ? P.cam_K[4 * (long long)gc + e] : (e < 16 ? P.cam_T[12 * (long long)gc + e - 4] : P.cam_isig[gc]);
        }
        for (int i = tid; i < T.n_kf; i += blockDim.x) rowTab[i] = P.tile_row[T.kf_off + i];
        const double* dp = P.delta + T.red_off;
        for (int i = tid; i < T.n_kf * 6; i += blockDim.x) {
            const int k = i / 6, e = i - 6 * k;
            const int fi = (i < PRE_KF * 6) ? pk6.y : P.kf_fidx[P.tile_kf[T.kf_off + k]];
            dpTab[i] = fi < 0 ? 0.0 : dp[fi * T.dpf + e];
        }
    } else {
        stage_tables(P, T, cur, poseTab, camTab, rowTab);
        const double* src = P.ptab + (long long)(1 - cur) * P.ptab_stride;
        for (int i = tid; i < T.n_kf * 12; i += blockDim.x) {
            const int k = i / 12, e = i - 12 * k;
            candTab[i] = src[(long long)P.tile_kf[T.kf_off + k] * POSE_TAB + e];
        }
        const double* dp = P.delta + T.red_off;
        for (int i = tid; i < T.n_kf * 6; i += blockDim.x) {
            const int k = i / 6, e = i - 6 * k;
            const int fi = P.kf_fidx[P.tile_kf[T.kf_off + k]];
            dpTab[i] = fi < 0 ? 0.0 : dp[fi * T.dpf + e];
        }
    }
    __syncthreads();
    double sn = 0.0, cn = 0.0, mcc = 0.0, cc = 0.0;
    for (int base = wv * lpw; base < nl; base += BUILD_WAVES * lpw) {
        const int lm = base + grp;
        const bool lmk_valid = lm < nl;
        const int gl = T.lmk0 + (lmk_valid ? lm : 0);
        const bool first = base == wv * lpw;
        const int ob = first ? pre_ob : P.lmk_ob[gl], oe = first ? pre_oe : P.lmk_oe[gl];
        const int nobs = lmk_valid ? oe - ob : 0;
        const int lcode = first ? pre_lcode : (P.lmk_const ? P.lmk_const[gl] : 0);
        const bool lfree = lcode == 0;
        double p0[3], x0[3];
#pragma unroll
        for (int i = 0; i < 3; i++) {
            p0[i] = first ? pre_p[i] : P.lmk_p[3 * (long long)gl + i];
            x0[i] = first ? pre_x[i] : xl[3 * (long long)gl + i];
        }
        ObsLin L;
        L.valid = q < nobs;
        L.row = -1; L.slot = 0; L.counted = false;
        ObsPre obq = pre_obs;
        if (L.valid) {
            const double pw[3] = {p0[0] + x0[0], p0[1] + x0[1], p0[2] + x0[2]};
            if (!first) obq = obs_prefetch<FACTOR>(P, ob + q);
            lane_linearize<FACTOR, RARE>(P, poseTab, camTab, rowTab, T.cam_base, obq, pw, lcode != 1, lcode != 1, L);
            if (!L.counted) { L.r[0] = 0.0; L.r[1] = 0.0; }
        } else {
            L.r[0] = L.r[1] = 0.0;
#pragma unroll
            for (int i = 0; i < 12; i++) L.Jp[i] = 0.0;
#pragma unroll
            for (int i = 0; i < 6; i++) L.Jl[i] = 0.0;
        }
        double Mi[6], g[3];
        const bool active = group_eliminate(P, L, G, gl, lmk_valid, lfree, nobs, st.radius, false, false, Mi, g);

        double e0 = L.r[0], e1 = L.r[1];
        const double* d = dpTab + L.slot * 6;
        if (L.valid && L.row >= 0) {
#pragma unroll
            for (int i = 0; i < 6; i++) { e0 += L.Jp[i] * d[i]; e1 += L.Jp[6 + i] * d[i]; }
        }
        const double tt[3] = {group_sum(L.Jl[0] * e0 + L.Jl[3] * e1, G), group_sum(L.Jl[1] * e0 + L.Jl[4] * e1, G),
                              group_sum(L.Jl[2] * e0 + L.Jl[5] * e1, G)};
        double ut[3], vt3[3];
        li_vec(Mi, tt, ut);
        li_tvec(Mi, ut, vt3);
        double d0 = -vt3[0], d1 = -vt3[1], d2 = -vt3[2];
        if (RARE && lcode == 2) {
            const double* dr = P.delta + T.red_off + P.lmk_red[gl];
            d0 = dr[0]; d1 = dr[1]; d2 = dr[2];
        }
        const double c0 = x0[0] + d0, c1 = x0[1] + d1, c2 = x0[2] + d2;
        if (lmk_valid && q == 0) {
            xlc[3 * (long long)gl] = c0; xlc[3 * (long long)gl + 1] = c1; xlc[3 * (long long)gl + 2] = c2;
            if (active) {
                sn += d0 * d0 + d1 * d1 + d2 * d2;
                cn += c0 * c0 + c1 * c1 + c2 * c2;
            } else if (RARE && lcode == 2 && (P.world == 1 || P.rank == 0)) cn += c0 * c0 + c1 * c1 + c2 * c2;
        }
        if (L.valid && L.counted) {
            const double m0 = (e0 - L.r[0]) + L.Jl[0] * d0 + L.Jl[1] * d1 + L.Jl[2] * d2;
            const double m1 = (e1 - L.r[1]) + L.Jl[3] * d0 + L.Jl[4] * d1 + L.Jl[5] * d2;
            mcc += -m0 * (L.r[0] + 0.5 * m0) - m1 * (L.r[1] + 0.5 * m1);
            const int craw = obq.craw;
            const int cam = craw < 0 ? 0 : craw - T.cam_base;
            const double* ct = camTab + cam * 17;
            const double pw[3] = {p0[0] + c0, p0[1] + c1, p0[2] + c2};
            const double* ctab = candTab + L.slot * 12;
            double r[2];
            if (RARE && craw < 0) {
                const int code = -1 - craw;
                const SparseDev& f = P.sparse[code >> 1];
                p2l_pseudo_obs<false>(ctab, pw, f.delta, f.W, code & 1, r, nullptr, nullptr);
                cc += r[0] * r[0] + r[1] * r[1];
            } else {
            if (FACTOR == 0) {
                pixel_factor<false>(ctab, ct, ct + 4, pw, obq.m[0], obq.m[1], ct[16], r, nullptr, nullptr);
            } else {
                double bb[3] = {obq.m[0], obq.m[1], obq.m[2]};
                angular_factor<false>(ctab, ct + 4, pw, bb, ct[16], r, nullptr, nullptr);
            }
            double sc_unused;
            cc += RARE ? huber_rho(P.o.huber_a, r[0] * r[0] + r[1] * r[1], sc_unused) : r[0] * r[0] + r[1] * r[1];
            }
        }
    }
    sn = wave_sum(sn); cn = wave_sum(cn); mcc = wave_sum(mcc); cc = wave_sum(cc);
    __shared__ double s_part[BUILD_WAVES * 4];
    if (ln == 0) { s_part[wv * 4] = cc; s_part[wv * 4 + 1] = mcc; s_part[wv * 4 + 2] = sn; s_part[wv * 4 + 3] = cn; }
// ... 930 lines not shown
```

Before: 18070 BA iterations/s.

## Pack landmarks into tiles by keyframe coverage with indirect landmark index

```diff
diff --git a/sadvio_amd/csrc/ba_capi.hip b/sadvio_amd/csrc/ba_capi.hip
--- a/sadvio_amd/csrc/ba_capi.hip
+++ b/sadvio_amd/csrc/ba_capi.hip
@@ -13,6 +13,7 @@
 
 #include "../../include/sadvio_ba.h"
 #include "kernels.h"
+#include "tile_pack.h"
 #include "dense_chol.h"
 #include "marg_kernels.h"
 #include "lm_kernels.h"
@@ -206,7 +207,7 @@
 
 struct LayoutScratch {
     std::vector<double> kf_T0, kf_vel, kf_ba, kf_bg, cam_K, cam_T, cam_isig, lmk_p, obs_meas;
-    std::vector<int> kf_fidx, lmk_ob, lmk_oe, obs_kf, obs_cam, tile_kf, tile_row, pkf, pcam, run_max, idx, mark, add, kfs, slot_of, chunk_ob, chunk_lm, perm;
+    std::vector<int> kf_fidx, lmk_ob, lmk_oe, obs_kf, obs_cam, tile_kf, tile_row, tile_lmk, pack_order, pack_cut, pkf, pcam, run_max, idx, mark, add, kfs, slot_of, chunk_ob, chunk_lm, perm;
     std::vector<unsigned char> lmk_const, obs_slot, obs_lslot;
     std::vector<char> held;
 };
@@ -217,7 +218,7 @@
     int tile_rounds = 0, lm_subs = 0, band_c = 0;
     double jacobi_tol = 1e-14;
     bool marg_last_small = false, marg_eig_mm = false, marg_pivoted = false, marg_unpivoted = false, pchol_swap = false, pchol_strict = false,
-         jacobi_b4 = false, jacobi_plain = false, no_lpt = false, no_pre = false, no_fork = false, no_bcr = false, imu_items = false;
+         jacobi_b4 = false, jacobi_plain = false, no_lpt = false, no_pre = false, no_fork = false, no_bcr = false, imu_items = false, contig_tiles = false;
     void read() {
         auto on = [](const char* k) { return getenv(k) != nullptr; };
         auto num = [](const char* k, int unset) { const char* e = getenv(k); return e ? atoi(e) : unset; };
@@ -228,6 +229,7 @@
         marg_unpivoted = on("SADVIO_MARG_UNPIVOTED"); pchol_swap = on("SADVIO_PCHOL_SWAP"); pchol_strict = on("SADVIO_PCHOL_STRICT");
         jacobi_b4 = on("SADVIO_JACOBI_B4"); jacobi_plain = on("SADVIO_JACOBI_PLAIN"); no_lpt = on("SADVIO_NO_LPT"); no_pre = on("SADVIO_NO_PRE"); no_fork = on("SADVIO_NO_FORK");
         no_bcr = on("SADVIO_NO_BCR");
+        contig_tiles = on("SADVIO_CONTIG_TILES");
         imu_items = on("SADVIO_IMU_ITEMS");
     }
 };
@@ -298,7 +300,7 @@
     DevBuf<double> d_cam_K, d_cam_T, d_cam_isig;
     DevBuf<double> d_lmk_p, d_xl, d_s_lmk;
     DevBuf<unsigned char> d_lmk_const;
-    DevBuf<int> d_lmk_ob, d_lmk_oe, d_obs_kf, d_obs_cam, d_tile_kf, d_tile_row;
+    DevBuf<int> d_lmk_ob, d_lmk_oe, d_obs_kf, d_obs_cam, d_tile_kf, d_tile_row, d_tile_lmk;
     DevBuf<int> d_pre_lane, d_pre_kf;
     bool pre_ok = false, pre_dirty = false;
     DevBuf<int> d_rank_col; DevBuf<double> d_rank_x;
@@ -400,7 +402,7 @@
     P.lmk_const = h->has_lmk_const ? h->d_lmk_const.p : nullptr;
     P.lmk_ob = h->d_lmk_ob.p; P.lmk_oe = h->d_lmk_oe.p;
     P.obs_kf = h->d_obs_kf.p; P.obs_cam = h->d_obs_cam.p; P.obs_meas = h->d_obs_meas.p;
-    P.obs_slot = h->d_obs_slot.p; P.tile_kf = h->d_tile_kf.p; P.tile_row = h->d_tile_row.p;
+    P.obs_slot = h->d_obs_slot.p; P.tile_kf = h->d_tile_kf.p; P.tile_lmk = h->d_tile_lmk.p; P.tile_row = h->d_tile_row.p;
     P.pre_lane = h->pre_ok ? (const int4*)h->d_pre_lane.p : nullptr; P.pre_kf = h->pre_ok ? (const int2*)h->d_pre_kf.p : nullptr;
     P.ptab = h->d_ptab.p; P.ptab_stride = (long long)POSE_TAB * h->n_kf_tot;
     P.priors = h->d_priors.p; P.prior_lin = h->d_prior_lin.p; P.prior_lin_stride = (long long)h->priors.size() * PRIOR_LIN; P.n_prior_tot = (int)h->priors.size();
@@ -665,7 +667,7 @@
     HIP_TRY(h->up.flush(h->stream));
     if (h->pre_ok && h->pre_dirty) {
         hipLaunchKernelGGL(k_pre_packets, dim3((unsigned)h->tiles.size()), dim3(BUILD_THREADS), 0, h->stream, h->d_tiles.p, h->d_lmk_ob.p, h->d_lmk_oe.p, h->d_tile_kf.p,
-                           h->d_kf_fidx.p, (int4*)h->d_pre_lane.p, (int2*)h->d_pre_kf.p);
+                           h->d_tile_lmk.p, h->d_kf_fidx.p, (int4*)h->d_pre_lane.p, (int2*)h->d_pre_kf.p);
         h->pre_dirty = false;
     }
     return SADVIO_OK;
@@ -745,7 +747,7 @@
     h->d_lmk_ob.release(); h->d_lmk_oe.release(); h->d_obs_kf.release(); h->d_obs_cam.release();
     h->d_obs_meas.release(); h->d_priors.release(); h->d_prior_lin.release(); h->d_S.release(); h->d_rank_s.release(); h->d_gred.release(); h->d_gfull.release();
     h->d_hdiag.release(); h->d_delta.release(); h->d_s_pose.release(); h->d_states.release(); h->d_trace.release(); h->d_tstart.release(); h->d_acc.release();
-    h->d_probe.release(); h->d_tile_kf.release(); h->d_tile_row.release(); h->d_obs_slot.release(); h->d_ptab.release(); h->d_tacc.release(); h->d_dbg.release(); h->d_imus.release(); h->d_imu_scratch.release();
+    h->d_probe.release(); h->d_tile_kf.release(); h->d_tile_row.release(); h->d_tile_lmk.release(); h->d_obs_slot.release(); h->d_ptab.release(); h->d_tacc.release(); h->d_dbg.release(); h->d_imus.release(); h->d_imu_scratch.release();
     delete h;
 }
 
@@ -884,7 +886,7 @@
     auto& kf_T0 = ls.kf_T0; auto& kf_vel = ls.kf_vel; auto& kf_ba = ls.kf_ba; auto& kf_bg = ls.kf_bg; auto& kf_fidx = ls.kf_fidx;
     auto& cam_K = ls.cam_K; auto& cam_T = ls.cam_T; auto& cam_isig = ls.cam_isig; auto& lmk_p = ls.lmk_p; auto& lmk_const = ls.lmk_const;
     auto& lmk_ob = ls.lmk_ob; auto& lmk_oe = ls.lmk_oe; auto& obs_kf = ls.obs_kf; auto& obs_cam = ls.obs_cam; auto& obs_meas = ls.obs_meas;
-    auto& tile_kf = ls.tile_kf; auto& tile_row = ls.tile_row; auto& obs_slot = ls.obs_slot;
+    auto& tile_kf = ls.tile_kf; auto& tile_row = ls.tile_row; auto& tile_lmk = ls.tile_lmk; auto& obs_slot = ls.obs_slot;
     kf_T0.resize(12 * (size_t)kf_b); kf_vel.assign(3 * (size_t)kf_b, 0.0); kf_ba.assign(3 * (size_t)kf_b, 0.0); kf_bg.assign(3 * (size_t)kf_b, 0.0);
     kf_fidx.resize(kf_b);
     cam_K.resize(4 * (size_t)cam_b); cam_T.resize(12 * (size_t)cam_b); cam_isig.resize(cam_b);
@@ -893,7 +895,7 @@
     lmk_ob.resize(std::max(lmk_b, 1)); lmk_oe.resize(std::max(lmk_b, 1)); obs_kf.resize(std::max(obs_b, 1)); obs_cam.resize(std::max(obs_b, 1));
     const int ms = h->factor_type == SADVIO_FACTOR_PIXEL ? 2 : 3;
     obs_meas.resize((size_t)ms * std::max(obs_b, 1));
-    tile_kf.clear(); tile_row.clear();
+    tile_kf.clear(); tile_row.clear(); tile_lmk.clear();
     obs_slot.assign(std::max(obs_b, 1), 0);
     h->obs_perm.assign(std::max(obs_b, 1), 0);
     h->max_tile_kf = 1; h->max_tile_free = 0; h->max_gemm_free = 0; h->gemm_run4 = false;
@@ -996,13 +998,26 @@
             if (h->env.tile_rounds > 0) tile_rounds = h->env.tile_rounds;
         }
         d.tile_begin = (int)h->tiles.size();
+        bool want_lm_w = lmk_b >= 65536;
+        if (h->env.lm >= 0) want_lm_w = h->env.lm != 0;
+        const bool packed = n_windows == 1 && tile_rounds == 1 && F.n_lmk > 0 && h->world == 1 && !h->coll_fn && !want_lm_w && !h->env.contig_tiles;
+        auto& order = ls.pack_order; auto& cut = ls.pack_cut;
+        if (packed) {
+            for (int l = 0; l < F.n_lmk; l++)
+                if (F.lmk_obs_ptr[l + 1] - F.lmk_obs_ptr[l] > MAX_LMK_OBS) { h->err = "set_windows: a landmark has more than 64 observations"; return SADVIO_E_INVALID_ARG; }
+            const TilePackIn in{F.n_lmk, F.n_kf, F.lmk_obs_ptr, pkf.data(), F.kf_const, run_max.data(), BUILD_WAVES * 64, MAX_TILE_KF, MAX_TILE_FREE_KF, MAX_GEMM_FREE_KF};
+            tile_pack(in, order, cut);
+        }
         {
             int l = 0;
+            size_t next_cut = 0;
+            auto lm_at = [&](int i) { return packed ? order[i] : i; };
             auto& mark = ls.mark; auto& add = ls.add; auto& kfs = ls.kfs; auto& slot_of = ls.slot_of;
             mark.assign(F.n_kf, -1); slot_of.assign(F.n_kf, -1);
             while (l < F.n_lmk || (int)h->tiles.size() == d.tile_begin) {
                 Tile t{};
-                t.w = w; t.lmk0 = d.lmk_base + l; t.kmax = 1; t.G = 8;
+                t.w = w; t.lmk0 = d.lmk_base + (l < F.n_lmk ? lm_at(l) : l); t.kmax = 1; t.G = 8;
+                t.lmk_off = packed ? (int)tile_lmk.size() : -1;
                 t.dpf = d.dpf;
                 t.cam_base = d.cam_base; t.n_cam = F.n_cam;
                 t.first_of_window = ((int)h->tiles.size() == d.tile_begin) ? 1 : 0;
@@ -1010,15 +1025,17 @@
                 int nfree = 0, tile_run_max = 0;
                 const int l_begin = l;
                 while (l < F.n_lmk) {
-                    const int k = F.lmk_obs_ptr[l + 1] - F.lmk_obs_ptr[l];
+                    const int gl = lm_at(l);
+                    if (packed && l == cut[next_cut]) break;
+                    const int k = F.lmk_obs_ptr[gl + 1] - F.lmk_obs_ptr[gl];
                     if (k > MAX_LMK_OBS) { h->err = "set_windows: a landmark has more than 64 observations"; return SADVIO_E_INVALID_ARG; }
                     int G = t.G;
                     while (G < k) G <<= 1;
                     const int cap = tile_rounds * BUILD_WAVES * (64 / G);
-                    if (l - l_begin + 1 > cap && l > l_begin) break;
+                    if (!packed && l - l_begin + 1 > cap && l > l_begin) break;
                     add.clear();
                     int add_free = 0;
-                    for (int o = F.lmk_obs_ptr[l]; o < F.lmk_obs_ptr[l + 1]; o++) {
+                    for (int o = F.lmk_obs_ptr[gl]; o < F.lmk_obs_ptr[gl + 1]; o++) {
                         const int kf = pkf[o];
                         if (mark[kf] != (int)h->tiles.size()) {
                             mark[kf] = (int)h->tiles.size();
@@ -1028,7 +1045,7 @@
                     }
                     const bool fits_hard = (int)(kfs.size() + add.size()) <= MAX_TILE_KF && nfree + add_free <= MAX_TILE_FREE_KF;
                     const bool fits = fits_hard && (nfree + add_free <= MAX_GEMM_FREE_KF || l == l_begin);
-                    if (!fits && l > l_begin) {
+                    if (!packed && !fits && l > l_begin) {
                         for (int kf : add) mark[kf] = -1;
                         break;
                     }
@@ -1036,11 +1053,14 @@
                     nfree += add_free;
                     t.G = G;
                     t.kmax = std::max(t.kmax, k);
-                    tile_run_max = std::max(tile_run_max, run_max[l]);
+                    tile_run_max = std::max(tile_run_max, run_max[gl]);
+                    if (packed) tile_lmk.push_back(d.lmk_base + gl);
                     l++;
-                    if (!fits_hard) break;
+                    if (!packed && !fits_hard) break;
                 }
-                t.lmk1 = d.lmk_base + l;
+                if (packed) next_cut++;
+                t.n_lmk = l - l_begin;
+                t.lmk1 = t.lmk0 + t.n_lmk;
                 std::sort(kfs.begin(), kfs.end());
                 t.lds_mode = ((int)kfs.size() <= MAX_TILE_KF && nfree <= MAX_TILE_FREE_KF) ? ((nfree <= MAX_GEMM_FREE_KF && tile_run_max <= (has_asrc ? 4 : 2) && t.G == 8) ? 2 : 1) : 0;
                 if (t.lds_mode == 2 && tile_run_max > 2) h->gemm_run4 = true;
@@ -1057,8 +1077,8 @@
                     else if (t.lds_mode) tile_row.push_back(6 * rank++);
                     else tile_row.push_back(6 * kf_fidx[d.kf_base + kf]);
                 }
-                for (int ll = l_begin; ll < l; ll++)
-                    for (int o = F.lmk_obs_ptr[ll]; o < F.lmk_obs_ptr[ll + 1]; o++)
+                for (int li = l_begin; li < l; li++)
+                    for (int o = F.lmk_obs_ptr[lm_at(li)]; o < F.lmk_obs_ptr[lm_at(li) + 1]; o++)
                         obs_slot[d.obs_base + o] = (unsigned char)slot_of[pkf[o]];
                 h->max_tile_kf = std::max(h->max_tile_kf, t.n_kf);
                 h->max_tile_free = std::max(h->max_tile_free, t.n_free);
@@ -1151,7 +1171,8 @@
     }
     HIP_TRY(h->d_win.alloc(n_windows)); HIP_TRY(h->d_tacc.alloc(2 * h->tiles.size()));
     if (tile_kf.empty()) { tile_kf.push_back(0); tile_row.push_back(-1); }
-    HIP_TRY(h->d_tile_kf.alloc(tile_kf.size())); HIP_TRY(h->d_tile_row.alloc(tile_row.size()));
+    if (tile_lmk.empty()) tile_lmk.push_back(0);
+    HIP_TRY(h->d_tile_kf.alloc(tile_kf.size())); HIP_TRY(h->d_tile_row.alloc(tile_row.size())); HIP_TRY(h->d_tile_lmk.alloc(tile_lmk.size()));
     HIP_TRY(h->d_obs_slot.alloc(obs_slot.size())); HIP_TRY(h->d_ptab.alloc(2 * (size_t)POSE_TAB * kf_b));
     HIP_TRY(h->d_kf_T0.alloc(kf_T0.size())); HIP_TRY(h->d_kf_fidx.alloc(kf_fidx.size()));
     HIP_TRY(h->d_xp.alloc(2 * 6 * (size_t)kf_b)); HIP_TRY(h->d_xv.alloc(2 * 3 * (size_t)kf_b));
@@ -1167,7 +1188,7 @@
     UP(h->d_kf_ba, kf_ba); UP(h->d_kf_bg, kf_bg); UP(h->d_cam_K, cam_K); UP(h->d_cam_T, cam_T); UP(h->d_cam_isig, cam_isig);
     if (lmk_b) { UP(h->d_lmk_p, lmk_p); }
     UP(h->d_lmk_ob, lmk_ob); UP(h->d_lmk_oe, lmk_oe); UP(h->d_obs_kf, obs_kf);
-    UP(h->d_obs_cam, obs_cam); UP(h->d_obs_meas, obs_meas); UP(h->d_tile_kf, tile_kf); UP(h->d_tile_row, tile_row); UP(h->d_obs_slot, obs_slot);
+    UP(h->d_obs_cam, obs_cam); UP(h->d_obs_meas, obs_meas); UP(h->d_tile_kf, tile_kf); UP(h->d_tile_row, tile_row); UP(h->d_tile_lmk, tile_lmk); UP(h->d_obs_slot, obs_slot);
     h->pre_ok = !h->tiles.empty() && h->tiles.size() <= PRE_MAX_TILES && !h->env.no_pre;
     if (h->pre_ok) {
         HIP_TRY(h->d_pre_lane.alloc((size_t)4 * (BUILD_THREADS / 8) * h->tiles.size())); HIP_TRY(h->d_pre_kf.alloc((size_t)2 * PRE_KF * h->tiles.size()));
@@ -1576,7 +1597,7 @@
     const double jtol = h->env.jacobi_tol;
     int sweeps = 0;
     long long* jts = nullptr;
-    if ((h->env.debug & 4096) && n > 500 && h->d_dbg.alloc(128) == hipSuccess) jts = h->d_dbg.p + 44;
+    if ((h->env.debug & 4096) && n > 500 && h->d_dbg.alloc(DBG_SLOTS) == hipSuccess) jts = h->d_dbg.p + 44;
     for (; sweeps < 40 && nbpad >= 2; sweeps++) {
         if (hipMemsetAsync(flag, 0, sizeof(int), h->stream) != hipSuccess) return -1;
         for (int st = 0; st < nbpad - 1; st++) {
@@ -2695,7 +2716,7 @@
     const int n_win = (int)h->wins.size();
     const int slots = std::max(1, o.max_num_iterations);
     const int stride = slots + 2;
-    HIP_TRY(h->d_dbg.alloc(128));
+    HIP_TRY(h->d_dbg.alloc(DBG_SLOTS));
     HIP_TRY(h->d_states.alloc((size_t)n_win * stride));
     HIP_TRY(h->d_trace.alloc((size_t)n_win * stride * 8));
     HIP_TRY(h->d_tstart.alloc(1));
@@ -2925,7 +2946,7 @@
         unsigned char* kp = key.data();
         memcpy(kp + sizeof(DevPtrs) + 8 * sizeof(int) + 3 * sizeof(size_t), lay.data(), lay.size() * sizeof(int));
         memcpy(kp, &P, sizeof(DevPtrs)); kp += sizeof(DevPtrs);
-        const int env_bits = (int)with_imu + 2 * (int)h->env.no_fork + 32 * (int)h->env.no_bcr + 128 * (int)h->env.no_lpt;
+        const int env_bits = (int)with_imu + 2 * (int)h->env.no_fork + 32 * (int)h->env.no_bcr + 128 * (int)h->env.no_lpt + 256 * (int)h->env.contig_tiles;
         const int ints[8] = {slots, n_tiles, n_win, mtk, strip_doubles, Rp, h->n_kf_tot, h->factor_type + 2 * (int)extras + 4 * (int)rare + 8 * (int)use_lm + 16 * env_bits};
         memcpy(kp, ints, sizeof(ints)); kp += sizeof(ints);
         const size_t szs[3] = {lds_build, lds_back, lds_solve};
@@ -2968,6 +2989,15 @@
             for (int i = 45; i < 55; i++) fprintf(stderr, " %d:%.2f", i - 44, (ts[i] - ts[44]) * 0.01);
             fprintf(stderr, "\n");
         }
+#ifdef SADVIO_KERNEL_TS
+        std::vector<long long> wg(4 * (size_t)std::min(n_tiles, DBG_WG_MAX));
+        if (!wg.empty() && hipMemcpy(wg.data(), h->d_dbg.p + DBG_WG_BASE, wg.size() * sizeof(long long), hipMemcpyDeviceToHost) == hipSuccess)
+            for (size_t b = 0; b < wg.size() / 4; b++) {
+                const unsigned hw = (unsigned)wg[4 * b + 2];
+                fprintf(stderr, "[sadvio dbg] k_build wg %zu start %.2f end %.2f xcc %d se %u sh %u cu %u simd %u\n", b, (wg[4 * b] - wg[0]) * 0.01, (wg[4 * b + 1] - wg[0]) * 0.01,
+                        (int)((wg[4 * b + 2] >> 32) & 15), (hw >> 13) & 7, (hw >> 12) & 1, (hw >> 8) & 15, (hw >> 4) & 3);
+            }
+#endif
     }
     h->fin.assign(h->h_final, h->h_final + n_win);
     h->deltas_cached = false;
diff --git a/sadvio_amd/csrc/ba_types.h b/sadvio_amd/csrc/ba_types.h
--- a/sadvio_amd/csrc/ba_types.h
+++ b/sadvio_amd/csrc/ba_types.h
@@ -40,6 +40,8 @@
 struct Tile {
     int w;
     int lmk0, lmk1;
+    int lmk_off;
+    int n_lmk;
     int G;
     int kf_off, n_kf;
     int n_free;
diff --git a/sadvio_amd/csrc/kernels.h b/sadvio_amd/csrc/kernels.h
--- a/sadvio_amd/csrc/kernels.h
+++ b/sadvio_amd/csrc/kernels.h
@@ -20,6 +20,7 @@
     const int* obs_kf; const int* obs_cam; const double* obs_meas;
     const unsigned char* obs_slot;
     const int* tile_kf;
+    const int* tile_lmk;
     const int* tile_row;
     const int4* pre_lane;
     const int2* pre_kf;
@@ -83,9 +84,15 @@
 #ifdef SADVIO_KERNEL_TS
 #define SADVIO_TS(slot_, idx_) do { if ((P.debug & 4096) && blockIdx.x == 0 && threadIdx.x == 0 && slot == (slot_)) P.dbg_ts[idx_] = wall_clock64(); } while (0)
 #define SADVIO_TS_PTR(cond_) ((cond_) ? P.dbg_ts : nullptr)
+constexpr int DBG_WG_MAX = 1024, DBG_WG_BASE = 128, DBG_SLOTS = DBG_WG_BASE + 4 * DBG_WG_MAX;
+#define SADVIO_WG_TS(slot_, which_) do { if ((P.debug & 4096) && blockIdx.x < DBG_WG_MAX && threadIdx.x == 0 && slot == (slot_)) { \
+        P.dbg_ts[DBG_WG_BASE + 4 * blockIdx.x + (which_)] = wall_clock64(); \
+        if ((which_) == 0) P.dbg_ts[DBG_WG_BASE + 4 * blockIdx.x + 2] = ((long long)__builtin_amdgcn_s_getreg(20 | (31 << 11)) << 32) | (unsigned)__builtin_amdgcn_s_getreg(4 | (31 << 11)); } } while (0)
 #else
 #define SADVIO_TS(slot_, idx_) do { } while (0)
 #define SADVIO_TS_PTR(cond_) nullptr
+#define SADVIO_WG_TS(slot_, which_) do { } while (0)
+constexpr int DBG_SLOTS = 128;
 #endif
 
 __device__ __forceinline__ int tri(int i, int j) { return i * (i + 1) / 2 + j; }
@@ -432,16 +439,18 @@
     return (b + 15) & ~(size_t)15;
 }
 
+__device__ __forceinline__ int tile_landmark(const Tile& T, const int* __restrict__ tile_lmk, int i) { return T.lmk_off >= 0 ? tile_lmk[T.lmk_off + i] : T.lmk0 + i; }
+
 __global__ __launch_bounds__(BUILD_THREADS) void k_pre_packets(const Tile* __restrict__ tiles, const int* __restrict__ lmk_ob, const int* __restrict__ lmk_oe,
-                                                               const int* __restrict__ tile_kf, const int* __restrict__ kf_fidx, int4* __restrict__ pre_lane,
+                                                               const int* __restrict__ tile_kf, const int* __restrict__ tile_lmk, const int* __restrict__ kf_fidx, int4* __restrict__ pre_lane,
                                                                int2* __restrict__ pre_kf) {
     const Tile T = tiles[blockIdx.x];
     const int tid = threadIdx.x;
     if (tid < BUILD_THREADS / 8) {
         const int lane0 = tid * 8, wv = lane0 >> 6, ln = lane0 & 63;
-        const int G = T.G, lpw = 64 / G, grp = ln / G, q0 = ln - grp * G, nl = T.lmk1 - T.lmk0;
+        const int G = T.G, lpw = 64 / G, grp = ln / G, q0 = ln - grp * G, nl = T.n_lmk;
         const bool valid = wv * lpw + grp < nl;
-        const int gl = T.lmk0 + (valid ? wv * lpw + grp : 0);
+        const int gl = nl > 0 ? tile_landmark(T, tile_lmk, valid ? wv * lpw + grp : 0) : T.lmk0;
         const int ob = nl > 0 ? lmk_ob[gl] : 0, nobs = (valid && nl > 0) ? lmk_oe[gl] - ob : 0;
         pre_lane[(long long)blockIdx.x * (BUILD_THREADS / 8) + tid] = make_int4(gl, ob, nobs | (valid ? 1 << 16 : 0), q0);
     }
@@ -469,6 +478,7 @@
         pk = P.pre_kf[(long long)blockIdx.x * PRE_KF + tid / POSE_TAB];
     }
     SADVIO_TS(3, 32);
+    SADVIO_WG_TS(3, 0);
     __shared__ double s_part[BUILD_WAVES * 4];
     double* poseTab = (double*)smem;
     double* camTab = poseTab + (size_t)max_tile_kf * POSE_TAB;
@@ -476,7 +486,7 @@
     double* stage = (double*)(smem + tile_tables_bytes(max_tile_kf));
     const int G = T.G, lpw = 64 / G;
     const int grp = ln / G, q = ln - grp * G;
-    const int nl = T.lmk1 - T.lmk0;
+    const int nl = T.n_lmk;
     LmState st;
     IterAcc a;
     LmState prev;
@@ -517,7 +527,7 @@
         pre_o = (pl.w + (tid & 7) < (pl.z & 0xff)) ? pl.y + pl.w + (tid & 7) : -1;
     } else {
         first_valid = wv * lpw + grp < nl;
-        gl_first = T.lmk0 + (first_valid ? wv * lpw + grp : 0);
+        gl_first = tile_landmark(T, P.tile_lmk, first_valid ? wv * lpw + grp : 0);
         pre_ob = P.lmk_ob[gl_first]; pre_oe = P.lmk_oe[gl_first];
         pre_o = (first_valid && q < pre_oe - pre_ob) ? pre_ob + q : -1;
     }
@@ -597,8 +607,8 @@
     for (int base = wv * lpw; base < nl; base += BUILD_WAVES * lpw) {
         const int lm = base + grp;
         const bool lmk_valid = lm < nl;
-        const int gl = T.lmk0 + (lmk_valid ? lm : 0);
         const bool first = base == wv * lpw;
+        const int gl = first ? gl_first : tile_landmark(T, P.tile_lmk, lmk_valid ? lm : 0);
         const int ob = first ? pre_ob : P.lmk_ob[gl], oe = first ? pre_oe : P.lmk_oe[gl];
         const int nobs = lmk_valid ? oe - ob : 0;
         const int lcode = first ? pre_lcode : (P.lmk_const ? P.lmk_const[gl] : 0);
@@ -863,6 +873,7 @@
         }
     }
     SADVIO_TS(3, 42);
+    SADVIO_WG_TS(3, 1);
 }
 
 __device__ __forceinline__ double rsqrt_nr(double d) {
@@ -1816,7 +1827,7 @@
     double* dpTab = candTab + (size_t)max_tile_kf * 12;
     const int G = T.G, lpw = 64 / G;
     const int grp = ln / G, q = ln - grp * G;
-    const int nl = T.lmk1 - T.lmk0;
+    const int nl = T.n_lmk;
     bool first_valid;
     int gl_first, pre_ob, pre_oe, pre_o;
     if (P.pre_lane) {
@@ -1824,7 +1835,7 @@
         pre_o = (pl.w + (tid & 7) < (pl.z & 0xff)) ? pl.y + pl.w + (tid & 7) : -1;
     } else {
         first_valid = wv * lpw + grp < nl;
-        gl_first = T.lmk0 + (first_valid ? wv * lpw + grp : 0);
+        gl_first = tile_landmark(T, P.tile_lmk, first_valid ? wv * lpw + grp : 0);
         pre_ob = P.lmk_ob[gl_first]; pre_oe = P.lmk_oe[gl_first];
         pre_o = (first_valid && q < pre_oe - pre_ob) ? pre_ob + q : -1;
     }
@@ -1903,8 +1914,8 @@
     for (int base = wv * lpw; base < nl; base += BUILD_WAVES * lpw) {
         const int lm = base + grp;
         const bool lmk_valid = lm < nl;
-        const int gl = T.lmk0 + (lmk_valid ? lm : 0);
         const bool first = base == wv * lpw;
+        const int gl = first ? gl_first : tile_landmark(T, P.tile_lmk, lmk_valid ? lm : 0);
         const int ob = first ? pre_ob : P.lmk_ob[gl], oe = first ? pre_oe : P.lmk_oe[gl];
         const int nobs = lmk_valid ? oe - ob : 0;
         const int lcode = first ? pre_lcode : (P.lmk_const ? P.lmk_const[gl] : 0);
diff --git a/sadvio_amd/csrc/tile_pack.h b/sadvio_amd/csrc/tile_pack.h
--- /dev/null
+++ b/sadvio_amd/csrc/tile_pack.h
@@ -0,0 +1,94 @@
+#pragma once
+#include <algorithm>
+#include <vector>
+
+constexpr int TILE_PACK_ASIDE = 4;
+
+struct TilePackIn {
+    int n_lmk, n_kf;
+    const int* obs_ptr;
+    const int* obs_kf;
+    const unsigned char* kf_const;
+    const int* run_max;
+    int lanes;
+    int max_kf, max_free, gemm_free;
+};
+
+inline void tile_pack(const TilePackIn& in, std::vector<int>& order, std::vector<int>& cut) {
+    order.clear(); cut.clear();
+    struct Open { std::vector<int> kfs; int begin = 0, n = 0, nfree = 0, G = 8, run = 0, aside = 0; bool hard = false; };
+    std::vector<int> mark(in.n_kf, -1);
+    std::vector<int> aside;
+    std::vector<Open> done;
+    auto is_free = [&](int kf) { return !(in.kf_const && in.kf_const[kf]); };
+    auto lanes_of = [&](int l, int G) { while (G < in.obs_ptr[l + 1] - in.obs_ptr[l]) G <<= 1; return G; };
+    auto probe = [&](const Open& t, int ti, int l, int& G, int& add_kf, int& add_free) {
+        G = lanes_of(l, t.G);
+        add_kf = add_free = 0;
+        if (t.n + 1 > in.lanes / G && t.n > 0) return false;
+        for (int o = in.obs_ptr[l]; o < in.obs_ptr[l + 1]; o++) {
+            const int kf = in.obs_kf[o];
+            bool seen = mark[kf] == ti;
+            for (int p = in.obs_ptr[l]; p < o && !seen; p++) seen = in.obs_kf[p] == kf;
+            if (!seen) { add_kf++; add_free += is_free(kf); }
+        }
+        const bool fits_hard = (int)t.kfs.size() + add_kf <= in.max_kf && t.nfree + add_free <= in.max_free;
+        return t.n == 0 || (fits_hard && t.nfree + add_free <= in.gemm_free);
+    };
+    auto admit = [&](Open& t, int ti, int l, int G) {
+        for (int o = in.obs_ptr[l]; o < in.obs_ptr[l + 1]; o++) {
+            const int kf = in.obs_kf[o];
+            if (mark[kf] != ti) { mark[kf] = ti; t.kfs.push_back(kf); t.nfree += is_free(kf); }
+        }
+        t.G = G; t.n++; t.run = std::max(t.run, in.run_max[l]);
+        t.hard = (int)t.kfs.size() > in.max_kf || t.nfree > in.max_free;
+        order.push_back(l);
+    };
+    auto run_cut = [&](const std::vector<int>* seq, int n, bool may_set_aside) {
+        int i = 0;
+        while (i < n) {
+            Open t; t.begin = (int)order.size();
+            const int ti = (int)done.size();
+            while (i < n) {
+                const int l = seq ? (*seq)[i] : i;
+                int G, ak, af;
+                if (probe(t, ti, l, G, ak, af)) { admit(t, ti, l, G); i++; if (t.hard) break; continue; }
+                int G2, ak2, af2;
+                const bool cap_cut = t.n + 1 > in.lanes / G;
+                if (may_set_aside && !cap_cut && t.aside < TILE_PACK_ASIDE && i + 1 < n && probe(t, ti, seq ? (*seq)[i + 1] : i + 1, G2, ak2, af2)) {
+                    aside.push_back(l); t.aside++; i++;
+                    continue;
+                }
+                break;
+            }
+            done.push_back(std::move(t));
+        }
+    };
+    run_cut(nullptr, in.n_lmk, true);
+    std::vector<std::vector<int>> extra(done.size());
+    std::vector<int> rest;
+    for (int l : aside) {
+        int home = -1;
+        for (int ti = 0; ti < (int)done.size() && home < 0; ti++) {
+            const Open& t = done[ti];
+            if (t.hard || lanes_of(l, t.G) != t.G || t.n + (int)extra[ti].size() + 1 > in.lanes / t.G || in.run_max[l] > t.run) continue;
+            bool covered = true;
+            for (int o = in.obs_ptr[l]; o < in.obs_ptr[l + 1] && covered; o++) covered = mark[in.obs_kf[o]] == ti || std::find(t.kfs.begin(), t.kfs.end(), in.obs_kf[o]) != t.kfs.end();
+            if (covered) home = ti;
+        }
+        if (home >= 0) extra[home].push_back(l); else rest.push_back(l);
+    }
+    std::vector<int> first_pass;
+    first_pass.swap(order);
+    for (size_t ti = 0; ti < done.size(); ti++) {
+        order.insert(order.end(), first_pass.begin() + done[ti].begin, first_pass.begin() + done[ti].begin + done[ti].n);
+        order.insert(order.end(), extra[ti].begin(), extra[ti].end());
+        cut.push_back((int)order.size());
+    }
+    std::stable_sort(rest.begin(), rest.end(), [&](int a, int b) {
+        const int ka = in.obs_ptr[a + 1] > in.obs_ptr[a] ? in.obs_kf[in.obs_ptr[a]] : -1, kb = in.obs_ptr[b + 1] > in.obs_ptr[b] ? in.obs_kf[in.obs_ptr[b]] : -1;
+        return ka < kb; });
+    const size_t n_first = done.size();
+    run_cut(&rest, (int)rest.size(), false);
+    for (size_t ti = n_first; ti < done.size(); ti++) cut.push_back(done[ti].begin + done[ti].n);
+}
```

Result: faster. 18640 BA iterations/s, median of 6 (+3.2%).
